# HoangChuongNguyen/ibgs

Measured on AMD Instinct MI355X. Metric: train-step fps (fwd+bwd raster) @1080p, 1M Gaussians, higher is better.
Workload: dtype f32

## Files before the change

ibgs_amd/_lib.py:

```python
import ctypes
import os

_HERE = os.path.dirname(os.path.abspath(__file__))
LIB_PATH = os.environ.get("IBGS_LIB") or os.path.join(_HERE, "libibgs_rast.so")

MAX_SRC = 5
MAX_BUFFER_LENGTH = 8
FLAG_DEBUG = 1
FLAG_TEX_QUANT = 2
FLAG_NO_TILE_CULL = 4
FLAG_CLEAR_GRAD_ACC = 8
FLAG_SH_FACTORED = 16
FLAG_TILE_WAVES = 32
FLAG_QUADRANT_WAVES = 64
FLAG_DETERMINISTIC = 128
FLAG_TEX_PACKED = 256
FLAG_NO_REF_POWER_SKIP = 512
FLAG_NO_ABS_GRAD = 1024
FLAG_REF_ARITH = 4096
FLAG_SRC_DEPTH_SLOTS = 8192
PLANE_NONE, PLANE_LEARNT, PLANE_SMALLEST_AXIS = 0, 1, 2
MAX_VIEWS = 8

c_float_p = ctypes.c_void_p

ALLOC_FN = ctypes.CFUNCTYPE(ctypes.c_void_p, ctypes.c_size_t, ctypes.c_void_p)


class ForwardArgs(ctypes.Structure):
    _fields_ = [
        ("stream", ctypes.c_void_p),
        ("P", ctypes.c_int32), ("D", ctypes.c_int32), ("M", ctypes.c_int32),
        ("W", ctypes.c_int32), ("H", ctypes.c_int32),
        ("means3D", c_float_p), ("shs", c_float_p), ("colors_precomp", c_float_p), ("opacities", c_float_p),
        ("scales", c_float_p), ("rotations", c_float_p), ("cov3D_precomp", c_float_p), ("all_map", c_float_p),
        ("scale_modifier", ctypes.c_float),
        ("bg", c_float_p), ("viewmatrix", c_float_p), ("projmatrix", c_float_p), ("campos", c_float_p),
        ("tanfovx", ctypes.c_float), ("tanfovy", ctypes.c_float),
        ("n_src", ctypes.c_int32),
        ("ref_to_src", c_float_p), ("src_cam_pos", c_float_p), ("src_images", c_float_p), ("src_depths", c_float_p),
        ("buffer_length", ctypes.c_int32), ("depth_error_threshold", ctypes.c_float),
        ("prefiltered", ctypes.c_int32), ("render_geo", ctypes.c_int32), ("render_depth_only", ctypes.c_int32),
        ("flags", ctypes.c_uint32),
        ("geom", ctypes.c_void_p), ("geom_bytes", ctypes.c_size_t),
        ("img", ctypes.c_void_p), ("img_bytes", ctypes.c_size_t),
        ("binning_alloc", ALLOC_FN), ("binning_user", ctypes.c_void_p),
        ("tex", ctypes.c_void_p), ("tex_bytes", ctypes.c_size_t),
        ("out_color", c_float_p), ("radii", ctypes.c_void_p), ("out_normal", c_float_p), ("out_depth", c_float_p),
        ("out_cam_feat", c_float_p), ("out_warped", c_float_p), ("out_min_depth_diff", c_float_p),
        ("out_camera_ray", c_float_p), ("out_mask", ctypes.c_void_p),
        ("rendered_hint", ctypes.c_int64),
        ("plane_normal", c_float_p), ("plane_offset", c_float_p), ("plane_mode", ctypes.c_int32),
        ("n_views", ctypes.c_int32), ("view_tanfovx", ctypes.c_float * 8), ("view_tanfovy", ctypes.c_float * 8),
        ("tile_order_hint", ctypes.c_void_p),
        ("binning", ctypes.c_void_p), ("binning_bytes", ctypes.c_size_t),
        ("shs_rest", c_float_p),
        ("src_depth_slot", ctypes.c_int32 * 5),
    ]


class AdamTensor(ctypes.Structure):
    _fields_ = [("param", ctypes.c_void_p), ("grad", ctypes.c_void_p), ("exp_avg", ctypes.c_void_p), ("exp_avg_sq", ctypes.c_void_p),
                ("numel", ctypes.c_int64), ("lr", ctypes.c_double), ("beta1", ctypes.c_double), ("beta2", ctypes.c_double),
                ("eps", ctypes.c_double), ("bias_correction1", ctypes.c_double), ("bias_correction2", ctypes.c_double)]


class CompactTensor(ctypes.Structure):
    _fields_ = [("src", ctypes.c_void_p), ("append", ctypes.c_void_p), ("dst", ctypes.c_void_p), ("width", ctypes.c_int32), ("reserved", ctypes.c_int32)]


COMPACT_MAX_TENSORS = 40


class BackwardArgs(ctypes.Structure):
    _fields_ = [
        ("stream", ctypes.c_void_p),
        ("P", ctypes.c_int32), ("D", ctypes.c_int32), ("M", ctypes.c_int32),
        ("W", ctypes.c_int32), ("H", ctypes.c_int32),
        ("R", ctypes.c_int64),
        ("means3D", c_float_p), ("shs", c_float_p), ("colors_precomp", c_float_p),
        ("scales", c_float_p), ("rotations", c_float_p), ("cov3D_precomp", c_float_p), ("all_map", c_float_p),
        ("scale_modifier", ctypes.c_float),
        ("bg", c_float_p), ("viewmatrix", c_float_p), ("projmatrix", c_float_p), ("campos", c_float_p),
        ("tanfovx", ctypes.c_float), ("tanfovy", ctypes.c_float),
        ("n_src", ctypes.c_int32),
        ("ref_to_src", c_float_p), ("src_cam_pos", c_float_p), ("src_images", c_float_p), ("src_depths", c_float_p),
        ("radii", ctypes.c_void_p),
        ("out_depth", c_float_p), ("out_warped", c_float_p),
        ("geom", ctypes.c_void_p), ("binning", ctypes.c_void_p), ("img", ctypes.c_void_p),
        ("tex", ctypes.c_void_p), ("tex_bytes", ctypes.c_size_t),
        ("dL_dcolor", c_float_p), ("dL_dnormal", c_float_p), ("dL_ddepth", c_float_p), ("dL_dwarped", c_float_p),
        ("grad_acc", c_float_p),
        ("dL_dmean2D", c_float_p), ("dL_dmean2D_abs", c_float_p), ("dL_dconic", c_float_p), ("dL_dopacity", c_float_p),
        ("dL_dcolors", c_float_p), ("dL_dmean3D", c_float_p), ("dL_dcov3D", c_float_p), ("dL_dsh", c_float_p),
        ("dL_dscale", c_float_p), ("dL_drot", c_float_p), ("dL_dall_map", c_float_p),
        ("render_geo", ctypes.c_int32), ("flags", ctypes.c_uint32),
        ("plane_normal", c_float_p), ("plane_offset", c_float_p), ("plane_mode", ctypes.c_int32),
        ("dL_dplane_normal", c_float_p), ("dL_dplane_offset", c_float_p),
        ("geo_table", ctypes.c_void_p), ("geo_table_bytes", ctypes.c_size_t),
        ("det_scratch", ctypes.c_void_p), ("det_scratch_bytes", ctypes.c_size_t),
        ("buffer_length", ctypes.c_int32),
        ("tile_order_out", ctypes.c_void_p),
        ("shs_rest", c_float_p), ("dL_dsh_rest", c_float_p),
    ]


EXPORTS = ["ibgs_required_geom", "ibgs_required_img", "ibgs_required_binning", "ibgs_required_tex",
           "ibgs_forward", "ibgs_backward", "ibgs_mark_visible", "ibgs_tile_order_slots",
           "ibgs_geom_offset", "ibgs_img_offset", "ibgs_binning_offset",
           "ibgs_sizeof_forward_args", "ibgs_sizeof_backward_args", "ibgs_timing_enable", "ibgs_timing_collect",
           "ibgs_required_knn", "ibgs_knn_mean_dist2", "ibgs_sh_grad_from_views", "ibgs_adam_step", "ibgs_adam_step_sh",
           "ibgs_required_compact", "ibgs_compact_plan", "ibgs_compact_apply", "ibgs_densify_stats", "ibgs_required_deterministic", "ibgs_required_geo_table", "ibgs_required_deterministic_for", "ibgs_required_geo_table_for", "ibgs_last_forward_stats", "ibgs_check_async",
           "ibgs_required_l1", "ibgs_l1_loss", "ibgs_l1_grad", "ibgs_l1_rescale",
           "ibgs_depth_normal_forward", "ibgs_depth_normal_backward", "ibgs_activate_forward", "ibgs_activate_backward",
           "ibgs_last_error", "ibgs_version"]

TSDF_EXPORTS = ["ibgs_tsdf_sizeof_volume", "ibgs_tsdf_sizeof_view", "ibgs_tsdf_sizeof_mesh_scratch", "ibgs_tsdf_mc_table",
                "ibgs_tsdf_integrate", "ibgs_tsdf_mesh_count", "ibgs_tsdf_mesh_emit"]
TSDF_STATE_WORDS = 8
TSDF_ALLOCATED, TSDF_FAILED, TSDF_IGNORED, TSDF_ACTIVE, TSDF_VERTICES, TSDF_FACES, TSDF_OVERRUN, TSDF_TABLE_FULL = range(8)
TSDF_FLAG_NO_DEDUP = 1


class TsdfVolume(ctypes.Structure):
    _fields_ = [("voxel_length", ctypes.c_float), ("sdf_trunc", ctypes.c_float), ("capacity", ctypes.c_int32), ("slot_bits", ctypes.c_int32),
                ("slot_key", ctypes.c_void_p), ("slot_block", ctypes.c_void_p), ("slot_mark", ctypes.c_void_p), ("active", ctypes.c_void_p),
                ("block_key", ctypes.c_void_p), ("tsdf", ctypes.c_void_p), ("weight", ctypes.c_void_p), ("color", ctypes.c_void_p),
                ("state", ctypes.c_void_p)]


class TsdfView(ctypes.Structure):
    _fields_ = [("W", ctypes.c_int32), ("H", ctypes.c_int32), ("fx", ctypes.c_float), ("fy", ctypes.c_float), ("cx", ctypes.c_float),
                ("cy", ctypes.c_float), ("depth_trunc", ctypes.c_float), ("world_to_camera", ctypes.c_float * 12),
                ("camera_to_world", ctypes.c_float * 12)]


class TsdfMeshScratch(ctypes.Structure):
    _fields_ = [("order", ctypes.c_void_p), ("rank", ctypes.c_void_p), ("vinfo", ctypes.c_void_p), ("vcount", ctypes.c_void_p),
                ("fcount", ctypes.c_void_p)]


MESH_EXPORTS = ["ibgs_mesh_sizeof_mesh", "ibgs_mesh_required_scratch", "ibgs_mesh_cluster", "ibgs_mesh_filter_count", "ibgs_mesh_filter_emit"]
MESH_STATE_WORDS = 8
MESH_BAD_FACES, MESH_CLUSTERS, MESH_VERTICES_OUT, MESH_FACES_OUT, MESH_TABLE_FULL, MESH_OVERRUN = range(6)
MESH_KEEP_VERTICES, MESH_KEEP_DEGENERATE = 1, 2


class Mesh(ctypes.Structure):
    _fields_ = [("V", ctypes.c_int32), ("F", ctypes.c_int32), ("vertices", ctypes.c_void_p), ("faces", ctypes.c_void_p), ("scratch", ctypes.c_void_p),
                ("scratch_bytes", ctypes.c_size_t), ("state", ctypes.c_void_p)]


MESH_EVAL_EXPORTS = ["ibgs_meval_required_sample_scratch", "ibgs_meval_sample_count", "ibgs_meval_sample_emit", "ibgs_meval_keys", "ibgs_meval_required_tree",
                     "ibgs_meval_build", "ibgs_meval_thin_rounds", "ibgs_meval_nearest", "ibgs_meval_reduce"]
MEVAL_STATE_WORDS = 8
MEVAL_BAD_FACES, MEVAL_SAMPLE_OVERFLOW, MEVAL_BAD_POINTS, MEVAL_OVERRUN, MEVAL_UNDECIDED = range(5)
MEVAL_MAX_SIDE = 32768
MEVAL_LEAF = 8
MEVAL_THIN_UNDECIDED, MEVAL_THIN_KEPT, MEVAL_THIN_REMOVED = 0, 1, 2

PCREG_EXPORTS = ["ibgs_pcreg_required_scratch", "ibgs_pcreg_bounds", "ibgs_pcreg_transform", "ibgs_pcreg_crop", "ibgs_pcreg_voxel_keys",
                 "ibgs_pcreg_voxel_count", "ibgs_pcreg_voxel_emit", "ibgs_pcreg_moments"]
PCREG_STATE_WORDS = 8
PCREG_BAD_POINTS, PCREG_KEY_OVERFLOW, PCREG_BAD_INDEX, PCREG_OVERRUN = range(4)
PCREG_MAX_POLYGON = 1024
PCREG_MAX_INDEX = (1 << 21) - 1
PCREG_LONG_SEGMENT = 64
PCREG_MOMENTS = 18


_lib = None


# ... 195 lines not shown
```

ibgs_amd/csrc/api.hip:

```cpp
#include "common.h"
#include "sh_color.h"
#include <sched.h>
#include <time.h>
#include <string.h>
#include <cstdlib>
#include <stdlib.h>
#include <stdio.h>
#include <cstdarg>
#include <cstdio>
#include <cstring>
#include <vector>
#include <map>
#include <mutex>

namespace ibgs {

static thread_local char g_err[512] = "";
void set_error(const char* fmt, ...)
{
    va_list ap; va_start(ap, fmt);
    vsnprintf(g_err, sizeof(g_err), fmt, ap);
    va_end(ap);
}

// ... 99 lines not shown

static int stage_check(hipStream_t s, bool debug, const char* what)
{
    if (!debug) return 0;
    hipError_t e = hipStreamSynchronize(s);
    if (e == hipSuccess) e = hipGetLastError();
    if (e != hipSuccess) { set_error("stage '%s' failed: %s", what, hipGetErrorString(e)); return -IBGS_ERR_HIP; }
    return 0;
}

__global__ void __launch_bounds__(1024) rendered_note_kernel(RenderedNote n)
{
    __shared__ unsigned long long s_w[16];
    rendered_note_block<1024>(n, s_w);
}

}

using namespace ibgs;

extern "C" {

const char* ibgs_last_error(void) { return g_err; }
const char* ibgs_version(void) { return "ibgs_rast 0.1 (gfx950)"; }
void ibgs_timing_enable(uint32_t stage_mask) { g_time_mask = stage_mask; }
int32_t ibgs_timing_collect(float* ms, int32_t* launches)
{
    for (int i = 0; i < IBGS_NUM_STAGES; i++) { if (ms) ms[i] = 0.f; if (launches) launches[i] = 0; }
    for (auto& p : g_pairs) {
        float t = 0.f;
        hipError_t e = hipEventSynchronize(p.b);
        if (e == hipSuccess) e = hipEventElapsedTime(&t, p.a, p.b);
        if (e != hipSuccess) { set_error("timing collect: %s", hipGetErrorString(e)); return -IBGS_ERR_HIP; }
        if (ms) ms[p.stage] += t;
        if (launches) launches[p.stage] += 1;
        g_free_events.push_back(p.a); g_free_events.push_back(p.b);
    }
    g_pairs.clear();
    return 0;
}
size_t ibgs_sizeof_forward_args(void) { return sizeof(ibgs_forward_args); }
size_t ibgs_sizeof_backward_args(void) { return sizeof(ibgs_backward_args); }

size_t ibgs_required_geom(int32_t P) { size_t t; GeomState::carve(nullptr, (size_t)(P > 0 ? P : 0), &t); return t; }
size_t ibgs_required_img(int32_t W, int32_t H) { size_t t; ImgState::carve(nullptr, W, H, &t); return t; }
size_t ibgs_required_binning(int64_t R, int32_t W, int32_t H) { size_t t; BinState::carve(nullptr, (size_t)(R > 0 ? R : 0), W, H, &t); return t; }
size_t ibgs_required_deterministic(int64_t R, int32_t P) { size_t t; DetState::carve(nullptr, (size_t)(R > 0 ? R : 0) * 4, (size_t)(P > 0 ? P : 0), &t); return t; }
size_t ibgs_required_tex(int32_t n_src, int32_t W, int32_t H) { return (size_t)n_src * W * H * sizeof(float4) + 128; }
size_t ibgs_required_geo_table(int32_t W, int32_t H) { return geo_table_floats(W, H) * sizeof(float) + 128; }
size_t ibgs_required_geo_table_for(int32_t W, int32_t H, int32_t L)
{
    const int slots = (L >= 1 && L < IBGS_MAX_BUFFER_LENGTH) ? L + 1 : IBGS_MAX_BUFFER_LENGTH;
    return (size_t)W * H * slots * GEO_TAB_FIELDS * sizeof(float) + 128;
}
size_t ibgs_required_deterministic_for(int64_t R, int32_t P, int32_t W, int32_t H, int32_t render_geo, uint32_t flags)
{
    ibgs_backward_args a{}; a.W = W; a.H = H; a.render_geo = render_geo; a.flags = flags;
    size_t t; DetState::carve(nullptr, (size_t)(R > 0 ? R : 0) * render_backward_waves_per_tile(a), (size_t)(P > 0 ? P : 0), &t); return t;
}

#define OFF(base_struct, field) if (!strcmp(name, #field)) return (int64_t)((char*)base_struct.field - (char*)nullptr)
int64_t ibgs_geom_offset(int32_t P, const char* name)
{
    size_t t; GeomState g = GeomState::carve(nullptr, (size_t)P, &t);
    OFF(g, rec); OFF(g, depths); OFF(g, cov3D); OFF(g, tiles); OFF(g, fp); OFF(g, tmask_hi); OFF(g, clamped); OFF(g, offsets);
    if (!strcmp(name, "order")) return (int64_t)((char*)g.sort_val[0] - (char*)nullptr);
    if (!strcmp(name, "order_alt")) return (int64_t)((char*)g.sort_val[1] - (char*)nullptr);
    if (!strcmp(name, "sorted_depth_keys")) return (int64_t)((char*)g.sort_key[0] - (char*)nullptr);
    if (!strcmp(name, "sorted_depth_keys_alt")) return (int64_t)((char*)g.sort_key[1] - (char*)nullptr);
    return -1;
}
size_t ibgs_tile_order_slots(int32_t W, int32_t H)
{
    const size_t tiles = (size_t)((W + TILE - 1) / TILE) * ((H + TILE - 1) / TILE);
    return (tiles + ORDER_CLASSES - 1) / ORDER_CLASSES * ORDER_CLASSES;
}
int64_t ibgs_img_offset(int32_t W, int32_t H, const char* name)
{
    size_t t; ImgState im = ImgState::carve(nullptr, W, H, &t);
    OFF(im, ranges); OFF(im, final_T); OFF(im, n_contrib); OFF(im, sum_w); OFF(im, low_high); OFF(im, valid_idx); OFF(im, valid_w); OFF(im, slot_c); OFF(im, meta); OFF(im, tile_walked); OFF(im, tile_order); OFF(im, tile_risky);
    return -1;
}
int64_t ibgs_binning_offset(int64_t R, int32_t W, int32_t H, const char* name)
{
    size_t t; BinState b = BinState::carve(nullptr, (size_t)R, W, H, &t);
    OFF(b, point_list);
    return -1;
}
#undef OFF

struct RSlot {
    uint32_t* host; hipEvent_t ev;
    uint32_t* stats; bool stats_pending;
    bool flag_pending;
    hipStream_t last_stream;
    uint32_t seq;
};
static std::mutex g_slot_mutex;
static std::map<std::pair<int, hipStream_t>, RSlot*> g_slots;
static RSlot* rslot(hipStream_t s, bool create)
{
    int dev = 0;
    if (hipGetDevice(&dev) != hipSuccess) { set_error("hipGetDevice failed"); return nullptr; }
    std::lock_guard<std::mutex> lock(g_slot_mutex);
    auto it = g_slots.find({dev, s});
    if (it != g_slots.end()) return it->second;
    if (!create) return nullptr;
    RSlot* slot = new RSlot();
    void* p = nullptr;
    if (hipHostMalloc(&p, 64, hipHostMallocCoherent | hipHostMallocMapped) != hipSuccess) { delete slot; set_error("hipHostMalloc for the R read-back failed"); return nullptr; }
    if (hipEventCreateWithFlags(&slot->ev, hipEventDisableTiming) != hipSuccess) { (void)hipHostFree(p); delete slot; set_error("hipEventCreate failed"); return nullptr; }
    slot->host = static_cast<uint32_t*>(p);
    memset(p, 0, 64);
    slot->stats = slot->host + 8;
    slot->stats_pending = false; slot->flag_pending = false; slot->last_stream = s; slot->seq = 0;
    g_slots[{dev, s}] = slot;
    return slot;
}
static int check_sort_flag(RSlot* rs, bool wait_for_note)
{
    if (!rs || !rs->flag_pending) return 0;
    volatile uint32_t* note = rs->stats + 4;
    bool final_ = __atomic_load_n(const_cast<uint32_t*>(note), __ATOMIC_ACQUIRE) == rs->seq;
    if (!final_ && wait_for_note) {
        struct timespec t0, t1; clock_gettime(CLOCK_MONOTONIC, &t0);
        for (uint32_t spins = 1; !final_; spins++) {
            final_ = __atomic_load_n(const_cast<uint32_t*>(note), __ATOMIC_ACQUIRE) == rs->seq;
            if ((spins & 255u) == 0) {
                clock_gettime(CLOCK_MONOTONIC, &t1);
                if ((t1.tv_sec - t0.tv_sec) * 1000000000ll + (t1.tv_nsec - t0.tv_nsec) > 2000000ll) break;
            }
        }
    }
    if (*(volatile uint32_t*)(rs->stats + 3)) {
        rs->stats[3] = 0u; rs->flag_pending = false;
        set_error("depth sort: decoupled look-back timed out (the lists of this stream's last forward were mis-ordered)"); return -IBGS_ERR_HIP;
    }
    if (final_) rs->flag_pending = false;
    return 0;
}

static thread_local int64_t g_last_stats[3] = {0, -1, 0};
static thread_local RSlot* g_stats_slot = nullptr;
void ibgs_last_forward_stats(int64_t* out)
{
    if (g_stats_slot && g_stats_slot->stats_pending) {
        if (hipStreamSynchronize(g_stats_slot->last_stream) == hipSuccess) g_last_stats[1] = (int64_t)*(volatile uint32_t*)(g_stats_slot->stats + 2);
        g_stats_slot->stats_pending = false;
    }
    out[0] = g_last_stats[0]; out[1] = g_last_stats[1]; out[2] = g_last_stats[2];
}
void ibgs_debug_set_lookback_spins(uint32_t v) { radix_set_lookback_spins(v); }
void ibgs_debug_set_sh_ride(int32_t on) { radix_set_sh_ride(on != 0); }
size_t ibgs_debug_scan_scratch_elems(size_t n) { return scan_scratch_elems(n); }
int32_t ibgs_debug_scan_u32(void* stream, const uint32_t* in, uint32_t* out, size_t n, uint32_t* scratch, size_t scratch_elems, int32_t with_total)
{
    return exclusive_scan_u32(reinterpret_cast<hipStream_t>(stream), in, out, n, scratch, scratch_elems, with_total != 0);
}
size_t ibgs_debug_sort_scratch_elems(size_t n) { return radix_hist_elems(n); }
int32_t ibgs_debug_sort_pairs(void* stream, uint32_t* keys0, uint32_t* keys1, uint32_t* vals0, uint32_t* vals1, size_t n, int32_t nbits,
                              uint32_t* scratch, size_t scratch_elems, uint32_t* kept_dev, uint32_t* result_alt)
{
    uint32_t* keys[2] = {keys0, keys1};
    uint32_t* vals[2] = {vals0, vals1};
    return radix_sort_pairs(reinterpret_cast<hipStream_t>(stream), keys, vals, n, nbits, scratch, scratch_elems, nullptr, kept_dev, false, result_alt, nullptr);
}
int32_t ibgs_debug_set_onesweep(int32_t mode) { return radix_set_onesweep(mode); }
int32_t ibgs_check_async(void* stream, int32_t wait)
{
    hipStream_t s = reinterpret_cast<hipStream_t>(stream);
    RSlot* rs = rslot(s, false);
    if (!rs || !rs->flag_pending) return 0;
    if (wait) IBGS_HIP(hipStreamSynchronize(s));
    return check_sort_flag(rs, false);
}

int64_t ibgs_forward(const ibgs_forward_args* ap)
{
    if (!ap) { set_error("null args"); return -IBGS_ERR_INVALID; }
    const ibgs_forward_args& a = *ap;
    hipStream_t s = reinterpret_cast<hipStream_t>(a.stream);
    const bool debug = (a.flags & IBGS_FLAG_DEBUG) != 0;
    if (a.P < 0 || a.W <= 0 || a.H <= 0) { set_error("bad sizes P=%d W=%d H=%d", a.P, a.W, a.H); return -IBGS_ERR_INVALID; }
    if (a.P == 0) return 0;
    if (!a.means3D || !a.opacities || !a.viewmatrix || !a.projmatrix || !a.campos || !a.bg || !a.radii) {
        set_error("missing required pointer"); return -IBGS_ERR_INVALID;
    }
    if ((a.shs == nullptr) == (a.colors_precomp == nullptr) && !a.render_depth_only) {
        set_error("provide exactly one of shs / colors_precomp"); return -IBGS_ERR_INVALID;
    }
    if (((a.scales == nullptr) || (a.rotations == nullptr)) == (a.cov3D_precomp == nullptr)) {
        set_error("provide exactly one of scales+rotations / cov3D_precomp"); return -IBGS_ERR_INVALID;
    }
    if (a.shs && (a.D < 0 || a.D > 3 || (a.D + 1) * (a.D + 1) > a.M)) { set_error("bad SH degree D=%d M=%d", a.D, a.M); return -IBGS_ERR_INVALID; }
    if (a.shs && a.M == 16 && (reinterpret_cast<uintptr_t>(a.shs) & 15u)) { set_error("shs (M = 16) must be 16-byte aligned"); return -IBGS_ERR_INVALID; }
    if (a.shs_rest && (!a.shs || a.M < 2 || (reinterpret_cast<uintptr_t>(a.shs_rest) & 15u) || (reinterpret_cast<uintptr_t>(a.shs) & 15u))) {
        set_error("shs_rest needs shs (the DC coefficients), M >= 2 and 16-byte aligned arrays"); return -IBGS_ERR_INVALID;
    }
    if (a.render_geo && a.render_depth_only) { set_error("render_geo together with render_depth_only is not supported"); return -IBGS_ERR_INVALID; }
    if (a.plane_mode != IBGS_PLANE_NONE) {
        if (a.all_map) { set_error("give either all_map or plane_mode, not both"); return -IBGS_ERR_INVALID; }
        if (a.plane_mode == IBGS_PLANE_LEARNT ? !a.plane_normal : (a.plane_mode != IBGS_PLANE_SMALLEST_AXIS || !a.scales || !a.rotations)) {
            set_error("plane_mode %d: plane_normal (learnt) or scales + rotations (smallest axis) required", a.plane_mode); return -IBGS_ERR_INVALID;
        }
    }
    if ((a.render_geo || a.render_depth_only) && !a.all_map && a.plane_mode == IBGS_PLANE_NONE) { set_error("all_map (or plane_mode) is required for render_geo / render_depth_only"); return -IBGS_ERR_INVALID; }
    if (a.render_geo || a.render_depth_only) {
        if (a.buffer_length < 1 || a.buffer_length > IBGS_MAX_BUFFER_LENGTH) { set_error("buffer_length %d outside 1..%d", a.buffer_length, IBGS_MAX_BUFFER_LENGTH); return -IBGS_ERR_INVALID; }
        if (!a.out_depth) { set_error("out_depth required"); return -IBGS_ERR_INVALID; }
    }
    if (a.render_geo) {
        if (a.n_src < 1 || a.n_src > IBGS_MAX_SRC) { set_error("n_src %d outside 1..%d", a.n_src, IBGS_MAX_SRC); return -IBGS_ERR_INVALID; }
        if (!a.ref_to_src || !a.src_cam_pos || !a.src_images || !a.src_depths) { set_error("source view pointers required for render_geo"); return -IBGS_ERR_INVALID; }
        if (a.flags & IBGS_FLAG_SRC_DEPTH_SLOTS) {
            for (int m = 0; m < a.n_src; m++) if (a.src_depth_slot[m] < 0) { set_error("src_depth_slot[%d] = %d is negative", m, a.src_depth_slot[m]); return -IBGS_ERR_INVALID; }
        }
        if (!a.out_normal || !a.out_cam_feat || !a.out_warped || !a.out_min_depth_diff || !a.out_camera_ray || !a.out_mask) { set_error("geo outputs required"); return -IBGS_ERR_INVALID; }
        if (!a.tex || a.tex_bytes < ibgs_required_tex(a.n_src, a.W, a.H)) { set_error("tex scratch too small"); return -IBGS_ERR_ALLOC; }
    }
    if (!a.render_depth_only && !a.out_color) { set_error("out_color required"); return -IBGS_ERR_INVALID; }
    const int nv = a.n_views > 1 ? a.n_views : 1;
    if (nv > 1) {
        if (nv > IBGS_MAX_VIEWS || !a.render_depth_only || a.plane_mode == IBGS_PLANE_NONE) {
            set_error("n_views = %d needs render_depth_only, plane_mode != 0 and n_views <= %d", a.n_views, IBGS_MAX_VIEWS); return -IBGS_ERR_INVALID;
        }
        if ((int64_t)nv * a.P > 0x7FFFFFFF) { set_error("n_views x P too large"); return -IBGS_ERR_INVALID; }
    }
    const int Pn = nv * a.P;
    const int Hn = nv > 1 ? nv * TILE * ((a.H + TILE - 1) / TILE) : a.H;
    if (!a.geom || a.geom_bytes < ibgs_required_geom(Pn)) { set_error("geom arena too small"); return -IBGS_ERR_ALLOC; }
    if (!a.img || a.img_bytes < ibgs_required_img(a.W, Hn)) { set_error("img arena too small"); return -IBGS_ERR_ALLOC; }
    if (!a.binning_alloc) { set_error("binning_alloc callback required"); return -IBGS_ERR_INVALID; }

    int rc;
    GeomState g = GeomState::carve(a.geom, (size_t)Pn, nullptr);
    ImgState im = ImgState::carve(a.img, a.W, Hn, nullptr);
    const int gx = (a.W + TILE - 1) / TILE, gy = nv * ((a.H + TILE - 1) / TILE);

    const bool deferred = a.rendered_hint > 0 && !debug;
    const size_t nwaves = (size_t)nv * (((size_t)a.P + 63) / 64);
    RSlot* rs = rslot(s, true);
    if (!rs) return -IBGS_ERR_HIP;
    uint32_t ticket = 0;
    ShRide ride;
    bool riding = false;
    { StageTimer t(s, IBGS_STAGE_PREPROCESS);
      if ((rc = launch_preprocess(s, a, g, deferred ? 1 : 0))) return rc;
      if (deferred) {
          ticket = ++rs->seq;
          const RenderedNote note{g.tile_partial, (uint32_t)nwaves, ticket, rs->host};
          riding = radix_takes_sh_ride((size_t)Pn, 32) && preprocess_sh_ride(a, g, &note, &ride);
          if (!riding) {
              if ((rc = launch_preprocess(s, a, g, 2, &note)) < 0) return rc;
              if (rc == 0) { hipLaunchKernelGGL(rendered_note_kernel, dim3(1), dim3(1024), 0, s, note); IBGS_HIP(hipGetLastError()); }
          }
      }
    }
    if ((rc = stage_check(s, debug, "preprocess"))) return rc;
    { StageTimer t(s, IBGS_STAGE_DEPTH_SORT);
      if ((rc = radix_sort_pairs(s, g.sort_key, g.sort_val, (size_t)Pn, 32, g.hist, g.hist_elems, deferred ? g.tile_partial + nwaves : g.offsets + Pn + 1,
                                 g.offsets + Pn + 3, true, g.offsets + Pn + 4, riding ? &ride : nullptr))) return rc; }
    if ((rc = stage_check(s, debug, "depth sort"))) return rc;
    { StageTimer t(s, IBGS_STAGE_SCAN);
      if (!deferred && (rc = exclusive_scan_u32(s, g.tiles, g.offsets, (size_t)Pn, g.hist, g.hist_elems, true))) return rc; }
    auto exact_R = [&](int64_t* R_out) -> int {
        IBGS_HIP(hipMemcpyAsync(rs->host, g.offsets + Pn, 2 * sizeof(uint32_t), hipMemcpyDeviceToHost, s));
        IBGS_HIP(hipEventRecord(rs->ev, s));
        IBGS_HIP(hipEventSynchronize(rs->ev));
        if (rs->host[1]) { set_error("depth sort: decoupled look-back timed out (lists would be mis-ordered)"); return -IBGS_ERR_HIP; }
        *R_out = (int64_t)rs->host[0];
        return 0;
    };
    int64_t R = 0, cap = 0;
    if (deferred) cap = a.rendered_hint < (int64_t)0xFFFF0000ll ? a.rendered_hint : (int64_t)0xFFFF0000ll;
    else { if ((rc = exact_R(&R))) return rc; cap = R; }

    auto tail = [&](int64_t n, bool read_back) -> int {
        int rc;
        const size_t need = ibgs_required_binning(n, a.W, Hn);
        char* bin_mem = (read_back && a.binning && a.binning_bytes >= need) ? a.binning : a.binning_alloc(need, a.binning_user);
        if (!bin_mem) { set_error("binning_alloc returned NULL for R=%lld", (long long)n); return -IBGS_ERR_ALLOC; }
        BinState b = BinState::carve(bin_mem, (size_t)n, a.W, Hn, nullptr);
        { StageTimer t(s, IBGS_STAGE_EMIT);
          if ((rc = launch_binning(s, Pn, n, gx, gy, g, b, im.ranges, a.tile_order_hint, im.meta, nv, read_back ? g.tile_partial + nwaves : nullptr, read_back ? rs->stats : nullptr, ticket))) return rc; }
        if (read_back) { rs->flag_pending = true; rs->last_stream = s; }
        { StageTimer t(s, IBGS_STAGE_TILE_SORT); if ((rc = launch_binning_scatter(s, n, gx, gy, b))) return rc; }
        if ((rc = stage_check(s, debug, "binning"))) return rc;
        const float4* rgba = nullptr;
        if (a.render_geo) {
            float4* t = reinterpret_cast<float4*>((reinterpret_cast<uintptr_t>(a.tex) + 127) & ~uintptr_t(127));
            if (!(a.flags & IBGS_FLAG_TEX_PACKED) && (rc = launch_pack_rgba(s, a.src_images, t, a.W, a.H, a.n_src))) return rc;
            rgba = t;
        }
        { StageTimer t(s, IBGS_STAGE_RENDER_FWD); if ((rc = launch_render_forward(s, a, g, b, im, rgba))) return rc; }
        return stage_check(s, debug, "render");
    };
    const bool prev_pending = rs->flag_pending;
    if ((rc = tail(cap, deferred))) return rc;
    g_last_stats[1] = -1; g_last_stats[2] = 0;
    g_stats_slot = rs; rs->stats_pending = false;
    if (deferred) {
        {
            volatile uint32_t* tk = rs->host + 2;
            const uint32_t want = ticket;
            uint64_t spins = 0;
            struct timespec t0; bool timed = false;
            while (__atomic_load_n(const_cast<uint32_t*>(tk), __ATOMIC_ACQUIRE) != want) {
                if (++spins > 4000) {
                    if (!timed) { clock_gettime(CLOCK_MONOTONIC, &t0); timed = true; }
                    sched_yield();
                    if ((spins & 1023) == 0) {
                        struct timespec t1; clock_gettime(CLOCK_MONOTONIC, &t1);
                        if (t1.tv_sec - t0.tv_sec > 5) {
                            if (hipStreamQuery(s) == hipErrorNotReady) { t0 = t1; continue; }
                            IBGS_HIP(hipStreamSynchronize(s));
                            if (*tk == want) break;
                            set_error("ibgs_forward: the device never reported R (ticket %u, last seen %u)", want, *tk); return -IBGS_ERR_HIP;
                        }
                    }
                }
            }
        }
        if (prev_pending && *(volatile uint32_t*)(rs->stats + 3)) {
            rs->stats[3] = 0u;
            set_error("depth sort of the previous forward: decoupled look-back timed out (its lists were mis-ordered)"); return -IBGS_ERR_HIP;
        }
        const uint64_t sum = (uint64_t)rs->host[0] | ((uint64_t)rs->host[1] << 32);
        R = (int64_t)sum;
        if (R > cap) {
            g_last_stats[2] = 1;
            IBGS_HIP(hipStreamSynchronize(s));
            if ((rc = check_sort_flag(rs, false))) return rc;
            if ((rc = tail(R, false))) return rc;
        } else rs->stats_pending = true;
    }
    g_last_stats[0] = R;
    return R;
}

int32_t ibgs_backward(const ibgs_backward_args* ap)
{
    if (!ap) { set_error("null args"); return -IBGS_ERR_INVALID; }
    const ibgs_backward_args& a = *ap;
    hipStream_t s = reinterpret_cast<hipStream_t>(a.stream);
    const bool debug = (a.flags & IBGS_FLAG_DEBUG) != 0;
    if (a.P <= 0) return 0;
    RSlot* rs = rslot(s, false);
    { int frc = check_sort_flag(rs, false); if (frc) return frc; }
    if (!a.geom || !a.img || (!a.binning && a.R > 0)) { set_error("backward needs the forward's arenas"); return -IBGS_ERR_INVALID; }
    if (!a.grad_acc) { set_error("grad_acc scratch required"); return -IBGS_ERR_INVALID; }
    if (!a.dL_dmean2D || (!a.dL_dmean2D_abs && !(a.flags & IBGS_FLAG_NO_ABS_GRAD)) || !a.dL_dopacity || !a.dL_dmean3D) {
        set_error("missing gradient output"); return -IBGS_ERR_INVALID;
    }
    if (a.shs && !a.dL_dsh && !(a.flags & IBGS_FLAG_SH_FACTORED)) { set_error("dL_dsh required"); return -IBGS_ERR_INVALID; }
    if (a.shs_rest && (!a.shs || a.M < 2 || (!(a.flags & IBGS_FLAG_SH_FACTORED) && !a.dL_dsh_rest)
                       || ((reinterpret_cast<uintptr_t>(a.shs_rest) | reinterpret_cast<uintptr_t>(a.shs) | reinterpret_cast<uintptr_t>(a.dL_dsh_rest) | reinterpret_cast<uintptr_t>(a.dL_dsh)) & 15u))) {
        set_error("shs_rest needs shs, M >= 2, dL_dsh_rest and 16-byte aligned arrays"); return -IBGS_ERR_INVALID;
    }
    if (a.shs && a.M == 16 && ((reinterpret_cast<uintptr_t>(a.shs) & 15u) || (a.dL_dsh && (reinterpret_cast<uintptr_t>(a.dL_dsh) & 15u)))) {
        set_error("shs / dL_dsh (M = 16) must be 16-byte aligned"); return -IBGS_ERR_INVALID;
    }
    if (!a.dL_dcolors && (!a.shs || (a.flags & IBGS_FLAG_SH_FACTORED))) { set_error("dL_dcolors required (precomputed colours, or IBGS_FLAG_SH_FACTORED)"); return -IBGS_ERR_INVALID; }
    if (!a.dL_dcov3D && a.cov3D_precomp) { set_error("dL_dcov3D required with cov3D_precomp"); return -IBGS_ERR_INVALID; }
    if (a.scales && (!a.dL_dscale || !a.dL_drot)) { set_error("dL_dscale / dL_drot required"); return -IBGS_ERR_INVALID; }
    if (a.render_geo) {
        if (a.plane_mode == IBGS_PLANE_NONE ? (!a.all_map || !a.dL_dall_map)
                                            : (a.plane_mode == IBGS_PLANE_LEARNT ? (!a.plane_normal || !a.dL_dplane_normal)
                                                                                 : (a.plane_mode != IBGS_PLANE_SMALLEST_AXIS || !a.scales || !a.rotations))) {
            set_error("geo backward: plane inputs / gradient outputs missing"); return -IBGS_ERR_INVALID;
        }
        if (!a.out_depth || !a.out_warped || !a.ref_to_src || !a.src_images) { set_error("geo backward inputs missing"); return -IBGS_ERR_INVALID; }
        if (!a.tex || a.tex_bytes < ibgs_required_tex(a.n_src, a.W, a.H)) { set_error("tex scratch too small"); return -IBGS_ERR_ALLOC; }
        if (!a.geo_table || a.geo_table_bytes < (a.buffer_length > 0 ? ibgs_required_geo_table_for(a.W, a.H, a.buffer_length) : ibgs_required_geo_table(a.W, a.H))) { set_error("geo_table scratch too small"); return -IBGS_ERR_ALLOC; }
    }
    int rc;
    GeomState g = GeomState::carve(a.geom, (size_t)a.P, nullptr);
    ImgState im = ImgState::carve(a.img, a.W, a.H, nullptr);
    BinState b = BinState::carve(a.binning, (size_t)a.R, a.W, a.H, nullptr);
    const float4* rgba = nullptr;
    float* geo_tab = nullptr;
    if (a.render_geo) {
        float4* t = reinterpret_cast<float4*>((reinterpret_cast<uintptr_t>(a.tex) + 127) & ~uintptr_t(127));
        const bool window = a.dL_ddepth || a.dL_dwarped;
        if (window && !(a.flags & IBGS_FLAG_TEX_PACKED) && (rc = launch_pack_rgba(s, a.src_images, t, a.W, a.H, a.n_src))) return rc;
        rgba = t;
        geo_tab = reinterpret_cast<float*>((reinterpret_cast<uintptr_t>(a.geo_table) + 127) & ~uintptr_t(127));
    }
    if (a.R > 0) {
        const bool det = (a.flags & IBGS_FLAG_DETERMINISTIC) != 0;
        DetState ds{};
        int ipt = 1;
        if (det) {
            if (!a.det_scratch || a.det_scratch_bytes < ibgs_required_deterministic_for(a.R, a.P, a.W, a.H, a.render_geo, a.flags)) { set_error("det_scratch too small"); return -IBGS_ERR_ALLOC; }
            ipt = render_backward_waves_per_tile(a);
            ds = DetState::carve(a.det_scratch, (size_t)a.R * ipt, (size_t)a.P, nullptr);
            if ((rc = launch_det_prepare(s, ds, (size_t)a.R * ipt))) return rc;
        }
        if ((rc = launch_render_backward(s, a, g, b, im, rgba, det ? ds.slab : nullptr, geo_tab))) return rc;
        if (det) { StageTimer t(s, IBGS_STAGE_TILE_ORDER); if ((rc = launch_det_reduce(s, ds, b.point_list, (size_t)a.R, ipt, a.P, a.grad_acc, g.offsets + a.P))) return rc; }
        if ((rc = stage_check(s, debug, "render backward"))) return rc;
    }
    { StageTimer t(s, IBGS_STAGE_PREPROCESS_BWD); if ((rc = launch_preprocess_backward(s, a, g))) return rc; }
    if ((rc = stage_check(s, debug, "preprocess backward"))) return rc;
    return check_sort_flag(rs, true);
}

int32_t ibgs_sh_grad_from_views(void* stream, int32_t P, int32_t D, int32_t M, int32_t n_views, const float* means3D,
                                const float* camposes, const float* dcolor, int64_t view_stride, float* dL_dsh)
{
    if (view_stride == 0) view_stride = (int64_t)P * 3;
    if (view_stride < (int64_t)P * 3) { set_error("view_stride smaller than P x 3"); return -IBGS_ERR_INVALID; }
    if (P <= 0 || M <= 0) return 0;
    if (D < 0 || D > 3 || (D + 1) * (D + 1) > M || n_views < 0) { set_error("bad SH degree / view count"); return -IBGS_ERR_INVALID; }
    if (!means3D || !dL_dsh || (n_views > 0 && (!camposes || !dcolor))) { set_error("null pointer"); return -IBGS_ERR_INVALID; }
    return launch_sh_grad_from_views(reinterpret_cast<hipStream_t>(stream), P, D, M, n_views, means3D, camposes, dcolor, (size_t)view_stride, dL_dsh);
}

int32_t ibgs_mark_visible(void* stream, int32_t P, const float* means3D, const float* viewmatrix,
                          const float* projmatrix, uint8_t* present)
{
    (void)projmatrix;
    if (P <= 0) return 0;
    if (!means3D || !viewmatrix || !present) { set_error("null pointer"); return -IBGS_ERR_INVALID; }
    return launch_mark_visible(reinterpret_cast<hipStream_t>(stream), P, means3D, viewmatrix, present);
}

}
```

ibgs_amd/csrc/common.h:

```cpp
#pragma once
#include <hip/hip_runtime.h>
#include <stdint.h>
#include <stddef.h>
#include <stdlib.h>
#include "../../include/ibgs_rast.h"

namespace ibgs {

constexpr int TILE = IBGS_TILE;
constexpr int WAVE = 64;
constexpr int REC_FLOATS = 16;
constexpr int GACC_FLOATS = 16;

constexpr int IBGS_CULL_WORDS = 4;
constexpr int IBGS_CULL_MAX_TILES = 64 * IBGS_CULL_WORDS;

enum RecField { R_X = 0, R_Y = 1, R_OP = 2, R_PAD0 = 3, R_CA = 4, R_CB = 5, R_CC = 6, R_DIST = 7,
                R_R = 8, R_G = 9, R_B = 10, R_PAD1 = 11, R_NX = 12, R_NY = 13, R_NZ = 14, R_PAD2 = 15 };

enum GaccField { G_SX = 0, G_SY = 1, G_AX = 2, G_AY = 3, G_SXX = 4, G_SXY = 5, G_SYY = 6, G_S0 = 7,
                 G_R = 8, G_G = 9, G_B = 10, G_NX = 11, G_NY = 12, G_NZ = 13, G_DIST = 14, G_PAD = 15 };

struct Carver {
    uintptr_t cur;
// ... 190 lines not shown
    float n[3];
    float ncam[3];
    float dist;
    float flip;
    float sgn;
    float inv_len;
    int axis;
};

__device__ __forceinline__ PlaneEval plane_eval(int mode, const float* __restrict__ raw_n, const float* __restrict__ raw_off,
                                                const float* __restrict__ scales, const float* __restrict__ rot, int i,
                                                float mx, float my, float mz, const float* __restrict__ campos,
                                                const float* __restrict__ vm)
{
    PlaneEval e;
    float off = 0.f;
    e.inv_len = 1.f; e.axis = 0;
    if (mode == IBGS_PLANE_LEARNT) {
        const float a = raw_n[3 * i], b = raw_n[3 * i + 1], c = raw_n[3 * i + 2];
        const float len = sqrtf(a * a + b * b + c * c);
        e.inv_len = 1.0f / len;
        e.n[0] = a / len; e.n[1] = b / len; e.n[2] = c / len;
        off = raw_off ? raw_off[i] : 0.f;
    } else {
        const float s0 = scales[3 * i], s1 = scales[3 * i + 1], s2 = scales[3 * i + 2];
        int k = 0; float sm = s0;
        if (s1 < sm) { sm = s1; k = 1; }
        if (s2 < sm) { sm = s2; k = 2; }
        e.axis = k;
        const float r = rot[4 * i], x = rot[4 * i + 1], y = rot[4 * i + 2], z = rot[4 * i + 3];
        if (k == 0)      { e.n[0] = 1.f - 2.f * (y * y + z * z); e.n[1] = 2.f * (x * y + r * z);       e.n[2] = 2.f * (x * z - r * y); }
        else if (k == 1) { e.n[0] = 2.f * (x * y - r * z);       e.n[1] = 1.f - 2.f * (x * x + z * z); e.n[2] = 2.f * (y * z + r * x); }
        else             { e.n[0] = 2.f * (x * z + r * y);       e.n[1] = 2.f * (y * z - r * x);       e.n[2] = 1.f - 2.f * (x * x + y * y); }
    }
    const float tc = e.n[0] * (campos[0] - mx) + e.n[1] * (campos[1] - my) + e.n[2] * (campos[2] - mz);
    e.flip = (tc < 0.0f) ? -1.f : 1.f;
    e.n[0] *= e.flip; e.n[1] *= e.flip; e.n[2] *= e.flip; off *= e.flip;
#pragma unroll
    for (int j = 0; j < 3; j++) e.ncam[j] = e.n[0] * vm[j] + e.n[1] * vm[4 + j] + e.n[2] * vm[8 + j];
    float gd = -(e.n[0] * mx + e.n[1] * my + e.n[2] * mz);
    if (mode == IBGS_PLANE_LEARNT) gd += off;
    const float sd = gd - (e.ncam[0] * vm[12] + e.ncam[1] * vm[13] + e.ncam[2] * vm[14]);
    e.sgn = sd > 0.f ? 1.f : (sd < 0.f ? -1.f : 0.f);
    e.dist = fabsf(sd);
    return e;
}

enum { TMAP_RR = 0, TMAP_GROUP = 1, TMAP_BLOCK = 2 };
struct TileMap { int mode, g, bx, by; };
inline int tile_map_grid(const TileMap& m, int gx, int gy, int ipt)
{
    if (m.mode == TMAP_BLOCK) {
        const int nb = ((gx + m.bx - 1) / m.bx) * ((gy + m.by - 1) / m.by);
        return ((nb + 7) / 8) * 8 * m.bx * m.by * ipt;
    }
    const int g = m.mode == TMAP_GROUP ? m.g : 1;
    return ((gx * gy * ipt + 8 * g - 1) / (8 * g)) * 8 * g;
}
__device__ __forceinline__ bool tile_map_item(const TileMap& m, int b, int gx, int gy, int ipt, int& tile, int& sub)
{
    const int xcd = b & 7, idx = b >> 3;
    if (m.mode == TMAP_BLOCK) {
        const int per = m.bx * m.by * ipt;
        const int blk = (idx / per) * 8 + xcd, within = idx % per;
        const int nbx = (gx + m.bx - 1) / m.bx;
        const int t = within / ipt;
        const int tx = (blk % nbx) * m.bx + t % m.bx, ty = (blk / nbx) * m.by + t / m.bx;
        sub = within % ipt;
        tile = ty * gx + tx;
        return tx < gx && ty < gy;
    }
    int item = b;
    if (m.mode == TMAP_GROUP) item = ((idx / m.g) * 8 + xcd) * m.g + idx % m.g;
    tile = item / ipt; sub = item % ipt;
    return item < gx * gy * ipt;
}

__device__ __forceinline__ bool hybrid_split(uint32_t work, unsigned long long total, uint32_t theta_pct)
{
    return (unsigned long long)work * 1024ull * 100ull > total * theta_pct;
}
constexpr uint32_t ORDER_SPLIT_BIT = 0x80000000u;
__device__ __forceinline__ bool hybrid_item(int b, int grid1, const uint32_t* __restrict__ order, int& tile, int& sub, bool& split)
{
    const int idx = (b - grid1) >> 3;
    const int slot = b < grid1 ? b : (idx / 3) * 8 + (b & 7);
    sub = b < grid1 ? 0 : idx % 3 + 1;
    const uint32_t t = order[slot];
    split = (t & ORDER_SPLIT_BIT) != 0u;
    tile = (int)(t & ~ORDER_SPLIT_BIT);
    return t != 0xFFFFFFFFu;
}
__device__ __forceinline__ bool hybrid_item_mapped(const TileMap& m, int b, int grid1, int gx, int gy, int& tile, int& sub)
{
    if (b < grid1) { const bool ok = tile_map_item(m, b, gx, gy, 1, tile, sub); sub = 0; return ok; }
    const bool ok = tile_map_item(m, b - grid1, gx, gy, 3, tile, sub);
    sub += 1;
    return ok;
}
constexpr int HYBRID_THETA = 50;
constexpr int HYBRID_MIN_TILES = 768;
constexpr int hybrid_max_tiles() { return 4096; }
constexpr int hybrid_theta() { return HYBRID_THETA; }

struct RenderedNote { const uint32_t* partial; uint32_t nwords; uint32_t ticket; uint32_t* host; };
template <int NT>
__device__ __forceinline__ void rendered_note_block(const RenderedNote& n, unsigned long long* s_w )
{
    unsigned long long sum = 0;
    for (uint32_t i = threadIdx.x; i < n.nwords; i += NT) sum += n.partial[i];
    for (int d = 32; d >= 1; d >>= 1) sum += __shfl_xor(sum, d, 64);
    if ((threadIdx.x & 63) == 0) s_w[threadIdx.x >> 6] = sum;
    __syncthreads();
    if (threadIdx.x == 0) {
        unsigned long long t = 0;
        for (int w = 0; w < NT / 64; w++) t += s_w[w];
        volatile uint32_t* host_words = n.host;
        host_words[0] = (uint32_t)t; host_words[1] = (uint32_t)(t >> 32);
        __threadfence_system();
        __hip_atomic_store(n.host + 2, n.ticket, __ATOMIC_RELEASE, __HIP_MEMORY_SCOPE_SYSTEM);
    }
}
struct ShRide;
int launch_preprocess(hipStream_t s, const ibgs_forward_args& a, const GeomState& g, int phase = 0, const RenderedNote* note = nullptr);
bool preprocess_sh_ride(const ibgs_forward_args& a, const GeomState& g, const RenderedNote* note, ShRide* out);
int launch_mark_visible(hipStream_t s, int P, const float* means3D, const float* vm, uint8_t* present);

size_t radix_hist_elems(size_t n);
int radix_sort_pairs(hipStream_t s, uint32_t* keys[2], uint32_t* vals[2], size_t n, int nbits,
                     uint32_t* hist, size_t hist_elems, uint32_t* err_dev = nullptr, uint32_t* kept_dev = nullptr, bool scratch_is_zero = false,
                     uint32_t* result_alt = nullptr, const ShRide* ride = nullptr);
bool radix_takes_sh_ride(size_t n, int nbits);
void radix_set_sh_ride(bool on);
size_t radix_zero_elems(size_t n, int nbits);
int exclusive_scan_u32(hipStream_t s, const uint32_t* in, uint32_t* out, size_t n, uint32_t* scratch,
                       size_t scratch_elems, bool with_total);
size_t scan_scratch_elems(size_t n);
int radix_set_onesweep(int mode);
void radix_set_lookback_spins(uint32_t v);

int launch_binning(hipStream_t s, int P, int64_t cap, int gx, int gy, const GeomState& g, const BinState& b, uint32_t* ranges,
                   const uint32_t* order_hint = nullptr, uint32_t* meta = nullptr ,
                   int n_views = 1 ,
                   const uint32_t* sort_flag = nullptr, uint32_t* host_note = nullptr ,
                   uint32_t note_ticket = 0 );
constexpr int ORDER_CLASSES = 1024;
int launch_binning_scatter(hipStream_t s, int64_t cap, int gx, int gy, const BinState& b);

int launch_pack_rgba(hipStream_t s, const float* src, float4* dst, int W, int H, int n);
constexpr int GEO_TAB_FIELDS = 6;
inline size_t geo_table_floats(int W, int H) { return (size_t)W * H * IBGS_MAX_BUFFER_LENGTH * GEO_TAB_FIELDS; }
int launch_render_forward(hipStream_t s, const ibgs_forward_args& a, const GeomState& g, const BinState& b,
                          const ImgState& im, const float4* src_rgba);
int launch_render_backward(hipStream_t s, const ibgs_backward_args& a, const GeomState& g, const BinState& b,
                           const ImgState& im, const float4* src_rgba, float* slab = nullptr, float* geo_tab = nullptr);
int launch_preprocess_backward(hipStream_t s, const ibgs_backward_args& a, const GeomState& g);

struct DetState {
    float* slab;
    uint32_t* keys[2];
    uint32_t* vals[2];
    uint32_t* seg;
    uint32_t* hist; size_t hist_elems;
    static DetState carve(char* base, size_t rows, size_t P, size_t* total);
};
int render_backward_waves_per_tile(const ibgs_backward_args& a);
int render_backward_ref_arith(uint32_t flags);
int launch_det_prepare(hipStream_t s, const DetState& d, size_t rows);
int launch_det_reduce(hipStream_t s, const DetState& d, const uint32_t* point_list, size_t R, int ipt, int P, float* gacc, const uint32_t* listed );
int launch_sh_grad_from_views(hipStream_t s, int P, int D, int M, int n_views, const float* means3D, const float* camposes,
                              const float* dcolor, size_t view_stride, float* dL_dsh);

__device__ __forceinline__ uint32_t pack_rect(int lo, int hi) { return (uint32_t)lo | ((uint32_t)hi << 16); }

}
```

ibgs_amd/csrc/preprocess_bwd.hip:

```cpp
#include "common.h"
#include "adam_math.h"

namespace ibgs {

__constant__ float bC1 = 0.4886025119029199f;
__constant__ float bC0 = 0.28209479177387814f;
__constant__ float bC2[5] = {1.0925484305920792f, -1.0925484305920792f, 0.31539156525252005f,
                             -1.0925484305920792f, 0.5462742152960396f};
__constant__ float bC3[7] = {-0.5900435899266435f, 2.890611442640554f, -0.4570457994644658f,
                             0.3731763325901154f, -0.4570457994644658f, 1.445305721320277f,
                             -0.5900435899266435f};

struct PreBwdParams {
    int P, D, M;
    const float* means3D; const int32_t* radii; const float* shs; const float* shs_rest; const uint8_t* clamped;
    const float* scales; const float* rotations; float scale_modifier;
    const float* cov3D;
    float* gacc;
    int clear_gacc;
    int risky_rows;
    const float* rec;
    float* dL_dmean2D; float* dL_dmean2D_abs; float* dL_dconic; float* dL_dopacity; float* dL_dcolors;
    float* dL_dall_map; float* dL_dmean3D; float* dL_dcov3D; float* dL_dsh; float* dL_dsh_rest; float* dL_dscale; float* dL_drot;
    const float* plane_normal; const float* plane_offset; int plane_mode;
    float* dL_dplane_normal; float* dL_dplane_offset;
};

__device__ __forceinline__ int sh_basis(int D, float x, float y, float z, float (&B)[16])
{
    int nb = 1;
    B[0] = bC0;
    const float xx = x * x, yy = y * y, zz = z * z, xy = x * y, yz = y * z, xz = x * z;
    if (D > 0) {
        B[1] = -bC1 * y; B[2] = bC1 * z; B[3] = -bC1 * x; nb = 4;
        if (D > 1) {
            B[4] = bC2[0] * xy; B[5] = bC2[1] * yz; B[6] = bC2[2] * (2.0f * zz - xx - yy);
            B[7] = bC2[3] * xz; B[8] = bC2[4] * (xx - yy); nb = 9;
            if (D > 2) {
                B[9] = bC3[0] * y * (3.0f * xx - yy); B[10] = bC3[1] * xy * z;
                B[11] = bC3[2] * y * (4.0f * zz - xx - yy);
                B[12] = bC3[3] * z * (2.0f * zz - 3.0f * xx - 3.0f * yy);
                B[13] = bC3[4] * x * (4.0f * zz - xx - yy); B[14] = bC3[5] * z * (xx - yy);
                B[15] = bC3[6] * x * (xx - 3.0f * yy); nb = 16;
            }
        }
    }
    return nb;
}

template <bool FAST16, bool WRITE_SH, bool SPLIT = false>
__global__ void __launch_bounds__(FAST16 ? 64 : 256) preprocess_bwd_kernel(PreBwdParams p, Cam cam)
{
    __shared__ float4 s_t[FAST16 ? 64 * 13 : 1];
    const int i = blockIdx.x * blockDim.x + threadIdx.x;
    const bool valid = i < p.P;
    bool vis = valid && (p.radii[i] > 0);
    float4 g0 = make_float4(0.f, 0.f, 0.f, 0.f), g1 = g0, g2 = g0, g3 = g0;
    if (vis) {
        float4* grow = reinterpret_cast<float4*>(p.gacc + (size_t)i * GACC_FLOATS);
        g0 = grow[0]; g1 = grow[1]; g2 = grow[2]; g3 = grow[3];
        const uint32_t any = (__float_as_uint(g0.x) | __float_as_uint(g0.y) | __float_as_uint(g0.z) | __float_as_uint(g0.w) |
                              __float_as_uint(g1.x) | __float_as_uint(g1.y) | __float_as_uint(g1.z) | __float_as_uint(g1.w) |
                              __float_as_uint(g2.x) | __float_as_uint(g2.y) | __float_as_uint(g2.z) | __float_as_uint(g2.w) |
                              __float_as_uint(g3.x) | __float_as_uint(g3.y) | __float_as_uint(g3.z) | __float_as_uint(g3.w)) & 0x7FFFFFFFu;
        if (any == 0u) vis = false;
        else if (p.clear_gacc) { const float4 z = make_float4(0.f, 0.f, 0.f, 0.f); grow[0] = z; grow[1] = z; grow[2] = z; grow[3] = z; }
    }
    float gv[(FAST16 && WRITE_SH) ? 48 : 1];
    if (FAST16 && WRITE_SH) {
#pragma unroll
        for (int k = 0; k < 48; k++) gv[k] = 0.f;
    }
    if (valid && !vis) {
        p.dL_dmean2D[3 * i] = 0.f; p.dL_dmean2D[3 * i + 1] = 0.f; p.dL_dmean2D[3 * i + 2] = 0.f;
        if (p.dL_dmean2D_abs) { p.dL_dmean2D_abs[3 * i] = 0.f; p.dL_dmean2D_abs[3 * i + 1] = 0.f; p.dL_dmean2D_abs[3 * i + 2] = 0.f; }
        if (p.dL_dconic) { p.dL_dconic[4 * i] = 0.f; p.dL_dconic[4 * i + 1] = 0.f; p.dL_dconic[4 * i + 2] = 0.f; p.dL_dconic[4 * i + 3] = 0.f; }
        p.dL_dopacity[i] = 0.f;
        if (p.dL_dcolors) { p.dL_dcolors[3 * i] = 0.f; p.dL_dcolors[3 * i + 1] = 0.f; p.dL_dcolors[3 * i + 2] = 0.f; }
        if (p.dL_dall_map) for (int k = 0; k < 5; k++) p.dL_dall_map[5 * i + k] = 0.f;
        if (p.dL_dplane_normal) { p.dL_dplane_normal[3 * i] = 0.f; p.dL_dplane_normal[3 * i + 1] = 0.f; p.dL_dplane_normal[3 * i + 2] = 0.f; }
        if (p.dL_dplane_offset) p.dL_dplane_offset[i] = 0.f;
        p.dL_dmean3D[3 * i] = 0.f; p.dL_dmean3D[3 * i + 1] = 0.f; p.dL_dmean3D[3 * i + 2] = 0.f;
        if (p.dL_dcov3D) for (int k = 0; k < 6; k++) p.dL_dcov3D[6 * i + k] = 0.f;
        if (!FAST16 && WRITE_SH && p.shs) {
            if (SPLIT) {
                float* gd = p.dL_dsh + (size_t)i * 3; float* gr = p.dL_dsh_rest + (size_t)i * (p.M - 1) * 3;
                gd[0] = gd[1] = gd[2] = 0.f;
                for (int k = 0; k < 3 * (p.M - 1); k++) gr[k] = 0.f;
            } else { float* gsh = p.dL_dsh + (size_t)i * p.M * 3; for (int k = 0; k < 3 * p.M; k++) gsh[k] = 0.f; }
        }
        if (p.scales) {
            p.dL_dscale[3 * i] = 0.f; p.dL_dscale[3 * i + 1] = 0.f; p.dL_dscale[3 * i + 2] = 0.f;
            p.dL_drot[4 * i] = 0.f; p.dL_drot[4 * i + 1] = 0.f; p.dL_drot[4 * i + 2] = 0.f; p.dL_drot[4 * i + 3] = 0.f;
        }
    }
    if (FAST16 && SPLIT && p.shs) {
        const int lane = threadIdx.x;
        const uint64_t vism = __builtin_amdgcn_ballot_w64(vis);
        const int i0 = blockIdx.x * 64;
        const int nrows = min(64, p.P - i0);
        const float4* rest4 = reinterpret_cast<const float4*>(p.shs_rest + (size_t)i0 * 45);
        const float4* dc4 = reinterpret_cast<const float4*>(p.shs + (size_t)i0 * 3);
        float4 v[12];
#pragma unroll
        for (int it = 0; it < 12; it++) {
            const int q = it * 64 + lane;
            v[it] = make_float4(0.f, 0.f, 0.f, 0.f);
            if (q < 720) {
                const int ra = (4 * q) / 45, rb = (4 * q + 3) / 45;
                if (((vism >> ra) & 1ull) || ((vism >> rb) & 1ull)) {
                    if (4 * q + 3 < nrows * 45) v[it] = rest4[q];
                    else { const float* sp = p.shs_rest + (size_t)i0 * 45; float* f = &v[it].x; for (int k = 0; k < 4; k++) if (4 * q + k < nrows * 45) f[k] = sp[4 * q + k]; }
                }
            } else {
                const int qd = q - 720, ra = (4 * qd) / 3, rb = (4 * qd + 3) / 3;
                if ((((vism >> ra) & 3ull) != 0ull) || ((vism >> rb) & 1ull)) {
                    if (4 * qd + 3 < nrows * 3) v[it] = dc4[qd];
                    else { const float* sp = p.shs + (size_t)i0 * 3; float* f = &v[it].x; for (int k = 0; k < 4; k++) if (4 * qd + k < nrows * 3) f[k] = sp[4 * qd + k]; }
                }
            }
        }
#pragma unroll
        for (int it = 0; it < 12; it++) s_t[it * 64 + lane] = v[it];
        __syncthreads();
    }
    if (vis) {

    const float4* rrow = reinterpret_cast<const float4*>(p.rec + (size_t)i * REC_FLOATS);
    const float4 r0 = rrow[0], r1 = rrow[1];
    const float ddelx_dx = (float)(0.5 * cam.W), ddely_dy = (float)(0.5 * cam.H);
    const float ca2 = r1.x, cb2 = r1.y, cc2 = r1.z, opa = r0.z;
    const int risky_row = conic_takes_ref_power(ca2, cb2, cc2) ? p.risky_rows : 0;
    const bool ref_row = risky_row == 2, l_row = risky_row == 1;
    const float g2x = ref_row ? ddelx_dx * g0.x : (l_row ? -ddelx_dx * (g0.x * EXP2_UNSCALE) : -ddelx_dx * (ca2 * g0.x + cb2 * g0.y));
    const float g2y = ref_row ? ddely_dy * g0.y : (l_row ? -ddely_dy * (g0.y * EXP2_UNSCALE) : -ddely_dy * (cc2 * g0.y + cb2 * g0.x));
    const float gcx = -0.5f * g1.x, gcy = -0.5f * g1.y, gcz = -0.5f * g1.z;
    const float gcol[3] = {g2.x, g2.y, g2.z};

    p.dL_dmean2D[3 * i] = g2x; p.dL_dmean2D[3 * i + 1] = g2y; p.dL_dmean2D[3 * i + 2] = 0.f;
    const float abs_unscale = ref_row ? 1.0f : EXP2_UNSCALE;
    if (p.dL_dmean2D_abs) { p.dL_dmean2D_abs[3 * i] = ddelx_dx * (g0.z * abs_unscale); p.dL_dmean2D_abs[3 * i + 1] = ddely_dy * (g0.w * abs_unscale); p.dL_dmean2D_abs[3 * i + 2] = 0.f; }
    if (p.dL_dconic && !l_row) { p.dL_dconic[4 * i] = gcx; p.dL_dconic[4 * i + 1] = gcy; p.dL_dconic[4 * i + 2] = 0.f; p.dL_dconic[4 * i + 3] = gcz; }
    p.dL_dopacity[i] = ref_row ? g1.w : (opa > 0.f ? g1.w / opa : 0.f);
    if ((WRITE_SH || !p.shs) && p.dL_dcolors) { p.dL_dcolors[3 * i] = gcol[0]; p.dL_dcolors[3 * i + 1] = gcol[1]; p.dL_dcolors[3 * i + 2] = gcol[2]; }
    if (p.dL_dall_map) {
        p.dL_dall_map[5 * i] = g2.w; p.dL_dall_map[5 * i + 1] = g3.x; p.dL_dall_map[5 * i + 2] = g3.y;
        p.dL_dall_map[5 * i + 3] = 0.f; p.dL_dall_map[5 * i + 4] = g3.z;
    }

    const float* __restrict__ vm = cam.vm; const float* __restrict__ pm = cam.pm;
    const float mean[3] = {p.means3D[3 * i], p.means3D[3 * i + 1], p.means3D[3 * i + 2]};

    float pgm[3] = {0.f, 0.f, 0.f}, prot[4] = {0.f, 0.f, 0.f, 0.f};
    if (p.plane_mode) {
        const PlaneEval e = plane_eval(p.plane_mode, p.plane_normal, p.plane_offset, p.scales, p.rotations, i, mean[0], mean[1], mean[2], cam.campos, vm);
        const float gnc[3] = {g2.w, g3.x, g3.y};
        const float ggd = e.sgn * g3.z;
        float gl[3], gn0[3];
#pragma unroll
        for (int j = 0; j < 3; j++) gl[j] = gnc[j] - ggd * vm[12 + j];
#pragma unroll
        for (int k = 0; k < 3; k++) {
            const float gn = gl[0] * vm[4 * k] + gl[1] * vm[4 * k + 1] + gl[2] * vm[4 * k + 2] - ggd * mean[k];
            gn0[k] = e.flip * gn;
            pgm[k] = -ggd * e.n[k];
        }
        if (p.plane_mode == IBGS_PLANE_LEARNT) {
            const float u[3] = {e.n[0] * e.flip, e.n[1] * e.flip, e.n[2] * e.flip};
            const float dot = u[0] * gn0[0] + u[1] * gn0[1] + u[2] * gn0[2];
#pragma unroll
            for (int k = 0; k < 3; k++) p.dL_dplane_normal[3 * i + k] = (gn0[k] - u[k] * dot) * e.inv_len;
            if (p.dL_dplane_offset) p.dL_dplane_offset[i] = e.flip * ggd;
        } else {
            const float r_ = p.rotations[4 * i], x = p.rotations[4 * i + 1], y = p.rotations[4 * i + 2], z = p.rotations[4 * i + 3];
            const float a = gn0[0], b = gn0[1], c = gn0[2];
            if (e.axis == 0) {
                prot[0] = 2.f * (z * b - y * c); prot[1] = 2.f * (y * b + z * c);
                prot[2] = -4.f * y * a + 2.f * x * b - 2.f * r_ * c; prot[3] = -4.f * z * a + 2.f * r_ * b + 2.f * x * c;
            } else if (e.axis == 1) {
                prot[0] = 2.f * (x * c - z * a); prot[1] = 2.f * y * a - 4.f * x * b + 2.f * r_ * c;
                prot[2] = 2.f * (x * a + z * c); prot[3] = -2.f * r_ * a - 4.f * z * b + 2.f * y * c;
            } else {
                prot[0] = 2.f * (y * a - x * b); prot[1] = 2.f * z * a - 2.f * r_ * b - 4.f * x * c;
                prot[2] = 2.f * r_ * a + 2.f * z * b - 4.f * y * c; prot[3] = 2.f * (x * a + y * b);
            }
        }
    }
    float c6[6];
#pragma unroll
    for (int k = 0; k < 6; k++) c6[k] = p.cov3D[6 * i + k];

    float t[3] = {vm[0] * mean[0] + vm[4] * mean[1] + vm[8] * mean[2] + vm[12],
                  vm[1] * mean[0] + vm[5] * mean[1] + vm[9] * mean[2] + vm[13],
                  vm[2] * mean[0] + vm[6] * mean[1] + vm[10] * mean[2] + vm[14]};
    const float limx = 1.3f * cam.tanfovx, limy = 1.3f * cam.tanfovy;
    const float txtz = t[0] / t[2], tytz = t[1] / t[2];
    t[0] = fminf(limx, fmaxf(-limx, txtz)) * t[2];
    t[1] = fminf(limy, fmaxf(-limy, tytz)) * t[2];
    const float xmul = (txtz < -limx || txtz > limx) ? 0.f : 1.f;
    const float ymul = (tytz < -limy || tytz > limy) ? 0.f : 1.f;
    const float fx = cam.fx, fy = cam.fy;
    const float j00 = fx / t[2], j02 = -(fx * t[0]) / (t[2] * t[2]);
    const float j11 = fy / t[2], j12 = -(fy * t[1]) / (t[2] * t[2]);
    float A[2][3];
#pragma unroll
    for (int r = 0; r < 3; r++) {
        const float rv0 = vm[4 * r + 0], rv1 = vm[4 * r + 1], rv2 = vm[4 * r + 2];
        A[0][r] = rv0 * j00 + rv1 * 0.0f + rv2 * j02;
        A[1][r] = rv0 * 0.0f + rv1 * j11 + rv2 * j12;
    }
    const float S[3][3] = {{c6[0], c6[1], c6[2]}, {c6[1], c6[3], c6[4]}, {c6[2], c6[4], c6[5]}};
    float SA[2][3];
#pragma unroll
    for (int a = 0; a < 2; a++)
#pragma unroll
        for (int r = 0; r < 3; r++) SA[a][r] = S[r][0] * A[a][0] + S[r][1] * A[a][1] + S[r][2] * A[a][2];
    const float a_ = A[0][0] * SA[0][0] + A[0][1] * SA[0][1] + A[0][2] * SA[0][2] + 0.3f;
    const float b_ = A[0][0] * SA[1][0] + A[0][1] * SA[1][1] + A[0][2] * SA[1][2];
    const float c_ = A[1][0] * SA[1][0] + A[1][1] * SA[1][1] + A[1][2] * SA[1][2] + 0.3f;
    const float denom = a_ * c_ - b_ * b_;
    float da = 0, db = 0, dc = 0;
    const float d2inv = 1.0f / ((denom * denom) + 0.0000001f);
    float gS[6] = {0, 0, 0, 0, 0, 0};
    if (d2inv != 0) {
        da = d2inv * (-c_ * c_ * gcx + 2 * b_ * c_ * gcy + (denom - a_ * c_) * gcz);
        dc = d2inv * (-a_ * a_ * gcz + 2 * a_ * b_ * gcy + (denom - a_ * c_) * gcx);
        db = d2inv * 2 * (b_ * c_ * gcx - (denom + 2 * b_ * b_) * gcy + a_ * b_ * gcz);
        if (l_row) {
            const float kk = d2inv * (denom * denom);
            const float m00 = g1.x * (EXP2_UNSCALE * EXP2_UNSCALE), m01 = g1.y * (EXP2_UNSCALE * EXP2_UNSCALE), m11 = g1.z * (EXP2_UNSCALE * EXP2_UNSCALE);
            da = kk * 0.5f * m00; db = kk * m01; dc = kk * 0.5f * m11;
            if (p.dL_dconic) {
                p.dL_dconic[4 * i] = -0.5f * (a_ * a_ * m00 + 2 * a_ * b_ * m01 + b_ * b_ * m11);
                p.dL_dconic[4 * i + 1] = -0.5f * (a_ * b_ * m00 + (a_ * c_ + b_ * b_) * m01 + b_ * c_ * m11);
                p.dL_dconic[4 * i + 2] = 0.f;
                p.dL_dconic[4 * i + 3] = -0.5f * (b_ * b_ * m00 + 2 * b_ * c_ * m01 + c_ * c_ * m11);
            }
        }
        gS[0] = (A[0][0] * A[0][0] * da + A[0][0] * A[1][0] * db + A[1][0] * A[1][0] * dc);
        gS[3] = (A[0][1] * A[0][1] * da + A[0][1] * A[1][1] * db + A[1][1] * A[1][1] * dc);
        gS[5] = (A[0][2] * A[0][2] * da + A[0][2] * A[1][2] * db + A[1][2] * A[1][2] * dc);
        gS[1] = 2 * A[0][0] * A[0][1] * da + (A[0][0] * A[1][1] + A[0][1] * A[1][0]) * db + 2 * A[1][0] * A[1][1] * dc;
        gS[2] = 2 * A[0][0] * A[0][2] * da + (A[0][0] * A[1][2] + A[0][2] * A[1][0]) * db + 2 * A[1][0] * A[1][2] * dc;
        gS[4] = 2 * A[0][2] * A[0][1] * da + (A[0][1] * A[1][2] + A[0][2] * A[1][1]) * db + 2 * A[1][1] * A[1][2] * dc;
    }
#pragma unroll
    for (int k = 0; k < 6; k++) if (p.dL_dcov3D) p.dL_dcov3D[6 * i + k] = gS[k];
    float dA[2][3];
#pragma unroll
    for (int r = 0; r < 3; r++) {
        const float a0S = A[0][0] * S[r][0] + A[0][1] * S[r][1] + A[0][2] * S[r][2];
        const float a1S = A[1][0] * S[r][0] + A[1][1] * S[r][1] + A[1][2] * S[r][2];
        dA[0][r] = 2 * a0S * da + a1S * db;
        dA[1][r] = 2 * a1S * dc + a0S * db;
    }
    const float dJ00 = vm[0] * dA[0][0] + vm[4] * dA[0][1] + vm[8] * dA[0][2];
    const float dJ02 = vm[2] * dA[0][0] + vm[6] * dA[0][1] + vm[10] * dA[0][2];
    const float dJ11 = vm[1] * dA[1][0] + vm[5] * dA[1][1] + vm[9] * dA[1][2];
    const float dJ12 = vm[2] * dA[1][0] + vm[6] * dA[1][1] + vm[10] * dA[1][2];
    const float tz = 1.f / t[2], tz2 = tz * tz, tz3 = tz2 * tz;
    const float dtx = xmul * -fx * tz2 * dJ02;
    const float dty = ymul * -fy * tz2 * dJ12;
    const float dtz = -fx * tz2 * dJ00 - fy * tz2 * dJ11 + (2 * fx * t[0]) * tz3 * dJ02 + (2 * fy * t[1]) * tz3 * dJ12;
    float gm[3] = {vm[0] * dtx + vm[1] * dty + vm[2] * dtz,
                   vm[4] * dtx + vm[5] * dty + vm[6] * dtz,
                   vm[8] * dtx + vm[9] * dty + vm[10] * dtz};

    const float hw = pm[3] * mean[0] + pm[7] * mean[1] + pm[11] * mean[2] + pm[15];
    const float mw = 1.0f / (hw + 0.0000001f);
    const float mul1 = (pm[0] * mean[0] + pm[4] * mean[1] + pm[8] * mean[2] + pm[12]) * mw * mw;
    const float mul2 = (pm[1] * mean[0] + pm[5] * mean[1] + pm[9] * mean[2] + pm[13]) * mw * mw;
    gm[0] += (pm[0] * mw - pm[3] * mul1) * g2x + (pm[1] * mw - pm[3] * mul2) * g2y;
    gm[1] += (pm[4] * mw - pm[7] * mul1) * g2x + (pm[5] * mw - pm[7] * mul2) * g2y;
    gm[2] += (pm[8] * mw - pm[11] * mul1) * g2x + (pm[9] * mw - pm[11] * mul2) * g2y;

    if (p.shs) {
        const float dorig[3] = {mean[0] - cam.campos[0], mean[1] - cam.campos[1], mean[2] - cam.campos[2]};
        const float len = sqrtf(dorig[0] * dorig[0] + dorig[1] * dorig[1] + dorig[2] * dorig[2]);
        const float x = dorig[0] / len, y = dorig[1] / len, z = dorig[2] / len;
        const float* shg = p.shs + (size_t)i * (SPLIT ? 1 : p.M) * 3;
        float* gsh = p.dL_dsh + (size_t)i * p.M * 3;
        float shv[FAST16 ? 48 : 1];
        if (FAST16) {
            if (SPLIT) {
                const float* s_w = reinterpret_cast<const float*>(s_t);
                const float* rr = s_w + 45 * threadIdx.x;
                const float* rd = s_w + 2880 + 3 * threadIdx.x;
                shv[0] = rd[0]; shv[1] = rd[1]; shv[2] = rd[2];
#pragma unroll
                for (int k = 0; k < 45; k++) shv[3 + k] = rr[k];
            } else {
                const float4* r4 = reinterpret_cast<const float4*>(shg);
#pragma unroll
                for (int v = 0; v < 12; v++) { const float4 q = r4[v]; shv[4 * v] = q.x; shv[4 * v + 1] = q.y; shv[4 * v + 2] = q.z; shv[4 * v + 3] = q.w; }
            }
        }
        const uint8_t cb = p.clamped[i];
        float g[3];
#pragma unroll
        for (int ch = 0; ch < 3; ch++) g[ch] = gcol[ch] * (((cb >> ch) & 1) ? 0.f : 1.f);
        if (!WRITE_SH) { p.dL_dcolors[3 * i] = g[0]; p.dL_dcolors[3 * i + 1] = g[1]; p.dL_dcolors[3 * i + 2] = g[2]; }
        float B[16];
        const int D = p.D;
        const int nb = sh_basis(D, x, y, z, B);
        const float xx = x * x, yy = y * y, zz = z * z, xy = x * y, yz = y * z, xz = x * z;
        if (!WRITE_SH) {
        } else if (FAST16) {
#pragma unroll
            for (int k = 0; k < 16; k++) {
                if (k < nb) { gv[3 * k] = B[k] * g[0]; gv[3 * k + 1] = B[k] * g[1]; gv[3 * k + 2] = B[k] * g[2]; }
            }
        } else if (SPLIT) {
            float* gd = p.dL_dsh + (size_t)i * 3; float* gr = p.dL_dsh_rest + (size_t)i * (p.M - 1) * 3;
            gd[0] = B[0] * g[0]; gd[1] = B[0] * g[1]; gd[2] = B[0] * g[2];
            for (int k = 1; k < nb; k++) { gr[3 * (k - 1)] = B[k] * g[0]; gr[3 * (k - 1) + 1] = B[k] * g[1]; gr[3 * (k - 1) + 2] = B[k] * g[2]; }
            for (int k = 3 * (nb - 1); k < 3 * (p.M - 1); k++) gr[k] = 0.f;
        } else {
            for (int k = 0; k < nb; k++) {
                gsh[3 * k] = B[k] * g[0]; gsh[3 * k + 1] = B[k] * g[1]; gsh[3 * k + 2] = B[k] * g[2];
            }
            for (int k = 3 * nb; k < 3 * p.M; k++) gsh[k] = 0.f;
        }
        float gd[3] = {0, 0, 0};
        if (D > 0) {
            float dx3[3], dy3[3], dz3[3];
#define SHK(k, ch) (FAST16 ? shv[3 * (k) + (ch)] : ((SPLIT && (k) > 0) ? p.shs_rest[((size_t)i * (p.M - 1) + ((k) - 1)) * 3 + (ch)] : shg[3 * (k) + (ch)]))
#pragma unroll
            for (int ch = 0; ch < 3; ch++) {
                dx3[ch] = -bC1 * SHK(3, ch); dy3[ch] = -bC1 * SHK(1, ch); dz3[ch] = bC1 * SHK(2, ch);
                if (D > 1) {
                    dx3[ch] += bC2[0] * y * SHK(4, ch) + bC2[2] * 2.f * -x * SHK(6, ch) + bC2[3] * z * SHK(7, ch) + bC2[4] * 2.f * x * SHK(8, ch);
                    dy3[ch] += bC2[0] * x * SHK(4, ch) + bC2[1] * z * SHK(5, ch) + bC2[2] * 2.f * -y * SHK(6, ch) + bC2[4] * 2.f * -y * SHK(8, ch);
                    dz3[ch] += bC2[1] * y * SHK(5, ch) + bC2[2] * 2.f * 2.f * z * SHK(6, ch) + bC2[3] * x * SHK(7, ch);
                    if (D > 2) {
                        dx3[ch] += (bC3[0] * SHK(9, ch) * 3.f * 2.f * xy + bC3[1] * SHK(10, ch) * yz + bC3[2] * SHK(11, ch) * -2.f * xy +
                                    bC3[3] * SHK(12, ch) * -3.f * 2.f * xz + bC3[4] * SHK(13, ch) * (-3.f * xx + 4.f * zz - yy) +
                                    bC3[5] * SHK(14, ch) * 2.f * xz + bC3[6] * SHK(15, ch) * 3.f * (xx - yy));
                        dy3[ch] += (bC3[0] * SHK(9, ch) * 3.f * (xx - yy) + bC3[1] * SHK(10, ch) * xz + bC3[2] * SHK(11, ch) * (-3.f * yy + 4.f * zz - xx) +
                                    bC3[3] * SHK(12, ch) * -3.f * 2.f * yz + bC3[4] * SHK(13, ch) * -2.f * xy +
                                    bC3[5] * SHK(14, ch) * -2.f * yz + bC3[6] * SHK(15, ch) * -3.f * 2.f * xy);
                        dz3[ch] += (bC3[1] * SHK(10, ch) * xy + bC3[2] * SHK(11, ch) * 4.f * 2.f * yz + bC3[3] * SHK(12, ch) * 3.f * (2.f * zz - xx - yy) +
                                    bC3[4] * SHK(13, ch) * 4.f * 2.f * xz + bC3[5] * SHK(14, ch) * (xx - yy));
                    }
                }
            }
#undef SHK
            gd[0] = dx3[0] * g[0] + dx3[1] * g[1] + dx3[2] * g[2];
            gd[1] = dy3[0] * g[0] + dy3[1] * g[1] + dy3[2] * g[2];
            gd[2] = dz3[0] * g[0] + dz3[1] * g[1] + dz3[2] * g[2];
        }
        const float s2 = dorig[0] * dorig[0] + dorig[1] * dorig[1] + dorig[2] * dorig[2];
        const float inv32 = 1.0f / sqrtf(s2 * s2 * s2);
        gm[0] += ((+s2 - dorig[0] * dorig[0]) * gd[0] - dorig[1] * dorig[0] * gd[1] - dorig[2] * dorig[0] * gd[2]) * inv32;
        gm[1] += (-dorig[0] * dorig[1] * gd[0] + (s2 - dorig[1] * dorig[1]) * gd[1] - dorig[2] * dorig[1] * gd[2]) * inv32;
        gm[2] += (-dorig[0] * dorig[2] * gd[0] - dorig[1] * dorig[2] * gd[1] + (s2 - dorig[2] * dorig[2]) * gd[2]) * inv32;
    }
    p.dL_dmean3D[3 * i] = gm[0] + pgm[0]; p.dL_dmean3D[3 * i + 1] = gm[1] + pgm[1]; p.dL_dmean3D[3 * i + 2] = gm[2] + pgm[2];

    if (p.scales) {
        const float r_ = p.rotations[4 * i], x = p.rotations[4 * i + 1], y = p.rotations[4 * i + 2], z = p.rotations[4 * i + 3];
        float R[3][3];
        R[0][0] = 1.f - 2.f * (y * y + z * z); R[0][1] = 2.f * (x * y - r_ * z);      R[0][2] = 2.f * (x * z + r_ * y);
        R[1][0] = 2.f * (x * y + r_ * z);      R[1][1] = 1.f - 2.f * (x * x + z * z); R[1][2] = 2.f * (y * z - r_ * x);
        R[2][0] = 2.f * (x * z - r_ * y);      R[2][1] = 2.f * (y * z + r_ * x);      R[2][2] = 1.f - 2.f * (x * x + y * y);
        const float sv[3] = {p.scale_modifier * p.scales[3 * i], p.scale_modifier * p.scales[3 * i + 1], p.scale_modifier * p.scales[3 * i + 2]};
        float Mm[3][3], dS[3][3], dM[3][3], G[3][3];
#pragma unroll
        for (int r = 0; r < 3; r++)
#pragma unroll
            for (int cc = 0; cc < 3; cc++) Mm[r][cc] = sv[r] * R[cc][r];
        dS[0][0] = gS[0]; dS[1][1] = gS[3]; dS[2][2] = gS[5];
        dS[0][1] = dS[1][0] = 0.5f * gS[1]; dS[0][2] = dS[2][0] = 0.5f * gS[2]; dS[1][2] = dS[2][1] = 0.5f * gS[4];
#pragma unroll
        for (int r = 0; r < 3; r++)
#pragma unroll
            for (int cc = 0; cc < 3; cc++) dM[r][cc] = 2.0f * (Mm[r][0] * dS[0][cc] + Mm[r][1] * dS[1][cc] + Mm[r][2] * dS[2][cc]);
#pragma unroll
        for (int r = 0; r < 3; r++) p.dL_dscale[3 * i + r] = R[0][r] * dM[r][0] + R[1][r] * dM[r][1] + R[2][r] * dM[r][2];
#pragma unroll
        for (int r = 0; r < 3; r++)
#pragma unroll
            for (int cc = 0; cc < 3; cc++) G[r][cc] = sv[r] * dM[r][cc];
        p.dL_drot[4 * i + 0] = prot[0] + 2 * z * (G[0][1] - G[1][0]) + 2 * y * (G[2][0] - G[0][2]) + 2 * x * (G[1][2] - G[2][1]);
        p.dL_drot[4 * i + 1] = prot[1] + 2 * y * (G[1][0] + G[0][1]) + 2 * z * (G[2][0] + G[0][2]) + 2 * r_ * (G[1][2] - G[2][1]) - 4 * x * (G[2][2] + G[1][1]);
        p.dL_drot[4 * i + 2] = prot[2] + 2 * x * (G[1][0] + G[0][1]) + 2 * r_ * (G[2][0] - G[0][2]) + 2 * z * (G[1][2] + G[2][1]) - 4 * y * (G[2][2] + G[0][0]);
        p.dL_drot[4 * i + 3] = prot[3] + 2 * r_ * (G[0][1] - G[1][0]) + 2 * x * (G[2][0] + G[0][2]) + 2 * y * (G[1][2] + G[2][1]) - 4 * z * (G[1][1] + G[0][0]);
    }
    }

    if (FAST16 && WRITE_SH && SPLIT && p.shs) {
        const int lane = threadIdx.x;
        __syncthreads();
        float* s_w = reinterpret_cast<float*>(s_t);
        s_w[2880 + 3 * lane] = gv[0]; s_w[2880 + 3 * lane + 1] = gv[1]; s_w[2880 + 3 * lane + 2] = gv[2];
#pragma unroll
        for (int k = 0; k < 45; k++) s_w[45 * lane + k] = gv[3 + k];
        __syncthreads();
        const int i0 = blockIdx.x * 64;
        const int nrows = min(64, p.P - i0);
        float4* dr = reinterpret_cast<float4*>(p.dL_dsh_rest + (size_t)i0 * 45);
        float4* dd = reinterpret_cast<float4*>(p.dL_dsh + (size_t)i0 * 3);
#pragma unroll
        for (int it = 0; it < 12; it++) {
            const int q = it * 64 + lane;
            const float4 f4 = s_t[q];
            const float f[4] = {f4.x, f4.y, f4.z, f4.w};
            if (q < 720) {
                if (4 * q + 3 < nrows * 45) dr[q] = f4;
                else { float* op = p.dL_dsh_rest + (size_t)i0 * 45; for (int k = 0; k < 4; k++) if (4 * q + k < nrows * 45) op[4 * q + k] = f[k]; }
            } else {
                const int qd = q - 720;
                if (4 * qd + 3 < nrows * 3) dd[qd] = f4;
                else { float* op = p.dL_dsh + (size_t)i0 * 3; for (int k = 0; k < 4; k++) if (4 * qd + k < nrows * 3) op[4 * qd + k] = f[k]; }
            }
        }
    } else if (FAST16 && WRITE_SH && p.shs) {
        const int lane = threadIdx.x;
#pragma unroll
        for (int v = 0; v < 12; v++) s_t[lane * 13 + v] = make_float4(gv[4 * v], gv[4 * v + 1], gv[4 * v + 2], gv[4 * v + 3]);
        __syncthreads();
        const int i0 = blockIdx.x * 64;
        const int nrows = min(64, p.P - i0);
        float4* dst = reinterpret_cast<float4*>(p.dL_dsh + (size_t)i0 * 48);
#pragma unroll
        for (int k = 0; k < 12; k++) {
            const int f = lane + 64 * k;
            const int r = f / 12, c = f - 12 * r;
            if (r < nrows) dst[f] = s_t[r * 13 + c];
        }
    }
}

int launch_preprocess_backward(hipStream_t s, const ibgs_backward_args& a, const GeomState& g)
{
    PreBwdParams p;
    p.P = a.P; p.D = a.D; p.M = a.M;
    p.means3D = a.means3D; p.radii = a.radii; p.shs = a.shs; p.shs_rest = a.shs_rest; p.clamped = g.clamped;
    p.scales = a.scales; p.rotations = a.rotations; p.scale_modifier = a.scale_modifier;
    p.cov3D = a.cov3D_precomp ? a.cov3D_precomp : g.cov3D;
    p.gacc = a.grad_acc; p.rec = g.rec; p.clear_gacc = (a.flags & IBGS_FLAG_CLEAR_GRAD_ACC) ? 1 : 0;
    { const int ra = render_backward_ref_arith(a.flags); p.risky_rows = (ra & 4) ? 2 : ((ra & 2) ? 1 : 0); }
    p.dL_dmean2D = a.dL_dmean2D; p.dL_dmean2D_abs = a.dL_dmean2D_abs; p.dL_dconic = a.dL_dconic;
    p.dL_dopacity = a.dL_dopacity; p.dL_dcolors = a.dL_dcolors; p.dL_dall_map = a.dL_dall_map;
    p.dL_dmean3D = a.dL_dmean3D; p.dL_dcov3D = a.dL_dcov3D; p.dL_dsh = a.dL_dsh; p.dL_dsh_rest = a.dL_dsh_rest; p.dL_dscale = a.dL_dscale; p.dL_drot = a.dL_drot;
    p.plane_normal = a.plane_normal; p.plane_offset = a.plane_offset; p.plane_mode = a.plane_mode;
    p.dL_dplane_normal = a.dL_dplane_normal; p.dL_dplane_offset = a.dL_dplane_offset;
    const Cam cam = make_cam(a.viewmatrix, a.projmatrix, a.campos, a.bg, a.tanfovx, a.tanfovy, a.W, a.H);
    const bool factored = a.shs && (a.flags & IBGS_FLAG_SH_FACTORED);
    const bool split = a.shs && a.shs_rest;
    if (a.shs && a.M == 16) {
        if (factored && split) hipLaunchKernelGGL((preprocess_bwd_kernel<true, false, true>), dim3((a.P + 63) / 64), dim3(64), 0, s, p, cam);
        else if (factored) hipLaunchKernelGGL((preprocess_bwd_kernel<true, false>), dim3((a.P + 63) / 64), dim3(64), 0, s, p, cam);
        else if (split) hipLaunchKernelGGL((preprocess_bwd_kernel<true, true, true>), dim3((a.P + 63) / 64), dim3(64), 0, s, p, cam);
        else hipLaunchKernelGGL((preprocess_bwd_kernel<true, true>), dim3((a.P + 63) / 64), dim3(64), 0, s, p, cam);
    } else {
        if (factored && split) hipLaunchKernelGGL((preprocess_bwd_kernel<false, false, true>), dim3((a.P + 255) / 256), dim3(256), 0, s, p, cam);
        else if (factored) hipLaunchKernelGGL((preprocess_bwd_kernel<false, false>), dim3((a.P + 255) / 256), dim3(256), 0, s, p, cam);
        else if (split) hipLaunchKernelGGL((preprocess_bwd_kernel<false, true, true>), dim3((a.P + 255) / 256), dim3(256), 0, s, p, cam);
        else hipLaunchKernelGGL((preprocess_bwd_kernel<false, true>), dim3((a.P + 255) / 256), dim3(256), 0, s, p, cam);
    }
    IBGS_HIP(hipGetLastError());
    return 0;
}

template <bool FAST16>
__global__ void __launch_bounds__(FAST16 ? 64 : 256) sh_grad_from_views_kernel(int P, int D, int M, int n_views, size_t view_stride, const float* __restrict__ means3D,
                                                                                const float* __restrict__ camposes, const float* __restrict__ dcolor,
                                                                                float* __restrict__ dL_dsh)
{
    __shared__ float4 s_t[FAST16 ? 64 * 13 : 1];
    const int i = blockIdx.x * blockDim.x + threadIdx.x;
    float acc[48];
#pragma unroll
    for (int k = 0; k < 48; k++) acc[k] = 0.f;
    if (i < P) {
        const float mx = means3D[3 * i], my = means3D[3 * i + 1], mz = means3D[3 * i + 2];
        for (int v = 0; v < n_views; v++) {
            const float* g = dcolor + (size_t)v * view_stride + (size_t)i * 3;
            const float g0 = g[0], g1 = g[1], g2 = g[2];
            const float dx = mx - camposes[3 * v], dy = my - camposes[3 * v + 1], dz = mz - camposes[3 * v + 2];
            const float len = sqrtf(dx * dx + dy * dy + dz * dz);
            float B[16];
            const int nb = sh_basis(D, dx / len, dy / len, dz / len, B);
#pragma unroll
            for (int k = 0; k < 16; k++) {
                if (k < nb) { acc[3 * k] += B[k] * g0; acc[3 * k + 1] += B[k] * g1; acc[3 * k + 2] += B[k] * g2; }
            }
        }
    }
    if (FAST16) {
        const int lane = threadIdx.x;
#pragma unroll
        for (int v = 0; v < 12; v++) s_t[lane * 13 + v] = make_float4(acc[4 * v], acc[4 * v + 1], acc[4 * v + 2], acc[4 * v + 3]);
        __syncthreads();
        const int i0 = blockIdx.x * 64;
        const int nrows = min(64, P - i0);
        float4* dst = reinterpret_cast<float4*>(dL_dsh + (size_t)i0 * 48);
#pragma unroll
        for (int k = 0; k < 12; k++) {
            const int f = lane + 64 * k;
            const int r = f / 12, c = f - 12 * r;
            if (r < nrows) dst[f] = s_t[r * 13 + c];
        }
    } else if (i < P) {
        float* gsh = dL_dsh + (size_t)i * M * 3;
        const int nact = min(M, 16);
#pragma unroll
        for (int k = 0; k < 16; k++) if (k < nact) { gsh[3 * k] = acc[3 * k]; gsh[3 * k + 1] = acc[3 * k + 1]; gsh[3 * k + 2] = acc[3 * k + 2]; }
        for (int k = 3 * nact; k < 3 * M; k++) gsh[k] = 0.f;
    }
}

int launch_sh_grad_from_views(hipStream_t s, int P, int D, int M, int n_views, const float* means3D, const float* camposes,
                              const float* dcolor, size_t view_stride, float* dL_dsh)
{
    if (M == 16) hipLaunchKernelGGL(sh_grad_from_views_kernel<true>, dim3((P + 63) / 64), dim3(64), 0, s, P, D, M, n_views, view_stride, means3D, camposes, dcolor, dL_dsh);
    else hipLaunchKernelGGL(sh_grad_from_views_kernel<false>, dim3((P + 255) / 256), dim3(256), 0, s, P, D, M, n_views, view_stride, means3D, camposes, dcolor, dL_dsh);
    IBGS_HIP(hipGetLastError());
    return 0;
}

struct AdamShParams {
    int P, D, n_views, n; size_t view_stride;
    const float* means3D; const float* camposes; const float* dcolor;
    AdamDev t[2]; int k0[2], K3[2]; uint32_t inv24[2];
};
constexpr int ASH_ROW = 49;
__global__ void __launch_bounds__(256) adam_sh_kernel(AdamShParams q)
{
    __shared__ float s_g[64 * ASH_ROW];
    const int tid = threadIdx.x;
    const int i0 = blockIdx.x * 64;
    if (tid < 64) {
        const int i = i0 + tid;
        float acc[48];
#pragma unroll
        for (int k = 0; k < 48; k++) acc[k] = 0.f;
        if (i < q.P) {
            const float mx = q.means3D[3 * i], my = q.means3D[3 * i + 1], mz = q.means3D[3 * i + 2];
            for (int v = 0; v < q.n_views; v++) {
                const float* g = q.dcolor + (size_t)v * q.view_stride + (size_t)i * 3;
                const float g0 = g[0], g1 = g[1], g2 = g[2];
                const float dx = mx - q.camposes[3 * v], dy = my - q.camposes[3 * v + 1], dz = mz - q.camposes[3 * v + 2];
                const float len = sqrtf(dx * dx + dy * dy + dz * dz);
                float B[16];
                const int nb = sh_basis(q.D, dx / len, dy / len, dz / len, B);
#pragma unroll
                for (int k = 0; k < 16; k++) {
                    if (k < nb) { acc[3 * k] += B[k] * g0; acc[3 * k + 1] += B[k] * g1; acc[3 * k + 2] += B[k] * g2; }
                }
            }
        }
#pragma unroll
        for (int k = 0; k < 48; k++) s_g[tid * ASH_ROW + k] = acc[k];
    }
    __syncthreads();
    const int nrows = min(64, q.P - i0);
    for (int t = 0; t < q.n; t++) {
        const AdamDev d = q.t[t];
        const int K3 = q.K3[t], off = 3 * q.k0[t];
        const uint32_t inv = q.inv24[t];
        const size_t base = (size_t)i0 * K3;
        const int count = nrows * K3;
        auto grad_of = [&](int e) { const int r = (int)(((uint32_t)e * inv) >> 24); return s_g[r * ASH_ROW + off + (e - r * K3)]; };
        const bool vec_ok = ((reinterpret_cast<uintptr_t>(d.param) | reinterpret_cast<uintptr_t>(d.exp_avg) | reinterpret_cast<uintptr_t>(d.exp_avg_sq)) & 15u) == 0;
        const int nvec = vec_ok ? (count & ~3) : 0;
        for (int e = tid * 4; e < nvec; e += 256 * 4) {
            float4 p = *reinterpret_cast<float4*>(d.param + base + e);
            float4 m = *reinterpret_cast<float4*>(d.exp_avg + base + e), v = *reinterpret_cast<float4*>(d.exp_avg_sq + base + e);
            adam_one(p.x, grad_of(e), m.x, v.x, d);
            adam_one(p.y, grad_of(e + 1), m.y, v.y, d);
            adam_one(p.z, grad_of(e + 2), m.z, v.z, d);
            adam_one(p.w, grad_of(e + 3), m.w, v.w, d);
            *reinterpret_cast<float4*>(d.param + base + e) = p;
            *reinterpret_cast<float4*>(d.exp_avg + base + e) = m; *reinterpret_cast<float4*>(d.exp_avg_sq + base + e) = v;
        }
        for (int e = nvec + tid; e < count; e += 256) {
            float p = d.param[base + e], m = d.exp_avg[base + e], v = d.exp_avg_sq[base + e];
            adam_one(p, grad_of(e), m, v, d);
            d.param[base + e] = p; d.exp_avg[base + e] = m; d.exp_avg_sq[base + e] = v;
        }
    }
}

}

extern "C" int32_t ibgs_adam_step_sh(void* stream, int32_t P, int32_t D, int32_t n_views, const float* means3D, const float* camposes, const float* dcolor,
                                     int64_t view_stride, int32_t n_tensors, const ibgs_adam_tensor* tensors, const int32_t* first_coeff, const int32_t* n_coeff)
{
    using namespace ibgs;
    if (P <= 0 || n_tensors <= 0) return 0;
    if (n_tensors > 2 || !tensors || !first_coeff || !n_coeff) { set_error("ibgs_adam_step_sh: 1 or 2 coefficient tensors"); return -IBGS_ERR_INVALID; }
    if (D < 0 || D > 3 || n_views < 1 || !means3D || !camposes || !dcolor) { set_error("ibgs_adam_step_sh: D in 0..3, n_views >= 1, non-null factors"); return -IBGS_ERR_INVALID; }
    AdamShParams q;
    q.P = P; q.D = D; q.n_views = n_views; q.n = 0; q.view_stride = view_stride > 0 ? (size_t)view_stride : (size_t)P * 3;
    q.means3D = means3D; q.camposes = camposes; q.dcolor = dcolor;
    for (int t = 0; t < n_tensors; t++) {
        const ibgs_adam_tensor& d = tensors[t];
        const int k0 = first_coeff[t], K = n_coeff[t];
        if (K <= 0) continue;
        if (k0 < 0 || k0 + K > 16) { set_error("ibgs_adam_step_sh: tensor %d holds coefficients %d .. %d (of 16)", t, k0, k0 + K - 1); return -IBGS_ERR_INVALID; }
        if (!d.param || !d.exp_avg || !d.exp_avg_sq || d.numel != (int64_t)P * K * 3) { set_error("ibgs_adam_step_sh: tensor %d must hold P x %d x 3 floats", t, K); return -IBGS_ERR_INVALID; }
        if (!(d.bias_correction1 > 0.f) || !(d.bias_correction2 > 0.f)) { set_error("ibgs_adam_step_sh: bias corrections must be positive"); return -IBGS_ERR_INVALID; }
        q.t[q.n] = adam_dev_from(d); q.t[q.n].grad = nullptr;
        q.k0[q.n] = k0; q.K3[q.n] = 3 * K; q.inv24[q.n] = (uint32_t)(((1u << 24) + 3u * (uint32_t)K - 1u) / (3u * (uint32_t)K));
        q.n++;
    }
    if (q.n == 0) return 0;
    hipLaunchKernelGGL(adam_sh_kernel, dim3((unsigned)((P + 63) / 64)), dim3(256), 0, reinterpret_cast<hipStream_t>(stream), q);
    IBGS_HIP(hipGetLastError());
    return 0;
}
// ... 1 lines not shown
```

ibgs_amd/csrc/render_bwd.hip:

```cpp
#include "common.h"
#include <stdlib.h>
#include "wave_reduce.h"
#include <type_traits>

namespace ibgs {

struct BwdParams {
    const uint32_t* ranges; const uint32_t* point_list; const float4* rec;
    Cam cam;
    int ntiles;
    TileMap tmap;
    int n_src; int tex_quant;
    int power_skip;
    const uint32_t* tile_risky;
    const float* ref_to_src; const float4* src_rgba;
    const float* final_T; const uint32_t* n_contrib; const float* sum_w; const uint32_t* low_high;
    const int32_t* valid_idx; const float* valid_w;
    const float* depth_pixels; const float* warped_pixels;
    const float* dL_dcolor; const float* dL_dnormal; const float* dL_ddepth; const float* dL_dwarped;
    float* gacc;
    int tab_slots;
    const uint32_t* slot_c; const uint32_t* meta; float* tab;
    const uint32_t* order;
    int slab_ipt;
// ... 521 lines not shown
                    p2q[2] = fmaf(-16.0f, ly0, P0 + 64.0f * cc);
                    p2q[3] = fmaf(128.0f, cb, p2q[2] + (p2q[1] - P0));
                    if constexpr (ABS) {
                        lxq[2] = fmaf(-8.0f, cb, lx0); lyq[2] = fmaf(-8.0f, cc, ly0);
                        lxq[3] = fmaf(-8.0f, cb, lxq[1]); lyq[3] = fmaf(-8.0f, cc, lyq[1]);
                    }
                }
                if constexpr (!RISK) {
                    if ((riskm >> j) & 1ull) {
                        const uint32_t gid = __builtin_amdgcn_readfirstlane(__float_as_uint(q0.w));
                        const float4 g0 = p.rec[(size_t)gid * 4], g1 = p.rec[(size_t)gid * 4 + 1];
#pragma unroll
                        for (int q = 0; q < PPL; q++) {
                            const float ox = (PPL == 4) ? (float)((q & 1) * 8) : (float)(q * 8), oy = (PPL == 4) ? (float)((q >> 1) * 8) : 0.f;
                            p2q[q] = ref_power_E(g0.x - (pxf0 + ox), g0.y - (pyf0 + oy), g1.x, g1.y, g1.z, nlo);
                        }
                    }
                }
                if constexpr (RISK) {
                    if ((riskm >> j) & 1ull) {
                        const uint32_t gid = __builtin_amdgcn_readfirstlane(__float_as_uint(q0.w));
                        const float4 g0 = p.rec[(size_t)gid * 4], g1 = p.rec[(size_t)gid * 4 + 1];
                        float rs[8] = {0.f, 0.f, 0.f, 0.f, 0.f, 0.f, 0.f, 0.f}, rR = 0.f, rG = 0.f, rB = 0.f, rNx = 0.f, rNy = 0.f, rNz = 0.f, rD = 0.f;
                        bool rany = false;
#pragma unroll
                        for (int q = 0; q < PPL; q++) {
                            const float ox = (PPL == 4) ? (float)((q & 1) * 8) : (float)(q * 8), oy = (PPL == 4) ? (float)((q >> 1) * 8) : 0.f;
                            const float dx = g0.x - (pxf0 + ox), dy = g0.y - (pyf0 + oy);
                            const float power = ref_power(dx, dy, g1.x, g1.y, g1.z);
                            const float E = ref_power_E(dx, dy, g1.x, g1.y, g1.z, nlo);
                            const uint64_t okm = __builtin_amdgcn_ballot_w64(k < ncontrib[q]) & __builtin_amdgcn_ballot_w64(E <= ALPHA_SKIP_E);
                            if (okm == 0ull) continue;
                            rany = true;
                            const float Gr = __builtin_amdgcn_inverse_ballot_w64(okm) ? expf(power) : 0.f;
                            const float oG = g0.z * Gr;
                            const float alpha = fminf(0.99f, oG);
                            const float om = 1.f - alpha;
                            T[q] = T[q] / om;
                            const float w = alpha * T[q];
                            const float4 gp = s_gpix[q][lane], gn = s_gnrm[q][lane];
                            const float cg = q2.x * gp.x + q2.y * gp.y + q2.z * gp.z + q3.x * gn.x + q3.y * gn.y + q3.z * gn.z;
                            float dL_dalpha = cg - S[q];
                            S[q] = fmaf(alpha, dL_dalpha, S[q]);
                            rR = fmaf(w, gp.x, rR); rG = fmaf(w, gp.y, rG); rB = fmaf(w, gp.z, rB);
                            rNx = fmaf(w, gn.x, rNx); rNy = fmaf(w, gn.y, rNy); rNz = fmaf(w, gn.z, rNz);
                            const uint64_t hit = okm & __builtin_amdgcn_ballot_w64(k + 1u == next_c[q]);
                            if (hit != 0ull) {
                                if (__builtin_amdgcn_inverse_ballot_w64(hit)) {
                                    const float* e = p.tab + (size_t)(slot[q] * GEO_TAB_FIELDS) * HW + pixo[q];
                                    dL_dalpha += e[HW];
                                    rNx = fmaf(w, e[2 * HW], rNx); rNy = fmaf(w, e[3 * HW], rNy); rNz = fmaf(w, e[4 * HW], rNz);
                                    rD = fmaf(w, e[5 * HW], rD);
                                    slot[q]++;
                                    next_c[q] = (slot[q] < (uint32_t)p.tab_slots) ? __float_as_uint(e[(size_t)GEO_TAB_FIELDS * HW]) : 0u;
                                }
                            }
                            dL_dalpha = dL_dalpha * T[q];
                            if constexpr (!BG0) dL_dalpha += gp.w / om;
                            ref_pair_sums(rs, Gr, dL_dalpha, dx, dy, g0.z, g1.x, g1.y, g1.z);
                        }
                        if (__builtin_amdgcn_ballot_w64(rany) != 0ull) {
                            float v[16] = {rs[0], rs[1], rs[2], rs[3], rs[4], rs[5], rs[6], rs[7], rR, rG, rB, rNx, rNy, rNz, rD, 0.f};
                            const float tot = wave_transpose_reduce16(v, lane);
                            if (col >= 0) {
                                if (p.slab) p.slab[((size_t)(r0 + k) * (p.slab_ipt ? p.slab_ipt : IPT) + (size_t)sub) * GACC_FLOATS + col] = tot;
                                else atomicAdd(p.gacc + (size_t)gid * GACC_FLOATS + col, tot);
                            }
                        }
                        continue;
                    }
                }
                float Q[PPL], aX = 0.f, aY = 0.f, vR = 0.f, vG = 0.f, vB = 0.f, vNx = 0.f, vNy = 0.f, vNz = 0.f, vD = 0.f;
                bool any = false;
#pragma unroll
                for (int q = 0; q < PPL; q++) {
                    const uint64_t live = STABLE ? ncm[q] : __builtin_amdgcn_ballot_w64(k < ncontrib[q]);
                    const uint64_t okm = live & __builtin_amdgcn_ballot_w64(p2q[q] <= ALPHA_SKIP_E);
                    Q[q] = 0.f;
                    if (okm != 0ull) {
                        any = true;
                        const float oG = select_or_zero_after_trans(okm, __builtin_amdgcn_exp2f(-p2q[q]));
                        const float alpha = min_099(oG);
                        const float rinv = __builtin_amdgcn_rcpf(1.f - alpha);
                        T[q] = T[q] * rinv;
                        const float w = alpha * T[q];
                        const float4 gp = s_gpix[q][lane], gn = s_gnrm[q][lane];
                        const float cg = q2.x * gp.x + q2.y * gp.y + q2.z * gp.z + q3.x * gn.x + q3.y * gn.y + q3.z * gn.z;
                        float dL_dalpha = cg - S[q];
                        S[q] = fmaf(alpha, dL_dalpha, S[q]);
                        vR = fmaf(w, gp.x, vR); vG = fmaf(w, gp.y, vG); vB = fmaf(w, gp.z, vB);
                        vNx = fmaf(w, gn.x, vNx); vNy = fmaf(w, gn.y, vNy); vNz = fmaf(w, gn.z, vNz);
                        const uint64_t hit = okm & __builtin_amdgcn_ballot_w64(k + 1u == next_c[q]);
                        if (hit != 0ull) {
                            if (__builtin_amdgcn_inverse_ballot_w64(hit)) {
                                const float* e = p.tab + (size_t)(slot[q] * GEO_TAB_FIELDS) * HW + pixo[q];
                                dL_dalpha += e[HW];
                                vNx = fmaf(w, e[2 * HW], vNx); vNy = fmaf(w, e[3 * HW], vNy); vNz = fmaf(w, e[4 * HW], vNz);
                                vD = fmaf(w, e[5 * HW], vD);
                                slot[q]++;
                                next_c[q] = (slot[q] < (uint32_t)p.tab_slots) ? __float_as_uint(e[(size_t)GEO_TAB_FIELDS * HW]) : 0u;
                            }
                        }
                        if constexpr (BG0) dL_dalpha = dL_dalpha * T[q];
                        else dL_dalpha = fmaf(dL_dalpha, T[q], gp.w * rinv);
                        const float qv = oG * dL_dalpha;
                        Q[q] = qv;
                        if constexpr (ABS) { aX = fmaf(fabsf(qv), fabsf(lxq[q]), aX); aY = fmaf(fabsf(qv), fabsf(lyq[q]), aY); }
                    }
                }
                if (__builtin_amdgcn_ballot_w64(any) != 0ull) {
                    float v[16];
                    if (!RISK && ((riskm >> j) & 1ull)) l_moments<PPL>(v, Q, dx0, dy0, ca, cb, cc);
                    else
                    if constexpr (PPL == 4) {
                        const float A = Q[1] + Q[3], B = Q[2] + Q[3], S0 = (Q[0] + Q[2]) + A;
                        const float t = dx0 * S0, u = dy0 * S0;
                        v[0] = fmaf(-8.0f, A, t); v[1] = fmaf(-8.0f, B, u);
                        v[4] = fmaf(dx0, fmaf(-16.0f, A, t), 64.0f * A);
                        v[6] = fmaf(dy0, fmaf(-16.0f, B, u), 64.0f * B);
                        v[5] = fmaf(-8.0f, fmaf(-8.0f, Q[3], dx0 * B), dy0 * v[0]);
                        v[7] = S0;
                    } else if constexpr (PPL == 2) {
                        const float S0 = Q[0] + Q[1];
                        const float t = dx0 * S0;
                        v[0] = fmaf(-8.0f, Q[1], t); v[1] = dy0 * S0;
                        v[4] = fmaf(dx0, fmaf(-16.0f, Q[1], t), 64.0f * Q[1]);
                        v[5] = dy0 * v[0]; v[6] = dy0 * v[1];
                        v[7] = S0;
                    } else {
                        const float qdx = Q[0] * dx0, qdy = Q[0] * dy0;
                        v[0] = qdx; v[1] = qdy; v[4] = qdx * dx0; v[5] = qdx * dy0; v[6] = qdy * dy0; v[7] = Q[0];
                    }
                    v[2] = aX; v[3] = aY;
                    v[8] = vR; v[9] = vG; v[10] = vB; v[11] = vNx; v[12] = vNy; v[13] = vNz; v[14] = vD; v[15] = 0.f;
                    const float tot = wave_transpose_reduce16(v, lane);
                    const uint32_t id = __float_as_uint(q0.w);
                    if (col >= 0) {
                        if (p.slab) p.slab[((size_t)(r0 + k) * (p.slab_ipt ? p.slab_ipt : IPT) + (size_t)sub) * GACC_FLOATS + col] = tot;
                        else atomicAdd(p.gacc + (size_t)id * GACC_FLOATS + col, tot);
                    }
                }
            }
        };
        if (bg0) { if (stable) chunk(std::true_type{}, std::true_type{}); else chunk(std::false_type{}, std::true_type{}); }
        else { if (stable) chunk(std::true_type{}, std::false_type{}); else chunk(std::false_type{}, std::false_type{}); }
        __syncthreads();
        top -= count;
    }
}

#ifdef IBGS_TRACE_WAVES
__device__ uint4 g_trace_bwd[IBGS_TRACE_MAX];
#endif
__global__ void __launch_bounds__(64, 8) render_bwd_color_kernel(BwdParams p)
{
    IBGS_TRACE_BEGIN();
    int tile, sub = 0;
    bool have;
    if (p.order) { const uint32_t t = p.order[blockIdx.x]; tile = (int)(t & ~ORDER_SPLIT_BIT); have = t != 0xFFFFFFFFu; }
    else have = tile_map_item(p.tmap, blockIdx.x, p.cam.gx, p.cam.gy, 1, tile, sub);
    __shared__ float4 s_rec[3][BWD_CHUNK];
    __shared__ __align__(16) unsigned char s_pix[4 * WAVE * sizeof(float4)];
    if (have && !tile_is_risky(p.tile_risky, tile)) render_bwd_color_body<4, true, false, true>(p, tile, sub, s_rec, reinterpret_cast<float4 (*)[WAVE]>(s_pix));
    IBGS_TRACE_END(g_trace_bwd);
}
__global__ void __launch_bounds__(64, 8) render_bwd_color_noabs_kernel(BwdParams p)
{
    int tile, sub = 0;
    bool have;
    if (p.order) { const uint32_t t = p.order[blockIdx.x]; tile = (int)(t & ~ORDER_SPLIT_BIT); have = t != 0xFFFFFFFFu; }
    else have = tile_map_item(p.tmap, blockIdx.x, p.cam.gx, p.cam.gy, 1, tile, sub);
    __shared__ float4 s_rec[3][BWD_CHUNK];
    __shared__ __align__(16) unsigned char s_pix[4 * WAVE * sizeof(float4)];
    if (have && !tile_is_risky(p.tile_risky, tile)) render_bwd_color_body<4, false, false, true>(p, tile, sub, s_rec, reinterpret_cast<float4 (*)[WAVE]>(s_pix));
}
template <bool ABS>
__global__ void __launch_bounds__(64, 4) render_bwd_color_risk_kernel(BwdParams p)
{
    __shared__ float4 s_rec[3][BWD_CHUNK];
    __shared__ float4 s_gpix[4][WAVE];
    int tile = (int)blockIdx.x;
    if (p.order) { const uint32_t t = p.order[blockIdx.x]; if (t == 0xFFFFFFFFu) return; tile = (int)(t & ~ORDER_SPLIT_BIT); }
    if (tile >= p.ntiles || !tile_is_risky(p.tile_risky, tile)) return;
    render_bwd_color_body<4, ABS, true>(p, tile, 0, s_rec, s_gpix);
}

constexpr int ORDER_SNAKE_ROUNDS = 8;
__global__ void __launch_bounds__(1024) tile_order_kernel(int ntiles, int nslots , int slot_rounds ,
                                                          const uint32_t* __restrict__ walked_waves, const uint32_t* __restrict__ meta, uint32_t* __restrict__ order,
                                                          uint32_t* __restrict__ order_out ,
                                                          int theta_pct = 0 )
{
    __shared__ uint32_t s_hist[1024];
    __shared__ uint32_t s_w[16];
    __shared__ uint32_t s_max;
    __shared__ unsigned long long s_total;
    const int tid = threadIdx.x, lane = tid & 63, wave = tid >> 6;
    const uint32_t ipt = meta[10];
    if (ipt != 1u && ipt != 2u && ipt != 4u) {
        for (int i = tid; i < nslots; i += 1024) { const uint32_t v = i < ntiles ? ((uint32_t)i | (theta_pct > 0 ? ORDER_SPLIT_BIT : 0u)) : 0xFFFFFFFFu; order[i] = v; if (order_out) order_out[i] = v; }
        return;
    }
    auto walked_of = [&](int t) { uint32_t v = walked_waves[(size_t)t * ipt]; for (uint32_t k = 1; k < ipt; k++) v = max(v, walked_waves[(size_t)t * ipt + k]); return v; };
    s_hist[tid] = 0u;
    if (tid == 0) { s_max = 0u; s_total = 0ull; }
    for (int i = tid; i < nslots; i += 1024) { order[i] = 0xFFFFFFFFu; if (order_out) order_out[i] = 0xFFFFFFFFu; }
    __syncthreads();
    constexpr int KEEP = 16;
    uint32_t w[KEEP];
    uint32_t m = 0;
    unsigned long long sum = 0ull;
#pragma unroll
    for (int k = 0; k < KEEP; k++) { const int t = tid + k * 1024; w[k] = t < ntiles ? walked_of(t) : 0u; m = max(m, w[k]); sum += w[k]; }
    for (int t = tid + KEEP * 1024; t < ntiles; t += 1024) { const uint32_t v = walked_of(t); m = max(m, v); sum += v; }
    for (int d = 32; d >= 1; d >>= 1) m = max(m, (uint32_t)__shfl_xor((int)m, d, 64));
    if (lane == 0) atomicMax(&s_max, m);
    if (theta_pct > 0) {
        for (int d = 32; d >= 1; d >>= 1) sum += __shfl_xor(sum, d, 64);
        if (lane == 0) atomicAdd(&s_total, sum);
    }
    __syncthreads();
    const uint32_t mx = s_max;
    const unsigned long long total = s_total;
    const int sh = mx >= 1024u ? (32 - __builtin_clz(mx)) - 10 : 0;
    auto bucket = [&](uint32_t v) { return 1023u - min(v >> sh, 1023u); };
#pragma unroll
    for (int k = 0; k < KEEP; k++) if (tid + k * 1024 < ntiles) atomicAdd(&s_hist[bucket(w[k])], 1u);
    for (int t = tid + KEEP * 1024; t < ntiles; t += 1024) atomicAdd(&s_hist[bucket(walked_of(t))], 1u);
    __syncthreads();
    const uint32_t v = s_hist[tid];
    uint32_t inc = v;
    for (int d = 1; d < 64; d <<= 1) { const uint32_t o = (uint32_t)__shfl_up((int)inc, d, 64); if (lane >= d) inc += o; }
    if (lane == 63) s_w[wave] = inc;
    __syncthreads();
    uint32_t before = 0;
    for (int ww = 0; ww < wave; ww++) before += s_w[ww];
    s_hist[tid] = before + inc - v;
    __syncthreads();
    const uint32_t nrounds = (uint32_t)nslots / (uint32_t)ORDER_CLASSES;
    auto put = [&](int t, uint32_t key) {
        const uint32_t r = atomicAdd(&s_hist[bucket(key)], 1u);
        const uint32_t stratum = r / ORDER_CLASSES, c = r % ORDER_CLASSES;
        uint32_t slot = r;
        if (nrounds <= (uint32_t)slot_rounds) {
            const uint32_t round = (stratum + 1u) % nrounds;
            slot = round * ORDER_CLASSES + ((stratum & 1u) ? ORDER_CLASSES - 1u - c : c);
        }
        const uint32_t word = (uint32_t)t | ((theta_pct > 0 && hybrid_split(key, total, (uint32_t)theta_pct)) ? ORDER_SPLIT_BIT : 0u);
        order[slot] = word;
        if (order_out) order_out[slot] = word;
    };
#pragma unroll
    for (int k = 0; k < KEEP; k++) if (tid + k * 1024 < ntiles) put(tid + k * 1024, w[k]);
    for (int t = tid + KEEP * 1024; t < ntiles; t += 1024) put(t, walked_of(t));
}
__global__ void __launch_bounds__(64, 8) render_bwd_color_small_kernel(BwdParams p)
{
    int tile, sub;
    __shared__ float4 s_rec[3][BWD_CHUNK];
    __shared__ float4 s_gpix[1][WAVE];
    if (tile_map_item(p.tmap, blockIdx.x, p.cam.gx, p.cam.gy, 4, tile, sub) && !tile_is_risky(p.tile_risky, tile)) render_bwd_color_body<1>(p, tile, sub, s_rec, s_gpix);
}
template <bool ABS>
__global__ void __launch_bounds__(64, 8) render_bwd_color_hybrid_kernel(BwdParams p)
{
    __shared__ float4 s_rec[3][BWD_CHUNK];
    __shared__ float4 s_gpix[4][WAVE];
    int tile, sub; bool split;
    if (!hybrid_item(blockIdx.x, p.hybrid_grid1, p.order, tile, sub, split) || tile_is_risky(p.tile_risky, tile)) return;
    if (split) render_bwd_color_body<1, ABS>(p, tile, sub, s_rec, s_gpix);
    else if (sub == 0) render_bwd_color_body<4, ABS>(p, tile, 0, s_rec, s_gpix);
}
template <int PPL, bool ABS>
__device__ __forceinline__ void render_bwd_geo_entry(const BwdParams& p)
{
    __shared__ float4 s_rec[4][BWD_CHUNK];
    __shared__ float4 s_gpix[PPL][WAVE];
    __shared__ float4 s_gnrm[PPL][WAVE];
    int tile, sub;
    if (PPL == 4 && p.order) { const uint32_t t = p.order[blockIdx.x]; if (t == 0xFFFFFFFFu) return; tile = (int)(t & ~ORDER_SPLIT_BIT); sub = 0; }
    else if (!tile_map_item(p.tmap, blockIdx.x, p.cam.gx, p.cam.gy, 4 / PPL, tile, sub)) return;
    if (tile_is_risky(p.tile_risky, tile)) return;
    render_bwd_geo_body<PPL, ABS>(p, tile, sub, s_rec, s_gpix, s_gnrm);
}
template <bool ABS>
__global__ void __launch_bounds__(64, 3) render_bwd_geo_risk_kernel(BwdParams p)
{
    __shared__ float4 s_rec[4][BWD_CHUNK];
    __shared__ float4 s_gpix[4][WAVE];
    __shared__ float4 s_gnrm[4][WAVE];
    int tile = (int)blockIdx.x;
    if (p.order) { const uint32_t t = p.order[blockIdx.x]; if (t == 0xFFFFFFFFu) return; tile = (int)(t & ~ORDER_SPLIT_BIT); }
    if (tile >= p.ntiles || !tile_is_risky(p.tile_risky, tile)) return;
    render_bwd_geo_body<4, ABS, true>(p, tile, 0, s_rec, s_gpix, s_gnrm);
}
__global__ void __launch_bounds__(64, 4) render_bwd_geo4_kernel(BwdParams p) { render_bwd_geo_entry<4, true>(p); }
__global__ void __launch_bounds__(64, 4) render_bwd_geo4_noabs_kernel(BwdParams p) { render_bwd_geo_entry<4, false>(p); }
__global__ void __launch_bounds__(64, 6) render_bwd_geo_kernel(BwdParams p) { render_bwd_geo_entry<1, true>(p); }
template <bool ABS>
__global__ void __launch_bounds__(64, 4) render_bwd_geo_hybrid_kernel(BwdParams p)
{
    __shared__ float4 s_rec[4][BWD_CHUNK];
    __shared__ float4 s_gpix[4][WAVE];
    __shared__ float4 s_gnrm[4][WAVE];
    int tile, sub; bool split;
    if (!hybrid_item(blockIdx.x, p.hybrid_grid1, p.order, tile, sub, split) || tile_is_risky(p.tile_risky, tile)) return;
    if (split) render_bwd_geo_body<1, ABS>(p, tile, sub, s_rec, s_gpix, s_gnrm);
    else if (sub == 0) render_bwd_geo_body<4, ABS>(p, tile, 0, s_rec, s_gpix, s_gnrm);
}

int render_backward_ref_arith(uint32_t flags)
{
    if (flags & IBGS_FLAG_NO_REF_POWER_SKIP) return 0;
    return RA_DECIDE | ((flags & IBGS_FLAG_REF_ARITH) ? RA_ASSOC : RA_LFORM);
}

int render_backward_waves_per_tile(const ibgs_backward_args& a)
{
    const int nt = ((a.W + TILE - 1) / TILE) * ((a.H + TILE - 1) / TILE);
    if (a.render_geo) return ((a.flags & IBGS_FLAG_QUADRANT_WAVES) ? false : ((a.flags & IBGS_FLAG_TILE_WAVES) ? true : nt >= 4096)) ? 1 : 4;
    return ((a.flags & IBGS_FLAG_QUADRANT_WAVES) ? true : ((a.flags & IBGS_FLAG_TILE_WAVES) ? false : nt < hybrid_max_tiles())) ? 4 : 1;
}

int launch_render_backward(hipStream_t s, const ibgs_backward_args& a, const GeomState& g, const BinState& b,
                           const ImgState& im, const float4* src_rgba, float* slab, float* geo_tab)
{
    BwdParams p;
    p.ranges = im.ranges; p.point_list = b.point_list; p.rec = reinterpret_cast<const float4*>(g.rec);
    p.cam = make_cam(a.viewmatrix, a.projmatrix, a.campos, a.bg, a.tanfovx, a.tanfovy, a.W, a.H);
    p.ntiles = p.cam.gx * p.cam.gy;
    p.n_src = a.n_src; p.tex_quant = (a.flags & IBGS_FLAG_TEX_QUANT) ? 1 : 0;
    p.power_skip = render_backward_ref_arith(a.flags);
    p.tile_risky = (p.power_skip & RA_ASSOC) ? im.tile_risky : nullptr;
    p.ref_to_src = a.ref_to_src; p.src_rgba = src_rgba;
    p.final_T = im.final_T; p.n_contrib = im.n_contrib; p.sum_w = im.sum_w; p.low_high = im.low_high;
    p.valid_idx = im.valid_idx; p.valid_w = im.valid_w;
    p.depth_pixels = a.out_depth; p.warped_pixels = a.out_warped;
    p.dL_dcolor = a.dL_dcolor; p.dL_dnormal = a.dL_dnormal; p.dL_ddepth = a.dL_ddepth; p.dL_dwarped = a.dL_dwarped;
    p.gacc = a.grad_acc; p.slab = slab; p.order = nullptr; p.slab_ipt = 0; p.hybrid_grid1 = 0;
    p.slot_c = im.slot_c; p.meta = im.meta; p.tab = geo_tab;
    p.tab_slots = (a.buffer_length >= 1 && a.buffer_length < IBGS_MAX_BUFFER_LENGTH) ? a.buffer_length + 1 : IBGS_MAX_BUFFER_LENGTH;
    const int nt = p.ntiles;
    p.tmap = a.render_geo ? TileMap{TMAP_BLOCK, 1, 8, 4} : TileMap{TMAP_BLOCK, 1, 8, 8};
    auto grid = [&](int ipt) { return dim3((unsigned)tile_map_grid(p.tmap, p.cam.gx, p.cam.gy, ipt)); };
    auto launch_risk = [&](int nslots_or_0) {
        if (!p.tile_risky) return;
        BwdParams r = p;
        r.slab_ipt = render_backward_waves_per_tile(a);
        r.hybrid_grid1 = 0;
        if (nslots_or_0 == 0) r.order = nullptr;
        const dim3 g((unsigned)(nslots_or_0 ? nslots_or_0 : nt));
        StageTimer t(s, IBGS_STAGE_RENDER_BWD);
        const bool noabs = (a.flags & IBGS_FLAG_NO_ABS_GRAD) != 0;
        if (a.render_geo) { if (noabs) hipLaunchKernelGGL(render_bwd_geo_risk_kernel<false>, g, dim3(64), 0, s, r); else hipLaunchKernelGGL(render_bwd_geo_risk_kernel<true>, g, dim3(64), 0, s, r); }
        else { if (noabs) hipLaunchKernelGGL(render_bwd_color_risk_kernel<false>, g, dim3(64), 0, s, r); else hipLaunchKernelGGL(render_bwd_color_risk_kernel<true>, g, dim3(64), 0, s, r); }
    };
    const bool noabs = (a.flags & IBGS_FLAG_NO_ABS_GRAD) != 0;
    const int nslots = (nt + ORDER_CLASSES - 1) / ORDER_CLASSES * ORDER_CLASSES;
    auto launch_order = [&](int slot_rounds, int theta) {
        StageTimer t(s, IBGS_STAGE_TILE_ORDER);
        hipLaunchKernelGGL(tile_order_kernel, dim3(1), dim3(1024), 0, s, nt, nslots, slot_rounds, im.tile_walked, im.meta, im.tile_order, a.tile_order_out, theta);
        p.order = im.tile_order;
    };
    int risk_slots = 0;
    if (a.render_geo) {
        const bool big = (a.flags & IBGS_FLAG_QUADRANT_WAVES) ? false : ((a.flags & IBGS_FLAG_TILE_WAVES) ? true : nt >= 4096);
        const bool window = a.dL_ddepth || a.dL_dwarped;
        if (window && !geo_tab) { set_error("geo backward needs the window table scratch"); return -IBGS_ERR_INVALID; }
        if (window) {
            StageTimer t(s, IBGS_STAGE_GEO_WINDOW);
            hipLaunchKernelGGL(geo_window_kernel, dim3((unsigned)(((size_t)a.W * a.H + 255) / 256)), dim3(256), 0, s, p);
        } else p.tab = nullptr;
        IBGS_HIP(hipGetLastError());
        if (big) {
            launch_order(4, 0);
            risk_slots = nslots;
            StageTimer t(s, IBGS_STAGE_RENDER_BWD);
            if (noabs) hipLaunchKernelGGL(render_bwd_geo4_noabs_kernel, dim3((unsigned)nslots), dim3(64), 0, s, p);
            else hipLaunchKernelGGL(render_bwd_geo4_kernel, dim3((unsigned)nslots), dim3(64), 0, s, p);
        } else if (!(a.flags & IBGS_FLAG_QUADRANT_WAVES) && nt >= HYBRID_MIN_TILES) {
            launch_order(4, hybrid_theta());
            IBGS_HIP(hipGetLastError());
            p.slab_ipt = 4; p.hybrid_grid1 = nslots;
            risk_slots = nslots;
            StageTimer t(s, IBGS_STAGE_RENDER_BWD);
            if (noabs) hipLaunchKernelGGL(render_bwd_geo_hybrid_kernel<false>, dim3(4u * (unsigned)nslots), dim3(64), 0, s, p);
            else hipLaunchKernelGGL(render_bwd_geo_hybrid_kernel<true>, dim3(4u * (unsigned)nslots), dim3(64), 0, s, p);
        } else {
            StageTimer t(s, IBGS_STAGE_RENDER_BWD);
            hipLaunchKernelGGL(render_bwd_geo_kernel, grid(4), dim3(64), 0, s, p);
        }
    } else if ((a.flags & IBGS_FLAG_QUADRANT_WAVES) ? true : ((a.flags & IBGS_FLAG_TILE_WAVES) ? false : nt < hybrid_max_tiles())) {
        if (!(a.flags & IBGS_FLAG_QUADRANT_WAVES) && nt >= HYBRID_MIN_TILES) {
            launch_order(ORDER_SNAKE_ROUNDS, hybrid_theta());
            IBGS_HIP(hipGetLastError());
            p.slab_ipt = 4; p.hybrid_grid1 = nslots;
            risk_slots = nslots;
            StageTimer t(s, IBGS_STAGE_RENDER_BWD);
            if (noabs) hipLaunchKernelGGL(render_bwd_color_hybrid_kernel<false>, dim3(4u * (unsigned)nslots), dim3(64), 0, s, p);
            else hipLaunchKernelGGL(render_bwd_color_hybrid_kernel<true>, dim3(4u * (unsigned)nslots), dim3(64), 0, s, p);
        } else {
            StageTimer t(s, IBGS_STAGE_RENDER_BWD);
            hipLaunchKernelGGL(render_bwd_color_small_kernel, grid(4), dim3(64), 0, s, p);
        }
    } else {
        launch_order(ORDER_SNAKE_ROUNDS, 0);
        IBGS_HIP(hipGetLastError());
        risk_slots = nslots;
        StageTimer t(s, IBGS_STAGE_RENDER_BWD);
        if (noabs) hipLaunchKernelGGL(render_bwd_color_noabs_kernel, dim3((unsigned)nslots), dim3(64), 0, s, p);
        else hipLaunchKernelGGL(render_bwd_color_kernel, dim3((unsigned)nslots), dim3(64), 0, s, p);
    }
    IBGS_HIP(hipGetLastError());
    launch_risk(risk_slots);
    IBGS_HIP(hipGetLastError());
    return 0;
}

}

#ifdef IBGS_COUNT_LANES
extern "C" int ibgs_debug_lanes_bwd(unsigned long long* dst, int reset)
{
    int rc = (int)hipMemcpyFromSymbol(dst, HIP_SYMBOL(ibgs::g_lanes_bwd), sizeof(unsigned long long) * 4, 0, hipMemcpyDeviceToHost);
    if (reset) { unsigned long long z[4] = {0, 0, 0, 0}; rc |= (int)hipMemcpyToSymbol(HIP_SYMBOL(ibgs::g_lanes_bwd), z, sizeof(z), 0, hipMemcpyHostToDevice); }
    return rc;
}
#endif
#ifdef IBGS_TRACE_WAVES
extern "C" int ibgs_debug_trace_bwd(void* dst, size_t bytes)
{
    return (int)hipMemcpyFromSymbol(dst, HIP_SYMBOL(ibgs::g_trace_bwd), bytes < sizeof(uint4) * ibgs::IBGS_TRACE_MAX ? bytes : sizeof(uint4) * ibgs::IBGS_TRACE_MAX, 0, hipMemcpyDeviceToHost);
}
#endif
```

ibgs_amd/rasterizer.py:

```python
import collections
import weakref
import ctypes
import os
import threading
from typing import NamedTuple, Optional

import torch
import torch.nn as nn

from . import _lib

NUM_CHANNELS = 3
NUM_NORMAL_CHANNELS = 3
NUM_PLANE_PARAMS = 5
M_SRC = _lib.MAX_SRC

TEX_QUANT = False
TILE_CULL = True

REF_POWER_SKIP = True
REF_ARITH = False

KEEP_DET_SCRATCH = False
DETERMINISTIC = False
# ... 125 lines not shown


def _tex_slot(device, nbytes, slot):
    pool = _tex_pool.get(_stream_key(device))
    if pool is None:
        if len(_tex_pool) > 8:
            _tex_pool.clear()
        pool = _tex_pool[_stream_key(device)] = collections.OrderedDict()
    buf = pool.get(slot)
    if buf is None or buf.numel() < nbytes:
        buf = pool[slot] = torch.empty(nbytes, dtype=torch.uint8, device=device)
    pool.move_to_end(slot)
    total = sum(x.numel() for x in pool.values())
    cap = _cache_cap(device, TEX_CACHE_BYTES, 16 << 30, 0.05)
    while total > cap and len(pool) > 1:
        k0 = next(iter(pool))
        if k0 == slot:
            break
        total -= pool.pop(k0).numel()
    return buf


def _tex_packed(device, nbytes, source=None):
    cacheable = TEX_CACHE and source is not None and source[1] is not None and not getattr(source[0], "_ibgs_transient", False)
    slot = ("src", id(source[0])) if cacheable else "scratch"
    buf = _tex_slot(device, nbytes, slot)
    _tex_writes[0] += 1
    buf._ibgs_ticket = _tex_writes[0]
    buf._ibgs_src = (weakref.ref(source[0]),) + tuple(source[1:]) if cacheable else None
    return buf, (_stream_key(device), slot, _tex_writes[0], nbytes)


def _tensor_version(t):
    try:
        return t._version
    except (RuntimeError, AttributeError):
        return None


def clear_caches():
    _tex_pool.clear(); _tex_scratch.clear(); _gacc_scratch.clear(); _order_hints.clear(); _last_rendered.clear(); _cache_caps.clear()


def invalidate_tex_cache():
    for pool in _tex_pool.values():
        for buf in pool.values():
            buf._ibgs_src = None


def _tex_cached(device, nbytes, source):
    if not TEX_CACHE or source[1] is None:
        return None
    pool = _tex_pool.get(_stream_key(device))
    slot = ("src", id(source[0]))
    buf = pool.get(slot) if pool is not None else None
    had = getattr(buf, "_ibgs_src", None) if buf is not None else None
    if had is None or buf.numel() < nbytes or had[0]() is not source[0] or had[1:] != tuple(source[1:]):
        return None
    pool.move_to_end(slot)
    return buf, (_stream_key(device), slot, buf._ibgs_ticket, nbytes)


def _tex_still(ticket, device, nbytes):
    if ticket is None:
        return None
    skey, slot, serial, had = ticket
    pool = _tex_pool.get(skey)
    buf = pool.get(slot) if pool is not None else None
    if buf is None or skey != _stream_key(device) or had < nbytes or getattr(buf, "_ibgs_ticket", None) != serial:
        return None
    return buf


def _gacc(device, P):
    key = _stream_key(device) + (P,)
    ent = _gacc_scratch.get(key)
    if ent is None:
        if len(_gacc_scratch) > 8:
            _gacc_scratch.clear()
        ent = [torch.zeros(P, 16, dtype=torch.float32, device=device), False]
        _gacc_scratch[key] = ent
    elif ent[1]:
        ent[0].zero_()
    ent[1] = True
    return ent


_zero_scalar = {}


class _CallState(threading.local):

    def __init__(self):
        self.fwd = _lib.ForwardArgs()
        self.bwd = _lib.BackwardArgs()
        self.holder = {}
        self.alloc_device = None

        def _alloc(nbytes, _user):
            try:
                self.holder["t"] = torch.empty(int(nbytes), dtype=torch.uint8, device=self.alloc_device)
                return self.holder["t"].data_ptr()
            except Exception as ex:
                self.holder["err"] = ex
                return 0

        self.cb = _lib.ALLOC_FN(_alloc)

    def forward_args(self, device):
        ctypes.memset(ctypes.byref(self.fwd), 0, ctypes.sizeof(self.fwd))
        self.holder.clear()
        self.alloc_device = device
        return self.fwd, self.holder, self.cb

    def backward_args(self):
        ctypes.memset(ctypes.byref(self.bwd), 0, ctypes.sizeof(self.bwd))
        return self.bwd


_call_state = _CallState()


class _on_device:

    def __init__(self, device):
        idx = device.index
        self.ctx = None if (idx is None or idx == torch.cuda.current_device()) else torch.cuda.device(device)

    def __enter__(self):
        if self.ctx is not None:
            self.ctx.__enter__()

    def __exit__(self, *exc):
        if self.ctx is not None:
            return self.ctx.__exit__(*exc)
        return False


def _zeros_view(shape, device, dtype=torch.float32):
    key = (device.index if device.index is not None else torch.cuda.current_device(), dtype)
    z = _zero_scalar.get(key)
    if z is None:
        z = torch.zeros(1, dtype=dtype, device=device)
        _zero_scalar[key] = z
    return z.expand(*shape)


def _zero_plane(c, H, W, device, dtype=torch.float32):
    return _zeros_view((c, H, W), device, dtype)


class _CModule:
    last_tex = None

    @staticmethod
    def rasterize_gaussians(background, means3D, colors, opacity, scales, rotations, scale_modifier,
                            cov3D_precomp, all_map, viewmatrix, projmatrix, ref_to_src_list, src_cam_pos,
                            src_images, src_rendered_depths, nb_src_images, buffer_length,
                            depth_error_threshold, tan_fovx, tan_fovy, image_height, image_width, sh, degree,
                            campos, prefiltered, render_geo, render_depth_only, debug, plane=None, sh_rest=None, depth_slots=None):
        lib = _lib.load()
        if means3D.ndimension() != 2 or means3D.size(1) != 3:
            raise RuntimeError("means3D must have dimensions (num_points, 3)")
        if not means3D.is_cuda:
            raise RuntimeError("means3D must live on a HIP device (libibgs_rast.so has no CPU path)")
        device = means3D.device
        P = int(means3D.size(0)); H = int(image_height); W = int(image_width)
        render_geo = bool(render_geo); render_depth_only = bool(render_depth_only)

        with _on_device(device):
            stream = torch.cuda.current_stream(device).cuda_stream
            means3D_c = _dev_f32(means3D, device)
            sh_c = _dev_f32(sh, device); colors_c = _dev_f32(colors, device)
            sh_rest_c = _dev_f32(sh_rest, device) if sh_rest is not None else None
            opacity_c = _dev_f32(opacity, device)
            scales_c = _dev_f32(scales, device); rot_c = _dev_f32(rotations, device)
            cov_c = _dev_f32(cov3D_precomp, device); all_map_c = _dev_f32(all_map, device)
            bg_c = _dev_f32(background, device); vm_c = _dev_f32(viewmatrix, device); pm_c = _dev_f32(projmatrix, device)
            campos_c = _dev_f32(campos, device)
            r2s_c = _dev_f32(ref_to_src_list, device); scp_c = _dev_f32(src_cam_pos, device)
            simg_c = _dev_f32(src_images, device); sdep_c = _dev_f32(src_rendered_depths, device)

            radii = torch.empty(P, dtype=torch.int32, device=device)
            write_color = not render_depth_only
            if write_color:
                out_color = (torch.empty if P != 0 else torch.zeros)(NUM_CHANNELS, H, W, dtype=torch.float32, device=device)
            else:
                out_color = _zero_plane(NUM_CHANNELS, H, W, device)
            if render_geo:
                mk = (lambda *shp, **kw: torch.empty(*shp, device=device, **kw)) if P != 0 else (lambda *shp, **kw: torch.zeros(*shp, device=device, **kw))
                out_normal = mk(NUM_NORMAL_CHANNELS, H, W)
                out_depth = mk(1, H, W)
                out_cam_feat = mk(4 * M_SRC, H, W)
                out_warped = mk(3 * M_SRC, H, W)
                out_min_depth_diff = mk(1, H, W)
                out_camera_ray = mk(3, H, W)
                out_mask = mk(1, H, W, dtype=torch.int32)
            else:
                out_normal = _zero_plane(NUM_NORMAL_CHANNELS, H, W, device)
                if render_depth_only:
                    out_depth = (torch.empty if P != 0 else torch.zeros)(1, H, W, dtype=torch.float32, device=device)
                else:
                    out_depth = _zero_plane(1, H, W, device)
                out_cam_feat = _zero_plane(4 * M_SRC, H, W, device)
                out_warped = _zero_plane(3 * M_SRC, H, W, device)
                out_min_depth_diff = _zero_plane(1, H, W, device)
                out_camera_ray = _zero_plane(3, H, W, device)
                out_mask = _zero_plane(1, H, W, device, torch.int32)

            geomBuffer = torch.empty(0, dtype=torch.uint8, device=device)
            binningBuffer = torch.empty(0, dtype=torch.uint8, device=device)
            imgBuffer = torch.empty(0, dtype=torch.uint8, device=device)
            rendered = 0
            if P != 0:
                M = 0 if sh_c is None else int(sh_c.size(1)) + (int(sh_rest_c.size(1)) if sh_rest_c is not None else 0)
                geomBuffer = torch.empty(lib.ibgs_required_geom(P), dtype=torch.uint8, device=device)
                imgBuffer = torch.empty(lib.ibgs_required_img(W, H), dtype=torch.uint8, device=device)
                a, holder, cb = _call_state.forward_args(device)
                a.stream = stream
                a.P, a.D, a.M, a.W, a.H = P, int(degree), M, W, H
                a.means3D = _ptr(means3D_c); a.shs = _ptr(sh_c); a.colors_precomp = _ptr(colors_c); a.shs_rest = _ptr(sh_rest_c)
                a.opacities = _ptr(opacity_c); a.scales = _ptr(scales_c); a.rotations = _ptr(rot_c)
                a.cov3D_precomp = _ptr(cov_c); a.all_map = _ptr(all_map_c)
                if plane is not None and plane[2]:
                    pn_c, po_c = _dev_f32(plane[0], device), _dev_f32(plane[1], device)
                    a.plane_normal = _ptr(pn_c); a.plane_offset = _ptr(po_c); a.plane_mode = int(plane[2]); a.all_map = None
                a.scale_modifier = float(scale_modifier)
                a.bg = _ptr(bg_c); a.viewmatrix = _ptr(vm_c); a.projmatrix = _ptr(pm_c); a.campos = _ptr(campos_c)
                a.tanfovx = float(tan_fovx); a.tanfovy = float(tan_fovy)
                a.n_src = int(nb_src_images)
                a.ref_to_src = _ptr(r2s_c); a.src_cam_pos = _ptr(scp_c); a.src_images = _ptr(simg_c); a.src_depths = _ptr(sdep_c)
                a.buffer_length = int(buffer_length); a.depth_error_threshold = float(depth_error_threshold)
                a.prefiltered = int(bool(prefiltered)); a.render_geo = int(render_geo); a.render_depth_only = int(render_depth_only)
                tex_flag = 0
                a.geom = geomBuffer.data_ptr(); a.geom_bytes = geomBuffer.numel()
                a.img = imgBuffer.data_ptr(); a.img_bytes = imgBuffer.numel()
                a.binning_alloc = cb; a.binning_user = None
                if render_geo:
                    if simg_c is None or simg_c.numel() < int(nb_src_images) * 3 * H * W:
                        raise RuntimeError("src_images must hold nb_src_images x 3 x H x W values")
                    if depth_slots is not None:
                        slots = [int(x) for x in depth_slots]
                        if len(slots) < int(nb_src_images) or min(slots[:int(nb_src_images)]) < 0:
                            raise RuntimeError("depth_slots must name one non-negative plane per source")
                        if sdep_c is None or sdep_c.numel() < (max(slots[:int(nb_src_images)]) + 1) * H * W:
                            raise RuntimeError("src_rendered_depths (a table of planes) does not hold plane %d" % max(slots[:int(nb_src_images)]))
                        for m_ in range(M_SRC):
                            a.src_depth_slot[m_] = slots[m_] if m_ < int(nb_src_images) else 0
                    elif sdep_c is None or sdep_c.numel() < int(nb_src_images) * H * W:
                        raise RuntimeError("src_rendered_depths must hold nb_src_images x 1 x H x W values")
                    nbytes = lib.ibgs_required_tex(int(nb_src_images), W, H)
                    source = (src_images, _tensor_version(src_images), int(nb_src_images), W, H)
                    hit = _tex_cached(device, nbytes, source)
                    if hit is not None:
                        tex, _CModule.last_tex = hit
                        tex_flag = _lib.FLAG_TEX_PACKED
                    else:
                        tex, _CModule.last_tex = _tex_packed(device, nbytes, source)
                    a.tex = tex.data_ptr(); a.tex_bytes = tex.numel()
                a.flags = ((_lib.FLAG_DEBUG if debug else 0) | (_lib.FLAG_TEX_QUANT if TEX_QUANT else 0)
                           | (0 if TILE_CULL else _lib.FLAG_NO_TILE_CULL) | _shape_flag() | tex_flag
                           | (_lib.FLAG_SRC_DEPTH_SLOTS if (render_geo and depth_slots is not None) else 0))
                a.out_color = out_color.data_ptr() if write_color else None
                a.radii = radii.data_ptr()
                if render_geo:
                    a.out_normal = out_normal.data_ptr(); a.out_depth = out_depth.data_ptr()
                    a.out_cam_feat = out_cam_feat.data_ptr(); a.out_warped = out_warped.data_ptr()
                    a.out_min_depth_diff = out_min_depth_diff.data_ptr(); a.out_camera_ray = out_camera_ray.data_ptr()
                    a.out_mask = out_mask.data_ptr()
                elif render_depth_only:
                    a.out_depth = out_depth.data_ptr()
                if ORDER_HINT and (ORDER_HINT_GEO or not render_geo) and not render_depth_only and not debug:
                    ckey = _camera_key(viewmatrix, device, W, H, render_geo, stream)
                    oh = _order_hints.get(ckey)
                    if oh is not None:
                        _order_hints.move_to_end(ckey)
                        a.tile_order_hint = oh.data_ptr()
                hkey = (device.index, P, W, H, render_geo, render_depth_only)
                hist = _last_rendered.get(hkey) if (RENDERED_HINT and not debug) else None
                prev = (max(hist) if isinstance(hist, list) else int(hist)) if hist else 0
                a.rendered_hint = (prev + prev // 4 + 4096) if prev > 0 else 0
                pre = None
                if prev > 0:
                    pre = torch.empty(lib.ibgs_required_binning(int(a.rendered_hint), W, H), dtype=torch.uint8, device=device)
                    a.binning = pre.data_ptr(); a.binning_bytes = pre.numel()
                rc = lib.ibgs_forward(ctypes.byref(a))
                if rc < 0:
                    if "err" in holder:
                        raise holder["err"]
                    raise RuntimeError("ibgs_forward failed (%d): %s" % (rc, _lib.last_error()))
                rendered = int(rc)
                if pre is not None and "t" not in holder:
                    binningBuffer = pre
                if len(_last_rendered) > 64:
                    _last_rendered.clear()
                hist = _last_rendered.get(hkey)
                hist = (hist if isinstance(hist, list) else ([int(hist)] if hist else [])) + [rendered]
                _last_rendered[hkey] = hist[-RENDERED_WINDOW:]
                global LAST_BINNING_CAPACITY, LAST_NUM_RENDERED, HINT_MISSES
                if a.rendered_hint and rendered > int(a.rendered_hint):
                    HINT_MISSES += 1
                LAST_NUM_RENDERED = rendered
                LAST_BINNING_CAPACITY = max(rendered, int(a.rendered_hint)) if a.rendered_hint else rendered
                binningBuffer = holder.get("t", binningBuffer)
        return (rendered, out_color, radii, out_normal, out_depth, out_cam_feat, out_warped, out_min_depth_diff,
                out_camera_ray, out_mask, geomBuffer, binningBuffer, imgBuffer)

    @staticmethod
    def rasterize_gaussians_backward(background, normal_map_pixels, intersected_depth_pixels, warped_image_pixels,
                                     means3D, radii, colors, all_maps, scales, rotations, scale_modifier,
                                     cov3D_precomp, viewmatrix, projmatrix, ref_to_src_list, src_cam_pos,
                                     src_images, src_rendered_depths, nb_src_images, tan_fovx, tan_fovy,
                                     dL_dout_color, dL_dout_normal_map, dL_dout_median_intersected_depth,
                                     dL_dout_warped_image, sh, degree, campos, geomBuffer, R, binningBuffer,
                                     imageBuffer, render_geo, debug, plane=None, packed_tex=None, skip_unused=False, buffer_length=0, want_abs=True, sh_rest=None):
        lib = _lib.load()
        device = means3D.device
        P = int(means3D.size(0))
        H = int(normal_map_pixels.size(1)); W = int(normal_map_pixels.size(2))
        render_geo = bool(render_geo)
        with _on_device(device):
            stream = torch.cuda.current_stream(device).cuda_stream
            sh_c = _dev_f32(sh, device)
            sh_rest_c = _dev_f32(sh_rest, device) if sh_rest is not None else None
            M_dc = int(sh.size(1)) if sh.dim() == 3 else 0
            M = M_dc + (int(sh_rest.size(1)) if sh_rest is not None else 0)
            opts = dict(dtype=torch.float32, device=device)
            have_sr = scales is not None and scales.numel() != 0
            new = torch.empty if P != 0 else torch.zeros
            dL_dmeans3D = _sink_or_new("means3D", (P, 3), new, opts) if P != 0 else new(P, 3, **opts); dL_dmeans2D = new(P, 3, **opts)
            dL_dmeans2D_abs = new(P, 3, **opts) if want_abs else None
            fused = plane is not None and bool(plane[2])
            dL_dall_map = new(P, NUM_PLANE_PARAMS, **opts) if (render_geo and all_maps.numel() != 0 and P != 0 and not fused) else _zeros_view((P, NUM_PLANE_PARAMS), device)
            dL_dplane_normal = dL_dplane_offset = None
            if fused:
                learnt = int(plane[2]) == _lib.PLANE_LEARNT
                want = render_geo and P != 0
                dL_dplane_normal = (new(P, 3, **opts) if want else _zeros_view((P, 3), device)) if (learnt and plane[0] is not None) else None
                dL_dplane_offset = (new(P, 1, **opts) if want else _zeros_view((P, 1), device)) if (learnt and plane[1] is not None) else None
            dL_dopacity = _sink_or_new("opacities", (P, 1), new, opts) if P != 0 else new(P, 1, **opts)
            factored = _sh_factor_sink is not None and M != 0 and P != 0
            want_colors = not skip_unused or factored or M == 0 or (colors is not None and colors.numel() != 0)
            want_cov = not skip_unused or not have_sr
            dL_dcolors = new(P, NUM_CHANNELS, **opts) if want_colors else _zeros_view((P, NUM_CHANNELS), device)
            dL_dcov3D = new(P, 6, **opts) if want_cov else _zeros_view((P, 6), device)
            dL_dsh = None if factored else new(P, M_dc, 3, **opts)
            dL_dsh_rest = None if (factored or sh_rest is None) else new(P, M - M_dc, 3, **opts)
            dL_dscales = _sink_or_new("scales", (P, 3), new, opts) if (have_sr and P != 0) else _zeros_view((P, 3), device)
            dL_drotations = _sink_or_new("rotations", (P, 4), new, opts) if (have_sr and P != 0) else _zeros_view((P, 4), device)
            if P != 0:
                means3D_c = _dev_f32(means3D, device); colors_c = _dev_f32(colors, device)
                scales_c = _dev_f32(scales, device); rot_c = _dev_f32(rotations, device)
                cov_c = _dev_f32(cov3D_precomp, device); all_map_c = _dev_f32(all_maps, device)
                bg_c = _dev_f32(background, device); vm_c = _dev_f32(viewmatrix, device); pm_c = _dev_f32(projmatrix, device)
                campos_c = _dev_f32(campos, device)
                r2s_c = _dev_f32(ref_to_src_list, device); scp_c = _dev_f32(src_cam_pos, device)
                simg_c = _dev_f32(src_images, device); sdep_c = _dev_f32(src_rendered_depths, device)
                g_color = _dev_f32(dL_dout_color, device)
                g_normal = _dev_f32(dL_dout_normal_map, device) if render_geo else None
                g_depth = _dev_f32(dL_dout_median_intersected_depth, device) if render_geo else None
                g_warp = _dev_f32(dL_dout_warped_image, device) if render_geo else None
                depth_c = _dev_f32(intersected_depth_pixels, device) if render_geo else None
                warped_c = _dev_f32(warped_image_pixels, device) if render_geo else None
                gacc_ent = _gacc(device, P)
                grad_acc = gacc_ent[0]
                radii_c = radii.contiguous()
                a = _call_state.backward_args()
                a.stream = stream
                a.P, a.D, a.M, a.W, a.H = P, int(degree), M, W, H
                a.R = int(R)
                a.means3D = _ptr(means3D_c); a.shs = _ptr(sh_c); a.colors_precomp = _ptr(colors_c); a.shs_rest = _ptr(sh_rest_c)
                a.scales = _ptr(scales_c); a.rotations = _ptr(rot_c); a.cov3D_precomp = _ptr(cov_c); a.all_map = _ptr(all_map_c)
                a.scale_modifier = float(scale_modifier)
                a.bg = _ptr(bg_c); a.viewmatrix = _ptr(vm_c); a.projmatrix = _ptr(pm_c); a.campos = _ptr(campos_c)
                a.tanfovx = float(tan_fovx); a.tanfovy = float(tan_fovy)
                a.n_src = int(nb_src_images)
                a.ref_to_src = _ptr(r2s_c); a.src_cam_pos = _ptr(scp_c); a.src_images = _ptr(simg_c); a.src_depths = _ptr(sdep_c)
                a.radii = radii_c.data_ptr()
                a.out_depth = _ptr(depth_c); a.out_warped = _ptr(warped_c)
                a.geom = geomBuffer.data_ptr(); a.binning = binningBuffer.data_ptr() if binningBuffer.numel() else None
                a.img = imageBuffer.data_ptr()
                tex_flag = 0
                if render_geo:
                    nbytes = lib.ibgs_required_tex(int(nb_src_images), W, H)
                    tex = _tex_still(packed_tex, device, nbytes)
                    if tex is not None:
                        tex_flag = _lib.FLAG_TEX_PACKED
                    else:
                        tex, _ = _tex_packed(device, nbytes)
                    a.tex = tex.data_ptr(); a.tex_bytes = tex.numel()
                    a.buffer_length = int(buffer_length)
                    tab = _tex(device, lib.ibgs_required_geo_table_for(W, H, int(buffer_length)), "geo_table")
                    a.geo_table = tab.data_ptr(); a.geo_table_bytes = tab.numel()
                a.dL_dcolor = _ptr(g_color); a.dL_dnormal = _ptr(g_normal); a.dL_ddepth = _ptr(g_depth); a.dL_dwarped = _ptr(g_warp)
                a.grad_acc = grad_acc.data_ptr()
                a.dL_dmean2D = dL_dmeans2D.data_ptr(); a.dL_dmean2D_abs = dL_dmeans2D_abs.data_ptr() if want_abs else None
                a.dL_dconic = None
                a.dL_dopacity = dL_dopacity.data_ptr(); a.dL_dcolors = dL_dcolors.data_ptr() if want_colors else None
                a.dL_dmean3D = dL_dmeans3D.data_ptr(); a.dL_dcov3D = dL_dcov3D.data_ptr() if want_cov else None
                a.dL_dsh = dL_dsh.data_ptr() if (M and not factored) else None
                a.dL_dsh_rest = dL_dsh_rest.data_ptr() if dL_dsh_rest is not None else None
                a.dL_dscale = dL_dscales.data_ptr() if have_sr else None; a.dL_drot = dL_drotations.data_ptr() if have_sr else None
                a.dL_dall_map = dL_dall_map.data_ptr() if (render_geo and all_maps.numel() != 0 and not fused) else None
                if fused and render_geo:
                    pn_c, po_c = _dev_f32(plane[0], device), _dev_f32(plane[1], device)
                    a.plane_normal = _ptr(pn_c); a.plane_offset = _ptr(po_c); a.plane_mode = int(plane[2]); a.all_map = None
                    a.dL_dplane_normal = _ptr(dL_dplane_normal); a.dL_dplane_offset = _ptr(dL_dplane_offset)
                a.render_geo = int(render_geo)
                a.flags = ((_lib.FLAG_DEBUG if debug else 0) | (_lib.FLAG_TEX_QUANT if TEX_QUANT else 0)
                           | _lib.FLAG_CLEAR_GRAD_ACC | (_lib.FLAG_SH_FACTORED if factored else 0) | _shape_flag() | tex_flag
                           | (0 if want_abs else _lib.FLAG_NO_ABS_GRAD))
                if DETERMINISTIC and int(R) > 0:
                    det = torch.empty(lib.ibgs_required_deterministic_for(int(R), P, W, H, int(render_geo), int(a.flags)), dtype=torch.uint8, device=device)
                    if KEEP_DET_SCRATCH:
                        _CModule.last_det = det
                    a.det_scratch = det.data_ptr(); a.det_scratch_bytes = det.numel()
                    a.flags |= _lib.FLAG_DETERMINISTIC
                if ORDER_HINT and (ORDER_HINT_GEO or not render_geo) and not debug:
                    ckey = _camera_key(viewmatrix, device, W, H, render_geo, stream)
                    if ckey is not None:
                        oh = _order_hints.get(ckey)
                        if oh is None:
                            while len(_order_hints) >= ORDER_HINT_MAX:
                                _order_hints.popitem(last=False)
                            oh = _order_hints[ckey] = torch.full((int(lib.ibgs_tile_order_slots(W, H)),), -1, dtype=torch.int32, device=device)
                        else:
                            _order_hints.move_to_end(ckey)
                        a.tile_order_out = oh.data_ptr()
                rc = lib.ibgs_backward(ctypes.byref(a))
                if rc < 0:
                    raise RuntimeError("ibgs_backward failed (%d): %s" % (rc, _lib.last_error()))
                gacc_ent[1] = False
                if factored:
                    _sh_factor_sink.append({"dcolor": dL_dcolors, "campos": campos_c.reshape(3), "degree": int(degree), "M": M})
        res = (dL_dmeans2D, dL_dmeans2D_abs, dL_dcolors, dL_dopacity, dL_dmeans3D, dL_dcov3D, dL_dsh,
               dL_dscales, dL_drotations, dL_dall_map)
        if plane is not None or sh_rest is not None:
            res = res + (dL_dplane_normal, dL_dplane_offset)
            if sh_rest is not None:
                res = res + (dL_dsh_rest,)
        return res

    @staticmethod
    def mark_visible(means3D, viewmatrix, projmatrix):
        lib = _lib.load()
        device = means3D.device
        P = int(means3D.size(0))
        present = torch.zeros(P, dtype=torch.bool, device=device)
        if P != 0:
            with torch.cuda.device(device):
                m = _dev_f32(means3D, device); vm = _dev_f32(viewmatrix, device); pm = _dev_f32(projmatrix, device)
                rc = lib.ibgs_mark_visible(torch.cuda.current_stream(device).cuda_stream, P, m.data_ptr(),
                                           vm.data_ptr(), _ptr(pm), present.data_ptr())
                if rc < 0:
                    raise RuntimeError("ibgs_mark_visible failed (%d): %s" % (rc, _lib.last_error()))
        return present


_C = _CModule()


def check_async_errors(device=None, wait=True):
    device = torch.device("cuda", torch.cuda.current_device()) if device is None else torch.device(device)
    with torch.cuda.device(device):
        rc = _lib.load().ibgs_check_async(torch.cuda.current_stream(device).cuda_stream, 1 if wait else 0)
    if rc < 0:
        raise RuntimeError("ibgs_check_async failed (%d): %s" % (rc, _lib.last_error()))


def rasterize_gaussians(means3D, means2D, means2D_abs, sh, colors_precomp, opacities, scales, rotations,
                        cov3Ds_precomp, all_map, raster_settings, plane_normal=None, plane_offset=None, plane_mode=0, sh_rest=None):
    return _RasterizeGaussians.apply(means3D, means2D, means2D_abs, sh, colors_precomp, opacities, scales,
                                     rotations, cov3Ds_precomp, all_map, raster_settings, plane_normal, plane_offset, plane_mode, sh_rest)


def rasterize_depth_batch(means3D, opacities, scales, rotations, cov3D_precomp, scale_modifier, viewmatrices, projmatrices,
                          camposes, tanfovxs, tanfovys, image_height, image_width, buffer_length, plane_normal=None,
                          plane_offset=None, plane_mode=2, debug=False):
    lib = _lib.load()
    device = means3D.device
    if not means3D.is_cuda:
        raise RuntimeError("means3D must live on a HIP device (libibgs_rast.so has no CPU path)")
    n = int(viewmatrices.shape[0])
    if not (1 <= n <= _lib.MAX_VIEWS):
        raise RuntimeError("rasterize_depth_batch: 1..%d views per call" % _lib.MAX_VIEWS)
    if not plane_mode:
        raise RuntimeError("rasterize_depth_batch needs plane_mode 1 (learnt normal) or 2 (smallest axis)")
    P, H, W = int(means3D.size(0)), int(image_height), int(image_width)
    with torch.cuda.device(device), torch.no_grad():
        depths = (torch.empty if P else torch.zeros)(n, 1, H, W, dtype=torch.float32, device=device)
        radii = (torch.empty if P else torch.zeros)(n, P, dtype=torch.int32, device=device)
        if P == 0:
            return depths, radii
        m_c = _dev_f32(means3D, device); o_c = _dev_f32(opacities, device)
        s_c = _dev_f32(scales, device); r_c = _dev_f32(rotations, device); cov_c = _dev_f32(cov3D_precomp, device)
        vm_c = _dev_f32(viewmatrices.reshape(n, 16), device); pm_c = _dev_f32(projmatrices.reshape(n, 16), device)
        cp_c = _dev_f32(camposes.reshape(n, 3), device)
        pn_c = _dev_f32(plane_normal, device); po_c = _dev_f32(plane_offset, device)
        bg_c = _zeros_view((3,), device).contiguous()
        gy = (H + 15) // 16
        geom = torch.empty(lib.ibgs_required_geom(n * P), dtype=torch.uint8, device=device)
        img = torch.empty(lib.ibgs_required_img(W, n * 16 * gy if n > 1 else H), dtype=torch.uint8, device=device)
        holder = {}

        def _alloc(nbytes, _user):
            try:
                holder["t"] = torch.empty(int(nbytes), dtype=torch.uint8, device=device)
                return holder["t"].data_ptr()
            except Exception as ex:
                holder["err"] = ex
                return 0

        cb = _lib.ALLOC_FN(_alloc)
        a = _lib.ForwardArgs()
        a.stream = torch.cuda.current_stream(device).cuda_stream
        a.P, a.D, a.M, a.W, a.H = P, 0, 0, W, H
        a.means3D = _ptr(m_c); a.opacities = _ptr(o_c); a.scales = _ptr(s_c); a.rotations = _ptr(r_c); a.cov3D_precomp = _ptr(cov_c)
        a.scale_modifier = float(scale_modifier)
        a.bg = _ptr(bg_c); a.viewmatrix = _ptr(vm_c); a.projmatrix = _ptr(pm_c); a.campos = _ptr(cp_c)
        a.tanfovx = float(tanfovxs[0]); a.tanfovy = float(tanfovys[0])
        a.n_src = 1; a.buffer_length = int(buffer_length); a.depth_error_threshold = 0.0
        a.render_geo = 0; a.render_depth_only = 1
        a.flags = (_lib.FLAG_DEBUG if debug else 0) | (0 if TILE_CULL else _lib.FLAG_NO_TILE_CULL) | (0 if REF_POWER_SKIP else _lib.FLAG_NO_REF_POWER_SKIP)
        a.geom = geom.data_ptr(); a.geom_bytes = geom.numel(); a.img = img.data_ptr(); a.img_bytes = img.numel()
        a.binning_alloc = cb; a.binning_user = None
        a.radii = radii.data_ptr(); a.out_depth = depths.data_ptr()
        a.plane_normal = _ptr(pn_c); a.plane_offset = _ptr(po_c); a.plane_mode = int(plane_mode)
        a.n_views = n if n > 1 else 0
        for v in range(n):
            a.view_tanfovx[v] = float(tanfovxs[v]); a.view_tanfovy[v] = float(tanfovys[v])
        hkey = (device.index, P, W, H, "depth_batch", n)
        hist = _last_rendered.get(hkey) if (RENDERED_HINT and not debug) else None
        prev = max(hist) if hist else 0
        a.rendered_hint = (prev + prev // 4 + 4096) if prev > 0 else 0
        rc = lib.ibgs_forward(ctypes.byref(a))
        if rc < 0:
            if "err" in holder:
                raise holder["err"]
            raise RuntimeError("ibgs_forward (depth batch) failed (%d): %s" % (rc, _lib.last_error()))
        _last_rendered[hkey] = ((hist or []) + [int(rc)])[-RENDERED_WINDOW:]
    return depths, radii


_EMPTY = torch.Tensor([])


class _RasterizeGaussians(torch.autograd.Function):
    @staticmethod
    def forward(ctx, means3D, means2D, means2D_abs, sh, colors_precomp, opacities, scales, rotations,
                cov3Ds_precomp, all_maps, raster_settings, plane_normal=None, plane_offset=None, plane_mode=0, sh_rest=None):
        plane = (plane_normal, plane_offset, int(plane_mode)) if plane_mode else None
        kw = {"plane": plane} if plane is not None else {}
        if sh_rest is not None:
            kw["sh_rest"] = sh_rest
        if raster_settings.render_geo and getattr(raster_settings, "src_depth_slots", None) is not None:
            kw["depth_slots"] = raster_settings.src_depth_slots
        args = (
            raster_settings.bg, means3D, colors_precomp, opacities, scales, rotations,
            raster_settings.scale_modifier, cov3Ds_precomp, all_maps,
            raster_settings.viewmatrix, raster_settings.projmatrix,
            raster_settings.ref_to_src_list, raster_settings.src_cam_pos, raster_settings.src_images,
            raster_settings.src_rendered_depths, raster_settings.nb_src_images,
            raster_settings.buffer_length, raster_settings.depth_error_threshold,
            raster_settings.tanfovx, raster_settings.tanfovy,
            raster_settings.image_height, raster_settings.image_width,
            sh, raster_settings.sh_degree, raster_settings.campos, raster_settings.prefiltered,
            raster_settings.render_geo, raster_settings.render_depth_only, raster_settings.debug,
        )
        if raster_settings.debug:
            cpu_args = cpu_deep_copy_tuple(args)
            try:
                res = _C.rasterize_gaussians(*args, **kw)
            except Exception as ex:
                torch.save(cpu_args, "snapshot_fw.dump")
                print("\nAn error occured in forward. Please forward snapshot_fw.dump for debugging.")
                raise ex
        else:
            res = _C.rasterize_gaussians(*args, **kw)
        (num_rendered, color, radii, out_normal_map, out_median_intersected_depth, out_cam_feat, out_warped_image,
         out_min_depth_diff, out_camera_ray, out_use_first_src_frame, geomBuffer, binningBuffer, imgBuffer) = res

        ctx.raster_settings = raster_settings
        ctx.packed_tex, _CModule.last_tex = _CModule.last_tex, None
        ctx.plane_mode = int(plane_mode) if plane is not None else 0
        ctx.num_rendered = num_rendered
        ctx.set_materialize_grads(False)
        none = _EMPTY
        ctx.save_for_backward(out_normal_map, out_median_intersected_depth, out_warped_image, colors_precomp,
                              all_maps, means3D, scales, rotations, cov3Ds_precomp, radii, sh,
                              plane_normal if plane_normal is not None else none, plane_offset if plane_offset is not None else none,
                              sh_rest if sh_rest is not None else none,
                              geomBuffer, binningBuffer, imgBuffer)
        ctx.has_sh_rest = sh_rest is not None
        ctx.mark_non_differentiable(radii, out_use_first_src_frame)
        return (color, radii, out_normal_map, out_median_intersected_depth, out_cam_feat, out_warped_image,
                out_min_depth_diff, out_camera_ray, out_use_first_src_frame)

    @staticmethod
    def backward(ctx, grad_out_color, grad_radii, grad_out_normal_map, grad_out_median_intersected_depth,
                 grad_out_cam_feat, grad_out_warped_image, grad_out_min_depth_diff, grad_out_camera_ray,
                 grad_out_use_first_src_frame):
        num_rendered = ctx.num_rendered
        raster_settings = ctx.raster_settings
        (normal_map_pixels, median_intersected_depth_pixels, warped_image_pixels, colors_precomp, all_maps, means3D,
         scales, rotations, cov3Ds_precomp, radii, sh, plane_normal, plane_offset, sh_rest, geomBuffer, binningBuffer, imgBuffer) = ctx.saved_tensors
        kw = {}
        if ctx.has_sh_rest:
            kw["sh_rest"] = sh_rest
        if ctx.plane_mode:
            kw["plane"] = (plane_normal if plane_normal.numel() else None, plane_offset if plane_offset.numel() else None, ctx.plane_mode)
        if getattr(ctx, "packed_tex", None) is not None:
            kw["packed_tex"] = ctx.packed_tex
        kw["skip_unused"] = True
        kw["buffer_length"] = int(raster_settings.buffer_length)
        kw["want_abs"] = bool(ctx.needs_input_grad[2]) or not NO_ABS_GRAD_WHEN_UNUSED

        args = (raster_settings.bg, normal_map_pixels, median_intersected_depth_pixels, warped_image_pixels,
                means3D, radii, colors_precomp, all_maps, scales, rotations, raster_settings.scale_modifier,
                cov3Ds_precomp, raster_settings.viewmatrix, raster_settings.projmatrix,
                raster_settings.ref_to_src_list, raster_settings.src_cam_pos, raster_settings.src_images,
                raster_settings.src_rendered_depths, raster_settings.nb_src_images,
                raster_settings.tanfovx, raster_settings.tanfovy,
                grad_out_color, grad_out_normal_map, grad_out_median_intersected_depth, grad_out_warped_image,
                sh, raster_settings.sh_degree, raster_settings.campos, geomBuffer, num_rendered, binningBuffer,
                imgBuffer, raster_settings.render_geo, raster_settings.debug)
        if raster_settings.debug:
            cpu_args = cpu_deep_copy_tuple(args)
            try:
                res = _C.rasterize_gaussians_backward(*args, **kw)
            except Exception as ex:
                torch.save(cpu_args, "snapshot_bw.dump")
                print("\nAn error occured in backward. Writing snapshot_bw.dump for debugging.\n")
                raise ex
        else:
            res = _C.rasterize_gaussians_backward(*args, **kw)
        (grad_means2D, grad_means2D_abs, grad_colors_precomp, grad_opacities, grad_means3D, grad_cov3Ds_precomp,
         grad_sh, grad_scales, grad_rotations, grad_all_map) = res[:10]
        grad_plane_normal, grad_plane_offset = (res[10], res[11]) if ctx.plane_mode else (None, None)
        grad_sh_rest = res[12] if ctx.has_sh_rest else None
        return (grad_means3D, grad_means2D, grad_means2D_abs, grad_sh, grad_colors_precomp, grad_opacities,
                grad_scales, grad_rotations, grad_cov3Ds_precomp, grad_all_map, None, grad_plane_normal, grad_plane_offset, None, grad_sh_rest)


class GaussianRasterizationSettings(NamedTuple):
    image_height: int
    image_width: int
    tanfovx: float
    tanfovy: float
    bg: torch.Tensor
    scale_modifier: float
    viewmatrix: torch.Tensor
    projmatrix: torch.Tensor
    ref_to_src_list: torch.Tensor
    src_cam_pos: torch.Tensor
    src_images: torch.Tensor
    src_rendered_depths: torch.Tensor
    nb_src_images: int
    buffer_length: int
    depth_error_threshold: float
    sh_degree: int
    campos: torch.Tensor
    prefiltered: bool
    render_geo: bool
    render_depth_only: bool
    debug: bool
    src_depth_slots: Optional[tuple] = None


class GaussianRasterizer(nn.Module):
    def __init__(self, raster_settings):
        super().__init__()
        self.raster_settings = raster_settings

    def markVisible(self, positions):
        with torch.no_grad():
            raster_settings = self.raster_settings
            visible = _C.mark_visible(positions, raster_settings.viewmatrix, raster_settings.projmatrix)
        return visible

    def forward(self, means3D, means2D, means2D_abs, opacities, shs=None, colors_precomp=None, scales=None,
                rotations=None, cov3D_precomp=None, all_map=None, plane_normal=None, plane_offset=None, plane_mode=0, shs_rest=None):
        if shs_rest is not None and (shs is None or shs.dim() != 3 or int(shs.shape[1]) != 1 or shs_rest.dim() != 3):
            raise Exception('shs_rest needs shs = the DC coefficients (P, 1, 3)')
        raster_settings = self.raster_settings
        if plane_mode and all_map is not None:
            raise Exception('Please provide either all_map or plane_mode, not both!')

        if (shs is None and colors_precomp is None) or (shs is not None and colors_precomp is not None):
            raise Exception('Please provide excatly one of either SHs or precomputed colors!')

        if ((scales is None or rotations is None) and cov3D_precomp is None) or \
                ((scales is not None or rotations is not None) and cov3D_precomp is not None):
            raise Exception('Please provide exactly one of either scale/rotation pair or precomputed 3D covariance!')

        if shs is None:
            shs = _EMPTY
        if colors_precomp is None:
            colors_precomp = _EMPTY
        if scales is None:
            scales = _EMPTY
        if rotations is None:
            rotations = _EMPTY
        if cov3D_precomp is None:
            cov3D_precomp = _EMPTY
        if all_map is None:
            all_map = _EMPTY

        return rasterize_gaussians(means3D, means2D, means2D_abs, shs, colors_precomp, opacities, scales,
                                   rotations, cov3D_precomp, all_map, raster_settings, plane_normal, plane_offset, plane_mode, shs_rest)
```

include/ibgs_rast.h:

```cpp
#ifndef IBGS_RAST_H
#define IBGS_RAST_H

#include <stddef.h>
#include <stdint.h>

#ifdef __cplusplus
extern "C" {
#endif

#define IBGS_MAX_SRC 5
#define IBGS_MAX_BUFFER_LENGTH 8
#define IBGS_MAX_VIEWS 8
#define IBGS_TILE 16

#define IBGS_ERR_INVALID 1
#define IBGS_ERR_HIP 2
#define IBGS_ERR_ALLOC 3

typedef char* (*ibgs_alloc_fn)(size_t bytes, void* user);

#define IBGS_FLAG_DEBUG 1u
#define IBGS_FLAG_TEX_QUANT 2u
#define IBGS_FLAG_CLEAR_GRAD_ACC 8u
#define IBGS_FLAG_NO_TILE_CULL 4u

#define IBGS_FLAG_TILE_WAVES 32u
#define IBGS_FLAG_QUADRANT_WAVES 64u

#define IBGS_PLANE_NONE 0
#define IBGS_PLANE_LEARNT 1
#define IBGS_PLANE_SMALLEST_AXIS 2

#define IBGS_FLAG_DETERMINISTIC 128u
#define IBGS_FLAG_TEX_PACKED 256u
#define IBGS_FLAG_SH_FACTORED 16u

#define IBGS_FLAG_NO_REF_POWER_SKIP 512u

#define IBGS_FLAG_REF_ARITH 4096u
#define IBGS_FLAG_SRC_DEPTH_SLOTS 8192u
#define IBGS_FLAG_NO_ABS_GRAD 1024u

typedef struct ibgs_forward_args {
    void* stream;
    int32_t P;
    int32_t D;
    int32_t M;
    int32_t W, H;
    const float* means3D;
    const float* shs;
    const float* colors_precomp;
    const float* opacities;
    const float* scales;
    const float* rotations;
    const float* cov3D_precomp;
    const float* all_map;
    float scale_modifier;
    const float* bg;
    const float* viewmatrix;
    const float* projmatrix;
    const float* campos;
    float tanfovx, tanfovy;
    int32_t n_src;
    const float* ref_to_src;
    const float* src_cam_pos;
    const float* src_images;
    const float* src_depths;
    int32_t buffer_length;
    float depth_error_threshold;
    int32_t prefiltered;
    int32_t render_geo;
    int32_t render_depth_only;
    uint32_t flags;
    char* geom;  size_t geom_bytes;
    char* img;   size_t img_bytes;
    ibgs_alloc_fn binning_alloc;
    void* binning_user;
    char* tex;   size_t tex_bytes;
    float* out_color;
    int32_t* radii;
    float* out_normal;
    float* out_depth;
    float* out_cam_feat;
    float* out_warped;
    float* out_min_depth_diff;
    float* out_camera_ray;
    int32_t* out_mask;
    int64_t rendered_hint;
    const float* plane_normal;
    const float* plane_offset;
    int32_t plane_mode;
    int32_t n_views;
    float view_tanfovx[8];
    float view_tanfovy[8];
    const uint32_t* tile_order_hint;
    char* binning; size_t binning_bytes;
    const float* shs_rest;
    int32_t src_depth_slot[IBGS_MAX_SRC];
} ibgs_forward_args;

typedef struct ibgs_backward_args {
    void* stream;
    int32_t P, D, M, W, H;
    int64_t R;
    const float* means3D;
    const float* shs;
    const float* colors_precomp;
    const float* scales;
    const float* rotations;
    const float* cov3D_precomp;
    const float* all_map;
    float scale_modifier;
    const float* bg;
    const float* viewmatrix;
    const float* projmatrix;
    const float* campos;
    float tanfovx, tanfovy;
    int32_t n_src;
    const float* ref_to_src;
    const float* src_cam_pos;
    const float* src_images;
    const float* src_depths;
    const int32_t* radii;
    const float* out_depth;
    const float* out_warped;
    char* geom; char* binning; char* img;
    char* tex; size_t tex_bytes;
    const float* dL_dcolor;
    const float* dL_dnormal;
    const float* dL_ddepth;
    const float* dL_dwarped;
    float* grad_acc;
    float* dL_dmean2D;
    float* dL_dmean2D_abs;
    float* dL_dconic;
    float* dL_dopacity;
    float* dL_dcolors;
    float* dL_dmean3D;
    float* dL_dcov3D;
    float* dL_dsh;
    float* dL_dscale;
    float* dL_drot;
    float* dL_dall_map;
    int32_t render_geo;
    uint32_t flags;
    const float* plane_normal;
    const float* plane_offset;
    int32_t plane_mode;
    float* dL_dplane_normal;
    float* dL_dplane_offset;
    char* geo_table; size_t geo_table_bytes;
    char* det_scratch; size_t det_scratch_bytes;
    int32_t buffer_length;
    uint32_t* tile_order_out;
    const float* shs_rest;
    float* dL_dsh_rest;
} ibgs_backward_args;

size_t ibgs_required_deterministic(int64_t R, int32_t P);
size_t ibgs_required_deterministic_for(int64_t R, int32_t P, int32_t W, int32_t H, int32_t render_geo, uint32_t flags);
size_t ibgs_required_geo_table(int32_t W, int32_t H);
size_t ibgs_required_geo_table_for(int32_t W, int32_t H, int32_t buffer_length);
size_t ibgs_required_geom(int32_t P);
size_t ibgs_required_img(int32_t W, int32_t H);
size_t ibgs_required_binning(int64_t R, int32_t W, int32_t H);
size_t ibgs_required_tex(int32_t n_src, int32_t W, int32_t H);

size_t ibgs_tile_order_slots(int32_t W, int32_t H);
int64_t ibgs_forward(const ibgs_forward_args* args);
void ibgs_last_forward_stats(int64_t* out3);
int32_t ibgs_check_async(void* stream, int32_t wait);
int32_t ibgs_backward(const ibgs_backward_args* args);
int32_t ibgs_mark_visible(void* stream, int32_t P, const float* means3D, const float* viewmatrix,
                          const float* projmatrix, uint8_t* present );

int32_t ibgs_sh_grad_from_views(void* stream, int32_t P, int32_t D, int32_t M, int32_t n_views, const float* means3D,
                                const float* camposes, const float* dcolor, int64_t view_stride, float* dL_dsh);

#define IBGS_ADAM_MAX_TENSORS 16
typedef struct ibgs_adam_tensor {
    float* param; const float* grad; float* exp_avg; float* exp_avg_sq;
    int64_t numel;
    double lr, beta1, beta2, eps;
    double bias_correction1, bias_correction2;
} ibgs_adam_tensor;
int32_t ibgs_adam_step(void* stream, int32_t n_tensors, const ibgs_adam_tensor* tensors);
int32_t ibgs_adam_step_sh(void* stream, int32_t P, int32_t D, int32_t n_views, const float* means3D, const float* camposes, const float* dcolor,
                          int64_t view_stride, int32_t n_tensors, const ibgs_adam_tensor* tensors, const int32_t* first_coeff, const int32_t* n_coeff);

size_t ibgs_required_l1(void);
int32_t ibgs_l1_loss(void* stream, int64_t n, const float* x, const float* y, float* grad, float* loss, char* scratch, size_t scratch_bytes);
int32_t ibgs_l1_grad(void* stream, int64_t n, const float* x, const float* y, const float* scale_dev, float* grad);
int32_t ibgs_l1_rescale(void* stream, int64_t n, float* grad, const float* scale_dev);

// ... 57 lines not shown
```

Measured before the change: 629.9.

## Fold backward tile-order kernel into render-bwd and preprocess-bwd as rider blocks

When the backward tile order output buffer is the same order hint used by the forward pass, the separate tile_order_kernel launch is removed. An extra block in the render backward grid computes the new walked-wave-sorted order into a scratch buffer, while the remaining blocks read the hint order. An extra block in preprocess backward then copies that order into the output buffer. This cuts kernel launches and serialization, but a single 64-thread block now does the histogram sort that used to run in a 1024-thread kernel, and that block could become a straggler.

Result: no change. 631.2 (median of 4 runs) (+0.2%).

```diff
diff --git a/ibgs_amd/_lib.py b/ibgs_amd/_lib.py
--- a/ibgs_amd/_lib.py
+++ b/ibgs_amd/_lib.py
@@ -19,6 +19,7 @@
 FLAG_NO_ABS_GRAD = 1024
 FLAG_REF_ARITH = 4096
 FLAG_SRC_DEPTH_SLOTS = 8192
+FLAG_ORDER_OUT_IS_HINT = 16384
 PLANE_NONE, PLANE_LEARNT, PLANE_SMALLEST_AXIS = 0, 1, 2
 MAX_VIEWS = 8
 
diff --git a/ibgs_amd/csrc/api.hip b/ibgs_amd/csrc/api.hip
--- a/ibgs_amd/csrc/api.hip
+++ b/ibgs_amd/csrc/api.hip
@@ -275,6 +275,7 @@
 }
 void ibgs_debug_set_lookback_spins(uint32_t v) { radix_set_lookback_spins(v); }
 void ibgs_debug_set_sh_ride(int32_t on) { radix_set_sh_ride(on != 0); }
+void ibgs_debug_set_bwd_riders(int32_t on) { render_backward_set_riders(on); }
 size_t ibgs_debug_scan_scratch_elems(size_t n) { return scan_scratch_elems(n); }
 int32_t ibgs_debug_scan_u32(void* stream, const uint32_t* in, uint32_t* out, size_t n, uint32_t* scratch, size_t scratch_elems, int32_t with_total)
 {
@@ -509,6 +510,7 @@
         rgba = t;
         geo_tab = reinterpret_cast<float*>((reinterpret_cast<uintptr_t>(a.geo_table) + 127) & ~uintptr_t(127));
     }
+    BwdRideDone ride;
     if (a.R > 0) {
         const bool det = (a.flags & IBGS_FLAG_DETERMINISTIC) != 0;
         DetState ds{};
@@ -519,11 +521,11 @@
             ds = DetState::carve(a.det_scratch, (size_t)a.R * ipt, (size_t)a.P, nullptr);
             if ((rc = launch_det_prepare(s, ds, (size_t)a.R * ipt))) return rc;
         }
-        if ((rc = launch_render_backward(s, a, g, b, im, rgba, det ? ds.slab : nullptr, geo_tab))) return rc;
+        if ((rc = launch_render_backward(s, a, g, b, im, rgba, det ? ds.slab : nullptr, geo_tab, &ride))) return rc;
         if (det) { StageTimer t(s, IBGS_STAGE_TILE_ORDER); if ((rc = launch_det_reduce(s, ds, b.point_list, (size_t)a.R, ipt, a.P, a.grad_acc, g.offsets + a.P))) return rc; }
         if ((rc = stage_check(s, debug, "render backward"))) return rc;
     }
-    { StageTimer t(s, IBGS_STAGE_PREPROCESS_BWD); if ((rc = launch_preprocess_backward(s, a, g))) return rc; }
+    { StageTimer t(s, IBGS_STAGE_PREPROCESS_BWD); if ((rc = launch_preprocess_backward(s, a, g, ride))) return rc; }
     if ((rc = stage_check(s, debug, "preprocess backward"))) return rc;
     return check_sort_flag(rs, true);
 }
diff --git a/ibgs_amd/csrc/common.h b/ibgs_amd/csrc/common.h
--- a/ibgs_amd/csrc/common.h
+++ b/ibgs_amd/csrc/common.h
@@ -366,9 +366,11 @@
 inline size_t geo_table_floats(int W, int H) { return (size_t)W * H * IBGS_MAX_BUFFER_LENGTH * GEO_TAB_FIELDS; }
 int launch_render_forward(hipStream_t s, const ibgs_forward_args& a, const GeomState& g, const BinState& b,
                           const ImgState& im, const float4* src_rgba);
+struct BwdRideDone { const uint32_t* order_src = nullptr; uint32_t* order_dst = nullptr; int order_words = 0; };
 int launch_render_backward(hipStream_t s, const ibgs_backward_args& a, const GeomState& g, const BinState& b,
-                           const ImgState& im, const float4* src_rgba, float* slab = nullptr, float* geo_tab = nullptr);
-int launch_preprocess_backward(hipStream_t s, const ibgs_backward_args& a, const GeomState& g);
+                           const ImgState& im, const float4* src_rgba, float* slab = nullptr, float* geo_tab = nullptr, BwdRideDone* done = nullptr);
+int launch_preprocess_backward(hipStream_t s, const ibgs_backward_args& a, const GeomState& g, const BwdRideDone& done = BwdRideDone());
+void render_backward_set_riders(int on);
 
 struct DetState {
     float* slab;
diff --git a/ibgs_amd/csrc/preprocess_bwd.hip b/ibgs_amd/csrc/preprocess_bwd.hip
--- a/ibgs_amd/csrc/preprocess_bwd.hip
+++ b/ibgs_amd/csrc/preprocess_bwd.hip
@@ -24,6 +24,7 @@
     float* dL_dall_map; float* dL_dmean3D; float* dL_dcov3D; float* dL_dsh; float* dL_dsh_rest; float* dL_dscale; float* dL_drot;
     const float* plane_normal; const float* plane_offset; int plane_mode;
     float* dL_dplane_normal; float* dL_dplane_offset;
+    const uint32_t* order_src; uint32_t* order_dst; int order_words;
 };
 
 __device__ __forceinline__ int sh_basis(int D, float x, float y, float z, float (&B)[16])
@@ -52,7 +53,12 @@
 __global__ void __launch_bounds__(FAST16 ? 64 : 256) preprocess_bwd_kernel(PreBwdParams p, Cam cam)
 {
     __shared__ float4 s_t[FAST16 ? 64 * 13 : 1];
-    const int i = blockIdx.x * blockDim.x + threadIdx.x;
+    int blk = blockIdx.x;
+    if (p.order_dst) {
+        if (blk == 0) { for (int k = threadIdx.x; k < p.order_words; k += blockDim.x) p.order_dst[k] = p.order_src[k]; return; }
+        blk--;
+    }
+    const int i = blk * blockDim.x + threadIdx.x;
     const bool valid = i < p.P;
     bool vis = valid && (p.radii[i] > 0);
     float4 g0 = make_float4(0.f, 0.f, 0.f, 0.f), g1 = g0, g2 = g0, g3 = g0;
@@ -97,7 +103,7 @@
     if (FAST16 && SPLIT && p.shs) {
         const int lane = threadIdx.x;
         const uint64_t vism = __builtin_amdgcn_ballot_w64(vis);
-        const int i0 = blockIdx.x * 64;
+        const int i0 = blk * 64;
         const int nrows = min(64, p.P - i0);
         const float4* rest4 = reinterpret_cast<const float4*>(p.shs_rest + (size_t)i0 * 45);
         const float4* dc4 = reinterpret_cast<const float4*>(p.shs + (size_t)i0 * 3);
@@ -396,7 +402,7 @@
 #pragma unroll
         for (int k = 0; k < 45; k++) s_w[45 * lane + k] = gv[3 + k];
         __syncthreads();
-        const int i0 = blockIdx.x * 64;
+        const int i0 = blk * 64;
         const int nrows = min(64, p.P - i0);
         float4* dr = reinterpret_cast<float4*>(p.dL_dsh_rest + (size_t)i0 * 45);
         float4* dd = reinterpret_cast<float4*>(p.dL_dsh + (size_t)i0 * 3);
@@ -419,7 +425,7 @@
 #pragma unroll
         for (int v = 0; v < 12; v++) s_t[lane * 13 + v] = make_float4(gv[4 * v], gv[4 * v + 1], gv[4 * v + 2], gv[4 * v + 3]);
         __syncthreads();
-        const int i0 = blockIdx.x * 64;
+        const int i0 = blk * 64;
         const int nrows = min(64, p.P - i0);
         float4* dst = reinterpret_cast<float4*>(p.dL_dsh + (size_t)i0 * 48);
 #pragma unroll
@@ -431,7 +437,7 @@
     }
 }
 
-int launch_preprocess_backward(hipStream_t s, const ibgs_backward_args& a, const GeomState& g)
+int launch_preprocess_backward(hipStream_t s, const ibgs_backward_args& a, const GeomState& g, const BwdRideDone& done)
 {
     PreBwdParams p;
     p.P = a.P; p.D = a.D; p.M = a.M;
@@ -445,19 +451,21 @@
     p.dL_dmean3D = a.dL_dmean3D; p.dL_dcov3D = a.dL_dcov3D; p.dL_dsh = a.dL_dsh; p.dL_dsh_rest = a.dL_dsh_rest; p.dL_dscale = a.dL_dscale; p.dL_drot = a.dL_drot;
     p.plane_normal = a.plane_normal; p.plane_offset = a.plane_offset; p.plane_mode = a.plane_mode;
     p.dL_dplane_normal = a.dL_dplane_normal; p.dL_dplane_offset = a.dL_dplane_offset;
+    p.order_src = done.order_src; p.order_dst = done.order_src ? done.order_dst : nullptr; p.order_words = done.order_words;
+    const unsigned extra = p.order_dst ? 1u : 0u;
     const Cam cam = make_cam(a.viewmatrix, a.projmatrix, a.campos, a.bg, a.tanfovx, a.tanfovy, a.W, a.H);
     const bool factored = a.shs && (a.flags & IBGS_FLAG_SH_FACTORED);
     const bool split = a.shs && a.shs_rest;
     if (a.shs && a.M == 16) {
-        if (factored && split) hipLaunchKernelGGL((preprocess_bwd_kernel<true, false, true>), dim3((a.P + 63) / 64), dim3(64), 0, s, p, cam);
-        else if (factored) hipLaunchKernelGGL((preprocess_bwd_kernel<true, false>), dim3((a.P + 63) / 64), dim3(64), 0, s, p, cam);
-        else if (split) hipLaunchKernelGGL((preprocess_bwd_kernel<true, true, true>), dim3((a.P + 63) / 64), dim3(64), 0, s, p, cam);
-        else hipLaunchKernelGGL((preprocess_bwd_kernel<true, true>), dim3((a.P + 63) / 64), dim3(64), 0, s, p, cam);
+        if (factored && split) hipLaunchKernelGGL((preprocess_bwd_kernel<true, false, true>), dim3((a.P + 63) / 64 + extra), dim3(64), 0, s, p, cam);
+        else if (factored) hipLaunchKernelGGL((preprocess_bwd_kernel<true, false>), dim3((a.P + 63) / 64 + extra), dim3(64), 0, s, p, cam);
+        else if (split) hipLaunchKernelGGL((preprocess_bwd_kernel<true, true, true>), dim3((a.P + 63) / 64 + extra), dim3(64), 0, s, p, cam);
+        else hipLaunchKernelGGL((preprocess_bwd_kernel<true, true>), dim3((a.P + 63) / 64 + extra), dim3(64), 0, s, p, cam);
     } else {
-        if (factored && split) hipLaunchKernelGGL((preprocess_bwd_kernel<false, false, true>), dim3((a.P + 255) / 256), dim3(256), 0, s, p, cam);
-        else if (factored) hipLaunchKernelGGL((preprocess_bwd_kernel<false, false>), dim3((a.P + 255) / 256), dim3(256), 0, s, p, cam);
-        else if (split) hipLaunchKernelGGL((preprocess_bwd_kernel<false, true, true>), dim3((a.P + 255) / 256), dim3(256), 0, s, p, cam);
-        else hipLaunchKernelGGL((preprocess_bwd_kernel<false, true>), dim3((a.P + 255) / 256), dim3(256), 0, s, p, cam);
+        if (factored && split) hipLaunchKernelGGL((preprocess_bwd_kernel<false, false, true>), dim3((a.P + 255) / 256 + extra), dim3(256), 0, s, p, cam);
+        else if (factored) hipLaunchKernelGGL((preprocess_bwd_kernel<false, false>), dim3((a.P + 255) / 256 + extra), dim3(256), 0, s, p, cam);
+        else if (split) hipLaunchKernelGGL((preprocess_bwd_kernel<false, true, true>), dim3((a.P + 255) / 256 + extra), dim3(256), 0, s, p, cam);
+        else hipLaunchKernelGGL((preprocess_bwd_kernel<false, true>), dim3((a.P + 255) / 256 + extra), dim3(256), 0, s, p, cam);
     }
     IBGS_HIP(hipGetLastError());
     return 0;
diff --git a/ibgs_amd/csrc/render_bwd.hip b/ibgs_amd/csrc/render_bwd.hip
--- a/ibgs_amd/csrc/render_bwd.hip
+++ b/ibgs_amd/csrc/render_bwd.hip
@@ -697,27 +697,109 @@
 #ifdef IBGS_TRACE_WAVES
 __device__ uint4 g_trace_bwd[IBGS_TRACE_MAX];
 #endif
-__global__ void __launch_bounds__(64, 8) render_bwd_color_kernel(BwdParams p)
-{
-    IBGS_TRACE_BEGIN();
-    int tile, sub = 0;
-    bool have;
-    if (p.order) { const uint32_t t = p.order[blockIdx.x]; tile = (int)(t & ~ORDER_SPLIT_BIT); have = t != 0xFFFFFFFFu; }
-    else have = tile_map_item(p.tmap, blockIdx.x, p.cam.gx, p.cam.gy, 1, tile, sub);
+struct BwdRide {
+    int n_order;
+    int nslots;
+    const uint32_t* hint;
+    const uint32_t* walked; uint32_t* order_w;
+};
+constexpr int ORDER_SNAKE_ROUNDS = 8;
+__device__ __forceinline__ void order_rider(const BwdParams& p, const BwdRide& r, uint32_t* __restrict__ s_hist)
+{
+    const int lane = threadIdx.x, ntiles = p.ntiles, nslots = r.nslots;
+    uint32_t* __restrict__ order = r.order_w;
+    const uint32_t ipt = p.meta[10];
+    if (ipt != 1u && ipt != 2u && ipt != 4u) {
+        for (int i = lane; i < nslots; i += 64) order[i] = i < ntiles ? (uint32_t)i : 0xFFFFFFFFu;
+        return;
+    }
+    auto walked_of = [&](int t) { uint32_t v = r.walked[(size_t)t * ipt]; for (uint32_t k = 1; k < ipt; k++) v = max(v, r.walked[(size_t)t * ipt + k]); return v; };
+    for (int i = lane; i < 1024; i += 64) s_hist[i] = 0u;
+    for (int i = lane; i < nslots; i += 64) order[i] = 0xFFFFFFFFu;
+    uint32_t m = 0;
+    constexpr int B = 8;
+    for (int t0 = 0; t0 < ntiles; t0 += 64 * B) {
+        uint32_t w[B];
+#pragma unroll
+        for (int k = 0; k < B; k++) { const int t = t0 + k * 64 + lane; w[k] = t < ntiles ? walked_of(t) : 0u; }
+#pragma unroll
+        for (int k = 0; k < B; k++) m = max(m, w[k]);
+    }
+    for (int d = 32; d >= 1; d >>= 1) m = max(m, (uint32_t)__shfl_xor((int)m, d, 64));
+    __syncthreads();
+    const int sh = m >= 1024u ? (32 - __builtin_clz(m)) - 10 : 0;
+    auto bucket = [&](uint32_t v) { return 1023u - min(v >> sh, 1023u); };
+    for (int t0 = 0; t0 < ntiles; t0 += 64 * B) {
+        uint32_t w[B];
+#pragma unroll
+        for (int k = 0; k < B; k++) { const int t = t0 + k * 64 + lane; w[k] = t < ntiles ? walked_of(t) : 0u; }
+#pragma unroll
+        for (int k = 0; k < B; k++) if (t0 + k * 64 + lane < ntiles) atomicAdd(&s_hist[bucket(w[k])], 1u);
+    }
+    __syncthreads();
+    {
+        uint32_t sum = 0;
+        for (int k = 0; k < 16; k++) sum += s_hist[lane * 16 + k];
+        uint32_t inc = sum;
+        for (int d = 1; d < 64; d <<= 1) { const uint32_t o = (uint32_t)__shfl_up((int)inc, d, 64); if (lane >= d) inc += o; }
+        uint32_t run = inc - sum;
+        for (int k = 0; k < 16; k++) { const uint32_t v = s_hist[lane * 16 + k]; s_hist[lane * 16 + k] = run; run += v; }
+    }
+    __syncthreads();
+    const uint32_t nrounds = (uint32_t)nslots / (uint32_t)ORDER_CLASSES;
+    for (int t0 = 0; t0 < ntiles; t0 += 64 * B) {
+        uint32_t w[B];
+#pragma unroll
+        for (int k = 0; k < B; k++) { const int t = t0 + k * 64 + lane; w[k] = t < ntiles ? walked_of(t) : 0u; }
+#pragma unroll
+        for (int k = 0; k < B; k++) {
+            const int t = t0 + k * 64 + lane;
+            if (t >= ntiles) continue;
+            const uint32_t rk = atomicAdd(&s_hist[bucket(w[k])], 1u);
+            const uint32_t stratum = rk / ORDER_CLASSES, c = rk % ORDER_CLASSES;
+            uint32_t slot = rk;
+            if (nrounds <= (uint32_t)ORDER_SNAKE_ROUNDS) {
+                const uint32_t round = (stratum + 1u) % nrounds;
+                slot = round * ORDER_CLASSES + ((stratum & 1u) ? ORDER_CLASSES - 1u - c : c);
+            }
+            order[slot] = (uint32_t)t;
+        }
+    }
+}
+__device__ __forceinline__ bool tile_wave_item(const BwdParams& p, const uint32_t* __restrict__ hint, unsigned slot, int& tile)
+{
+    if (p.order) { const uint32_t t = p.order[slot]; tile = (int)(t & ~ORDER_SPLIT_BIT); return t != 0xFFFFFFFFu; }
+    if (p.meta[11] == 1u) { const uint32_t t = hint[slot]; tile = (int)(t & ~ORDER_SPLIT_BIT); return t != 0xFFFFFFFFu && tile < p.ntiles; }
+    tile = (int)slot;
+    return tile < p.ntiles;
+}
+__global__ void __launch_bounds__(64, 8) render_bwd_color_kernel(BwdParams p, BwdRide r)
+{
     __shared__ float4 s_rec[3][BWD_CHUNK];
     __shared__ __align__(16) unsigned char s_pix[4 * WAVE * sizeof(float4)];
-    if (have && !tile_is_risky(p.tile_risky, tile)) render_bwd_color_body<4, true, false, true>(p, tile, sub, s_rec, reinterpret_cast<float4 (*)[WAVE]>(s_pix));
+    unsigned slot = blockIdx.x;
+    if (r.n_order) {
+        if (slot == 0u) { order_rider(p, r, reinterpret_cast<uint32_t*>(s_pix)); return; }
+        if (slot == (unsigned)r.nslots) slot = 0u;
+    }
+    IBGS_TRACE_BEGIN();
+    int tile;
+    const bool have = tile_wave_item(p, r.hint, slot, tile);
+    if (have && !tile_is_risky(p.tile_risky, tile)) render_bwd_color_body<4, true, false, true>(p, tile, 0, s_rec, reinterpret_cast<float4 (*)[WAVE]>(s_pix));
     IBGS_TRACE_END(g_trace_bwd);
 }
-__global__ void __launch_bounds__(64, 8) render_bwd_color_noabs_kernel(BwdParams p)
-{
-    int tile, sub = 0;
-    bool have;
-    if (p.order) { const uint32_t t = p.order[blockIdx.x]; tile = (int)(t & ~ORDER_SPLIT_BIT); have = t != 0xFFFFFFFFu; }
-    else have = tile_map_item(p.tmap, blockIdx.x, p.cam.gx, p.cam.gy, 1, tile, sub);
+__global__ void __launch_bounds__(64, 8) render_bwd_color_noabs_kernel(BwdParams p, BwdRide r)
+{
     __shared__ float4 s_rec[3][BWD_CHUNK];
     __shared__ __align__(16) unsigned char s_pix[4 * WAVE * sizeof(float4)];
-    if (have && !tile_is_risky(p.tile_risky, tile)) render_bwd_color_body<4, false, false, true>(p, tile, sub, s_rec, reinterpret_cast<float4 (*)[WAVE]>(s_pix));
+    unsigned slot = blockIdx.x;
+    if (r.n_order) {
+        if (slot == 0u) { order_rider(p, r, reinterpret_cast<uint32_t*>(s_pix)); return; }
+        if (slot == (unsigned)r.nslots) slot = 0u;
+    }
+    int tile;
+    const bool have = tile_wave_item(p, r.hint, slot, tile);
+    if (have && !tile_is_risky(p.tile_risky, tile)) render_bwd_color_body<4, false, false, true>(p, tile, 0, s_rec, reinterpret_cast<float4 (*)[WAVE]>(s_pix));
 }
 template <bool ABS>
 __global__ void __launch_bounds__(64, 4) render_bwd_color_risk_kernel(BwdParams p)
@@ -730,7 +812,6 @@
     render_bwd_color_body<4, ABS, true>(p, tile, 0, s_rec, s_gpix);
 }
 
-constexpr int ORDER_SNAKE_ROUNDS = 8;
 __global__ void __launch_bounds__(1024) tile_order_kernel(int ntiles, int nslots , int slot_rounds ,
                                                           const uint32_t* __restrict__ walked_waves, const uint32_t* __restrict__ meta, uint32_t* __restrict__ order,
                                                           uint32_t* __restrict__ order_out ,
@@ -867,8 +948,11 @@
     return ((a.flags & IBGS_FLAG_QUADRANT_WAVES) ? true : ((a.flags & IBGS_FLAG_TILE_WAVES) ? false : nt < hybrid_max_tiles())) ? 4 : 1;
 }
 
+static int g_bwd_riders = [] { const char* e = getenv("IBGS_BWD_RIDERS"); return (e && *e) ? (atoi(e) != 0 ? 1 : 0) : 1; }();
+void render_backward_set_riders(int on) { g_bwd_riders = on != 0 ? 1 : 0; }
+
 int launch_render_backward(hipStream_t s, const ibgs_backward_args& a, const GeomState& g, const BinState& b,
-                           const ImgState& im, const float4* src_rgba, float* slab, float* geo_tab)
+                           const ImgState& im, const float4* src_rgba, float* slab, float* geo_tab, BwdRideDone* done)
 {
     BwdParams p;
     p.ranges = im.ranges; p.point_list = b.point_list; p.rec = reinterpret_cast<const float4*>(g.rec);
@@ -949,12 +1033,19 @@
             hipLaunchKernelGGL(render_bwd_color_small_kernel, grid(4), dim3(64), 0, s, p);
         }
     } else {
-        launch_order(ORDER_SNAKE_ROUNDS, 0);
-        IBGS_HIP(hipGetLastError());
-        risk_slots = nslots;
+        BwdRide r{};
+        if (g_bwd_riders && done && a.tile_order_out && (a.flags & IBGS_FLAG_ORDER_OUT_IS_HINT)) {
+            r.n_order = 1; r.nslots = nslots; r.hint = a.tile_order_out; r.walked = im.tile_walked; r.order_w = im.tile_order;
+            done->order_src = im.tile_order; done->order_dst = a.tile_order_out; done->order_words = nslots;
+        } else {
+            launch_order(ORDER_SNAKE_ROUNDS, 0);
+            IBGS_HIP(hipGetLastError());
+            risk_slots = nslots;
+        }
         StageTimer t(s, IBGS_STAGE_RENDER_BWD);
-        if (noabs) hipLaunchKernelGGL(render_bwd_color_noabs_kernel, dim3((unsigned)nslots), dim3(64), 0, s, p);
-        else hipLaunchKernelGGL(render_bwd_color_kernel, dim3((unsigned)nslots), dim3(64), 0, s, p);
+        const dim3 grid_r((unsigned)(nslots + r.n_order));
+        if (noabs) hipLaunchKernelGGL(render_bwd_color_noabs_kernel, grid_r, dim3(64), 0, s, p, r);
+        else hipLaunchKernelGGL(render_bwd_color_kernel, grid_r, dim3(64), 0, s, p, r);
     }
     IBGS_HIP(hipGetLastError());
     launch_risk(risk_slots);
diff --git a/ibgs_amd/rasterizer.py b/ibgs_amd/rasterizer.py
--- a/ibgs_amd/rasterizer.py
+++ b/ibgs_amd/rasterizer.py
@@ -301,6 +301,7 @@
 
 class _CModule:
     last_tex = None
+    last_order_hint = None
 
     @staticmethod
     def rasterize_gaussians(background, means3D, colors, opacity, scales, rotations, scale_modifier,
@@ -419,12 +420,14 @@
                     a.out_mask = out_mask.data_ptr()
                 elif render_depth_only:
                     a.out_depth = out_depth.data_ptr()
+                _CModule.last_order_hint = None
                 if ORDER_HINT and (ORDER_HINT_GEO or not render_geo) and not render_depth_only and not debug:
                     ckey = _camera_key(viewmatrix, device, W, H, render_geo, stream)
                     oh = _order_hints.get(ckey)
                     if oh is not None:
                         _order_hints.move_to_end(ckey)
                         a.tile_order_hint = oh.data_ptr()
+                        _CModule.last_order_hint = oh
                 hkey = (device.index, P, W, H, render_geo, render_depth_only)
                 hist = _last_rendered.get(hkey) if (RENDERED_HINT and not debug) else None
                 prev = (max(hist) if isinstance(hist, list) else int(hist)) if hist else 0
@@ -462,7 +465,7 @@
                                      src_images, src_rendered_depths, nb_src_images, tan_fovx, tan_fovy,
                                      dL_dout_color, dL_dout_normal_map, dL_dout_median_intersected_depth,
                                      dL_dout_warped_image, sh, degree, campos, geomBuffer, R, binningBuffer,
-                                     imageBuffer, render_geo, debug, plane=None, packed_tex=None, skip_unused=False, buffer_length=0, want_abs=True, sh_rest=None):
+                                     imageBuffer, render_geo, debug, plane=None, packed_tex=None, skip_unused=False, buffer_length=0, want_abs=True, sh_rest=None, order_hint=None):
         lib = _lib.load()
         device = means3D.device
         P = int(means3D.size(0))
@@ -576,6 +579,8 @@
                         else:
                             _order_hints.move_to_end(ckey)
                         a.tile_order_out = oh.data_ptr()
+                        if order_hint is oh:
+                            a.flags |= _lib.FLAG_ORDER_OUT_IS_HINT
                 rc = lib.ibgs_backward(ctypes.byref(a))
                 if rc < 0:
                     raise RuntimeError("ibgs_backward failed (%d): %s" % (rc, _lib.last_error()))
@@ -731,6 +736,7 @@
 
         ctx.raster_settings = raster_settings
         ctx.packed_tex, _CModule.last_tex = _CModule.last_tex, None
+        ctx.order_hint, _CModule.last_order_hint = _CModule.last_order_hint, None
         ctx.plane_mode = int(plane_mode) if plane is not None else 0
         ctx.num_rendered = num_rendered
         ctx.set_materialize_grads(False)
@@ -760,6 +766,8 @@
             kw["plane"] = (plane_normal if plane_normal.numel() else None, plane_offset if plane_offset.numel() else None, ctx.plane_mode)
         if getattr(ctx, "packed_tex", None) is not None:
             kw["packed_tex"] = ctx.packed_tex
+        if getattr(ctx, "order_hint", None) is not None:
+            kw["order_hint"] = ctx.order_hint
         kw["skip_unused"] = True
         kw["buffer_length"] = int(raster_settings.buffer_length)
         kw["want_abs"] = bool(ctx.needs_input_grad[2]) or not NO_ABS_GRAD_WHEN_UNUSED
diff --git a/include/ibgs_rast.h b/include/ibgs_rast.h
--- a/include/ibgs_rast.h
+++ b/include/ibgs_rast.h
@@ -40,6 +40,7 @@
 #define IBGS_FLAG_REF_ARITH 4096u
 #define IBGS_FLAG_SRC_DEPTH_SLOTS 8192u
 #define IBGS_FLAG_NO_ABS_GRAD 1024u
+#define IBGS_FLAG_ORDER_OUT_IS_HINT 16384u
 
 typedef struct ibgs_forward_args {
     void* stream;
```
